# jweyn/DLWP-CS

Measured on AMD Instinct MI355X. Metric: cubed-sphere samples/sec (fwd+bwd), higher is better.
Workload: dtype bf16; 1 GPU; unet2 C48: x (32,6,48,48,14) per GPU, 14 out channels, base 32, MSE + Adam, fwd+bwd+update, bf16 activations + bf16 MFMA, fp32 master weights / gradients / Adam; global_batch=32, parallelism=dp1, hip_graphs=True

## Files before the change

dlwp-cs_amd/DLWP/_native.py:

```python
import ctypes
import os
import threading

import numpy as np
import torch

_HERE = os.path.dirname(os.path.abspath(__file__))
_TAG = os.environ.get('DLWPCS_LIB_TAG', '')
LIB_PATH = os.path.join(os.path.dirname(_HERE), 'lib', 'libdlwpcs%s.so' % ('_' + _TAG if _TAG else ''))

F32 = 0
BF16 = 1
I16 = 2
MAP_RENORMALIZE = 1
MSE_TARGET_F32 = 0x100
MSE_OVERWRITE = 0x200
ADAM_ZERO_GRAD = 1
HEAD_DEFER_STAGE2 = 2
LOSS_MSE, LOSS_MAE, LOSS_ACC = 0, 1, 2
REG_NONE, REG_MSE, REG_MAE, REG_GLOBAL = 0, 1, 2, 3
NORM_ALL, NORM_VALID = 0, 1
E_UNSUPPORTED = -2
ACT_NONE = 0
ACT_LEAKY_CLIP = 1
CONV_ACCUMULATE_WGRAD = 1
CONV_PREPACKED = 2
CONV_REUSE_DZ = 4
CONV_DEFER_REDUCE = 8
CONV_DEFER_RING0 = 16
CONV_OUT_PADDED = 32
CONV_DGRAD_GATHER = 64
CONSTRAINT_MAX_NORM, CONSTRAINT_NON_NEG, CONSTRAINT_UNIT_NORM, CONSTRAINT_MIN_MAX_NORM = 1, 2, 3, 4
PACK_FWD, PACK_BWD, PACK_BIAS = 0, 1, 2
WGRAD_BATCH_MAX = 24

c_void_p, c_int, c_float, c_size_t = ctypes.c_void_p, ctypes.c_int, ctypes.c_float, ctypes.c_size_t
c_i32p = ctypes.POINTER(ctypes.c_int32)


class ConvDesc(ctypes.Structure):
    _fields_ = [('B', ctypes.c_int32), ('N', ctypes.c_int32), ('C0', ctypes.c_int32), ('C1', ctypes.c_int32),
                ('Cout', ctypes.c_int32), ('ksize', ctypes.c_int32), ('halo', ctypes.c_int32),
                ('up0', ctypes.c_int32), ('flip_north_pole', ctypes.c_int32), ('act', ctypes.c_int32),
                ('alpha', ctypes.c_float), ('vmax', ctypes.c_float), ('dtype', ctypes.c_int32),
                ('flags', ctypes.c_int32), ('c0_valid', ctypes.c_int32)]


class PackItem(ctypes.Structure):
    _fields_ = [(n, ctypes.c_void_p) for n in ('w_eq', 'w_pol', 'w_np', 'b_eq', 'b_pol', 'b_np', 'wpk_fwd', 'wpk_bwd',
                                                'bias_pk')] + \
               [(n, ctypes.c_int32) for n in ('ksize', 'Cin', 'Cout', 'flip_north_pole', 'dtype', 'reserved')]


class ReduceItem(ctypes.Structure):
    _fields_ = [(n, ctypes.c_void_p) for n in ('partial', 'bpartial', 'dw_eq', 'dw_pol', 'dw_np', 'db_eq', 'db_pol',
                                                'db_np')] + \
               [(n, ctypes.c_int32) for n in ('ksize', 'Cin', 'Cout', 'CinP', 'CoutP', 'n_eq', 'n_4', 'n_5',
                                              'flip_north_pole', 'accumulate', 'vec', 'nblocks')] + \
               [('reserved', ctypes.c_int32 * 4)]


class WgradItem(ctypes.Structure):
    _fields_ = [('d', ConvDesc)] + [(n, ctypes.c_void_p) for n in ('src0', 'src1', 'dz', 'y', 'table_dev', 'dw_eq', 'dw_pol',
                                                                    'dw_np', 'db_eq', 'db_pol', 'db_np')]


class LossTail(ctypes.Structure):
    _fields_ = [('partial', ctypes.c_void_p), ('loss_out', ctypes.c_void_p), ('nblocks', ctypes.c_int32), ('inv_n', ctypes.c_float),
                ('weight', ctypes.c_float), ('overwrite', ctypes.c_int32)]


class LossDesc(ctypes.Structure):
    _fields_ = [('kind', ctypes.c_int32), ('loss_weight', ctypes.c_float), ('weight', ctypes.c_void_p),
                ('weight_div', ctypes.c_int32), ('weight_period', ctypes.c_int32), ('clim', ctypes.c_void_p),
                ('clim_div', ctypes.c_int32), ('clim_period', ctypes.c_int32), ('regularize', ctypes.c_int32),
                ('reverse', ctypes.c_int32), ('overwrite', ctypes.c_int32)]


class GConvDesc(ctypes.Structure):
    _fields_ = [(n, ctypes.c_int32) for n in
                ('B', 'H', 'W', 'Cin', 'Cout', 'kh', 'kw', 'sh', 'sw', 'dh', 'dw', 'pad_t', 'pad_l', 'Ho', 'Wo',
                 'flip_north_pole', 'dtype')]


SCORE_MSE, SCORE_RMSE, SCORE_MAE, SCORE_ACC, SCORE_COS, SCORE_MEAN = 0, 1, 2, 3, 4, 5
SCORE_MAX_DIMS = 8


class ScoreDesc(ctypes.Structure):
    _fields_ = [(n, ctypes.c_int32) for n in ('method', 'n_lead', 't_len', 't_cap', 't_slope', 'n_keep', 'n_red', 'kc')] + \
               [('keep_ext', ctypes.c_int64 * SCORE_MAX_DIMS), ('red_ext', ctypes.c_int64 * SCORE_MAX_DIMS),
                ('lead_stride', ctypes.c_int64 * 4), ('t_stride', ctypes.c_int64 * 4), ('kc_stride', ctypes.c_int64 * 4),
                ('keep_stride', (ctypes.c_int64 * SCORE_MAX_DIMS) * 4), ('red_stride', (ctypes.c_int64 * SCORE_MAX_DIMS) * 4)]


class OverlapDesc(ctypes.Structure):
    _fields_ = [('N', ctypes.c_int32), ('n_lat', ctypes.c_int32), ('n_lon', ctypes.c_int32), ('reserved', ctypes.c_int32),
                ('frames', ((ctypes.c_double * 3) * 3) * 6), ('dust', ctypes.c_double)]


class CubeBilinearDesc(ctypes.Structure):
    _fields_ = [('N', ctypes.c_int32), ('reserved', ctypes.c_int32), ('n_points', ctypes.c_int64),
                ('frames', ((ctypes.c_double * 3) * 3) * 6), ('edge', ((ctypes.c_int32 * 3) * 4) * 6)]


class SparseMapDesc(ctypes.Structure):
    _fields_ = [('n_a', ctypes.c_int64), ('n_b', ctypes.c_int64), ('nnz', ctypes.c_int64), ('x_dtype', ctypes.c_int32),
                ('n_outer', ctypes.c_int32), ('outer_ext', ctypes.c_int64 * 3), ('x_outer_stride', ctypes.c_int64 * 3),
                ('y_outer_stride', ctypes.c_int64 * 3), ('x_space_stride', ctypes.c_int64), ('y_space_stride', ctypes.c_int64),
                ('inner_ext', ctypes.c_int64), ('x_inner_stride', ctypes.c_int64), ('y_inner_stride', ctypes.c_int64)]


GROUP_SLAB_ROWS = 512


class RowsDesc(ctypes.Structure):
    _fields_ = [('n_inner', ctypes.c_int32), ('reserved', ctypes.c_int32), ('src_row_stride', ctypes.c_int64),
                ('out_row_stride', ctypes.c_int64), ('inner_ext', ctypes.c_int64 * SCORE_MAX_DIMS),
                ('src_stride', ctypes.c_int64 * SCORE_MAX_DIMS), ('out_stride', ctypes.c_int64 * SCORE_MAX_DIMS)]


class ZonalSpectrumDesc(ctypes.Structure):
    _fields_ = [(n, ctypes.c_int32) for n in ('L', 'n_wave', 'n_dims', 'remove_mean')] + \
               [('ext', ctypes.c_int64 * SCORE_MAX_DIMS), ('kept', ctypes.c_int32 * SCORE_MAX_DIMS),
                ('stride', (ctypes.c_int64 * SCORE_MAX_DIMS) * 3)]


ENSEMBLE_MAX_M = 128


class EnsembleDesc(ctypes.Structure):
    _fields_ = [(n, ctypes.c_int32) for n in ('M', 'n_dims', 'fair', 'ddof', 'variance', 'reserved')] + \
               [('member_stride', ctypes.c_int64), ('ext', ctypes.c_int64 * SCORE_MAX_DIMS),
                ('stride', (ctypes.c_int64 * SCORE_MAX_DIMS) * 2)]


AFFINE_MUL_ADD, AFFINE_SUB_DIV = 0, 1
AFFINE_MAX_CHANNELS = 1024


class ChanDesc(ctypes.Structure):
    _fields_ = [(n, ctypes.c_int64) for n in ('R', 'C', 'S', 'row_stride', 'chan_stride', 'inner_stride', 'dst_row_stride',
                                              'dst_chan_stride', 'dst_inner_stride')]


PROTOTYPES = {
    'dlwpcs_version': (c_int, []),
    'dlwpcs_last_error': (ctypes.c_char_p, []),
    'dlwpcs_halo_table': (c_int, [c_int, c_int, c_void_p]),
    'dlwpcs_halo_inverse_table': (c_int, [c_int, c_int, c_void_p]),
    'dlwpcs_dgrad_gather_plan_ints': (c_size_t, [c_int]),
    'dlwpcs_dgrad_gather_plan': (c_int, [c_int, c_void_p]),
    'dlwpcs_pad_fwd': (c_int, [c_void_p, c_void_p, c_int, c_int, c_int, c_int, c_int, c_void_p, c_void_p]),
    'dlwpcs_pad_bwd': (c_int, [c_void_p, c_void_p, c_int, c_int, c_int, c_int, c_int, c_void_p, c_void_p]),
    'dlwpcs_conv_workspace_bytes': (c_size_t, [ctypes.POINTER(ConvDesc)]),
    'dlwpcs_conv_packed_bytes': (c_size_t, [ctypes.POINTER(ConvDesc), c_int]),
    'dlwpcs_pack_batch': (c_int, [c_void_p, c_int, c_void_p]),
    'dlwpcs_conv_fwd': (c_int, [ctypes.POINTER(ConvDesc)] + [c_void_p] * 8 + [c_void_p, c_void_p, c_void_p, c_size_t,
                                                                                 c_void_p]),
    'dlwpcs_conv_fwd_pool': (c_int, [ctypes.POINTER(ConvDesc)] + [c_void_p] * 8 + [c_void_p, c_void_p, c_void_p, c_void_p, c_size_t,
                                                                                      c_void_p]),
    'dlwpcs_conv_fwd_head': (c_int, [ctypes.POINTER(ConvDesc)] + [c_void_p] * 4 + [ctypes.POINTER(ConvDesc)] + [c_void_p] * 6 +
                             [c_size_t, ctypes.POINTER(c_int), c_void_p]),
    'dlwpcs_conv_bwd_data': (c_int, [ctypes.POINTER(ConvDesc)] + [c_void_p] * 5 + [c_void_p, c_void_p, c_void_p,
                                                                                      c_void_p, c_size_t, c_void_p]),
    'dlwpcs_conv_bwd_data_masked': (c_int, [ctypes.POINTER(ConvDesc)] + [c_void_p] * 4 + [c_void_p] * 4 + [c_float, c_float] +
                                    [c_void_p, c_void_p, c_size_t, c_void_p]),
    'dlwpcs_conv_small_fwd': (c_int, [ctypes.POINTER(ConvDesc)] + [c_void_p] * 8 + [c_void_p, c_void_p, c_void_p, c_size_t,
                                                                                       c_void_p]),
    'dlwpcs_conv_small_bwd_data': (c_int, [ctypes.POINTER(ConvDesc)] + [c_void_p] * 4 + [c_void_p] * 4 + [c_float, c_float] +
                                   [c_void_p, c_void_p, c_size_t, c_void_p]),
    'dlwpcs_conv_bwd_weights': (c_int, [ctypes.POINTER(ConvDesc)] + [c_void_p] * 4 + [c_void_p] * 6 +
                                [c_void_p, c_void_p, c_size_t, c_void_p]),
    'dlwpcs_conv_wgrad_reduce_item': (c_int, [ctypes.POINTER(ConvDesc)] + [c_void_p] * 6 +
                                      [c_void_p, c_size_t, ctypes.POINTER(ReduceItem)]),
    'dlwpcs_wgrad_reduce_batch': (c_int, [c_void_p, c_void_p, c_int, c_void_p]),
    'dlwpcs_wgrad_batch_supported': (c_int, [ctypes.POINTER(ConvDesc)]),
    'dlwpcs_wgrad_batch_sizes': (c_int, [c_void_p, c_int, ctypes.POINTER(c_size_t), ctypes.POINTER(c_size_t)]),
    'dlwpcs_wgrad_batch_plan': (c_int, [c_void_p, c_int, c_void_p, c_size_t]),
    'dlwpcs_wgrad_batch': (c_int, [c_void_p, c_int, c_void_p, c_void_p, c_void_p, c_size_t, c_void_p]),
    'dlwpcs_wgrad_batch_adam': (c_int, [c_void_p, c_int, c_void_p, c_void_p, c_void_p, c_size_t, c_void_p, c_void_p, c_void_p,
                                        c_void_p, c_size_t, c_void_p, c_void_p, c_void_p]),
    'dlwpcs_wgrad_batch_adam_tail': (c_int, [c_void_p, c_int, c_void_p, c_void_p, c_void_p, c_size_t, c_void_p, c_void_p, c_void_p,
                                             c_void_p, c_size_t, c_void_p, c_void_p, c_void_p, c_void_p, c_void_p]),
    'dlwpcs_wgrad_batch_apply': (c_int, [c_void_p, c_int, c_void_p, c_void_p, c_void_p, c_void_p, c_void_p, c_void_p, c_size_t,
                                         c_void_p, c_void_p, c_void_p, c_void_p, c_void_p]),
    'dlwpcs_gconv_fwd': (c_int, [ctypes.POINTER(GConvDesc)] + [c_void_p] * 9),
    'dlwpcs_gconv_bwd_data': (c_int, [ctypes.POINTER(GConvDesc)] + [c_void_p] * 6),
    'dlwpcs_gconv_bwd_weights': (c_int, [ctypes.POINTER(GConvDesc)] + [c_void_p] * 9),
    'dlwpcs_act_fwd': (c_int, [c_void_p, c_void_p, c_size_t, c_int, c_float, c_float, c_int, c_void_p]),
    'dlwpcs_act_bwd': (c_int, [c_void_p, c_void_p, c_void_p, c_size_t, c_int, c_float, c_float, c_int, c_void_p]),
    'dlwpcs_avgpool2_fwd': (c_int, [c_void_p, c_void_p, c_int, c_int, c_int, c_int, c_void_p]),
    'dlwpcs_avgpool2_bwd': (c_int, [c_void_p, c_void_p, c_int, c_int, c_int, c_int, c_void_p]),
    'dlwpcs_avgpool2_bwd_add': (c_int, [c_void_p, c_void_p, c_void_p, c_int, c_int, c_int, c_int, c_void_p]),
    'dlwpcs_avgpool2_bwd_masked': (c_int, [c_void_p, c_void_p, c_void_p, c_void_p, c_int, c_int, c_int, c_float, c_float, c_int,
                                           c_void_p]),
    'dlwpcs_avgpool2_bwd_ring': (c_int, [c_void_p, c_void_p, c_void_p, c_void_p, c_int, c_int, c_int, c_float, c_float, c_int,
                                         c_void_p, c_void_p, c_int, c_int, c_void_p]),
    'dlwpcs_conv_ring_info': (c_int, [ctypes.POINTER(ConvDesc), ctypes.POINTER(c_size_t), ctypes.POINTER(c_int)]),
    'dlwpcs_upsample2_fwd': (c_int, [c_void_p, c_void_p, c_int, c_int, c_int, c_int, c_void_p]),
    'dlwpcs_upsample2_bwd': (c_int, [c_void_p, c_void_p, c_int, c_int, c_int, c_int, c_void_p]),
    'dlwpcs_concat2': (c_int, [c_void_p, c_void_p, c_void_p, c_size_t, c_int, c_int, c_int, c_void_p]),
    'dlwpcs_split2': (c_int, [c_void_p, c_void_p, c_void_p, c_size_t, c_int, c_int, c_int, c_void_p]),
    'dlwpcs_cf_to_cl': (c_int, [c_void_p, c_void_p, c_int, c_int, c_size_t, c_int, c_void_p]),
    'dlwpcs_cl_to_cf': (c_int, [c_void_p, c_void_p, c_int, c_int, c_size_t, c_int, c_void_p]),
    'dlwpcs_add': (c_int, [c_void_p, c_void_p, c_void_p, c_size_t, c_int, c_void_p]),
    'dlwpcs_l1l2_regularize': (c_int, [c_void_p, c_void_p, c_size_t, c_float, c_float, c_float, c_void_p, c_void_p]),
    'dlwpcs_weight_constraint': (c_int, [c_void_p, c_int, c_int, c_int, c_float, c_float, c_float, c_void_p]),
    'dlwpcs_mse_scratch_bytes': (c_size_t, []),
    'dlwpcs_mse_fwd_bwd': (c_int, [c_void_p, c_void_p, c_void_p, c_void_p, c_size_t, c_float, c_int, c_void_p,
                                   c_void_p]),
    'dlwpcs_loss_scratch_bytes': (c_size_t, []),
    'dlwpcs_loss_fwd_bwd': (c_int, [c_void_p, c_void_p, c_void_p, c_void_p, c_void_p, c_size_t, c_int, c_void_p, c_void_p]),
    'dlwpcs_loss_masked_fwd_bwd': (c_int, [c_void_p, c_void_p, c_void_p, c_int, c_void_p, c_void_p, c_void_p, c_size_t, c_int,
                                           c_void_p, c_void_p]),
    'dlwpcs_head_loss_step': (c_int, [c_void_p, c_void_p, c_void_p, c_void_p, c_void_p, c_void_p, c_void_p, c_void_p, c_void_p,
                                      c_void_p, c_void_p, c_int, c_float, c_float, c_void_p]),
    'dlwpcs_score_scratch_bytes': (c_size_t, [c_void_p]),
    'dlwpcs_score': (c_int, [c_void_p, c_void_p, c_void_p, c_void_p, c_void_p, c_void_p, c_int, c_void_p, c_size_t, c_void_p]),
    'dlwpcs_score_indexed': (c_int, [c_void_p, c_void_p, c_void_p, c_void_p, c_void_p, c_void_p, ctypes.c_int64, c_void_p, c_int,
                                     c_void_p, c_size_t, c_void_p]),
    'dlwpcs_score_plan_info': (c_int, [c_void_p, c_void_p, c_void_p, c_void_p, c_void_p, c_int, ctypes.c_int64, c_void_p]),
    'dlwpcs_group_mean_scratch_bytes': (c_size_t, [c_void_p, c_int, ctypes.c_int64, c_int]),
    'dlwpcs_group_mean': (c_int, [c_void_p, c_void_p, c_void_p, c_void_p, c_int, ctypes.c_int64, c_int, c_void_p, c_void_p,
                                  c_void_p, c_size_t, c_void_p]),
    'dlwpcs_rows_gather': (c_int, [c_void_p, c_void_p, c_void_p, ctypes.c_int64, c_void_p, c_void_p]),
    'dlwpcs_sparse_map_apply': (c_int, [c_void_p, c_void_p, c_void_p, c_void_p, c_void_p, c_void_p, c_void_p]),
    'dlwpcs_sparse_map_apply_masked': (c_int, [c_void_p, c_void_p, c_void_p, c_void_p, c_void_p, c_void_p, c_void_p, c_float, c_int,
                                               c_void_p]),
    'dlwpcs_missing_count': (c_int, [c_void_p, c_int, ctypes.c_int64, ctypes.c_int64, c_void_p, c_void_p]),
    'dlwpcs_fill_missing': (c_int, [c_void_p, c_int, c_size_t, c_void_p, c_int, c_int, c_void_p]),
    'dlwpcs_zonal_spectrum_scratch_bytes': (c_size_t, [c_void_p]),
    'dlwpcs_zonal_spectrum': (c_int, [c_void_p, c_void_p, c_void_p, c_void_p, c_void_p, c_void_p, c_void_p, c_void_p, c_void_p]),
    'dlwpcs_ensemble_stats': (c_int, [c_void_p, c_void_p, c_void_p, c_void_p, c_void_p, c_void_p, c_void_p, c_void_p]),
    'dlwpcs_ensemble_plan_info': (c_int, [c_void_p, c_void_p, c_void_p, c_void_p]),
    'dlwpcs_overlap_count': (c_int, [c_void_p, c_void_p, c_void_p, c_void_p, c_void_p]),
    'dlwpcs_overlap_fill': (c_int, [c_void_p, c_void_p, c_void_p, c_void_p, c_void_p, c_void_p, ctypes.c_int64, c_void_p]),
    'dlwpcs_cube_bilinear': (c_int, [c_void_p, c_void_p, c_void_p, c_void_p, c_void_p, c_void_p]),
    'dlwpcs_adam_step': (c_int, [c_void_p, c_void_p, c_void_p, c_void_p, c_size_t, c_void_p, c_float, c_float,
                                 c_float, c_float, c_float, c_void_p]),
    'dlwpcs_adam_step_fused': (c_int, [c_void_p, c_void_p, c_void_p, c_void_p, c_size_t, c_void_p, c_float, c_float,
                                       c_float, c_float, c_float, c_int, c_void_p]),
    'dlwpcs_pad_channels': (c_int, [c_void_p, c_void_p, c_size_t, c_int, c_int, c_int, c_void_p]),
    'dlwpcs_slice_channels': (c_int, [c_void_p, c_void_p, c_size_t, c_int, c_int, c_int, c_void_p]),
    'dlwpcs_state_repack': (c_int, [c_void_p, c_void_p, c_void_p, c_int, c_size_t, c_int, c_int, c_int, c_int, c_void_p]),
    'dlwpcs_head_mse_scratch_bytes': (c_size_t, []),
    'dlwpcs_head_mse_tail': (c_int, [c_void_p, c_float, c_int, c_void_p, c_void_p, c_void_p]),
    'dlwpcs_loss_tail_run': (c_int, [c_void_p, c_void_p]),
    'dlwpcs_head_mse_step': (c_int, [c_void_p, c_void_p, c_void_p, c_void_p, c_void_p, c_void_p, c_float, c_void_p, c_void_p,
                                     c_void_p, c_int, c_void_p, c_void_p]),
    'dlwpcs_head_mse_step_masked': (c_int, [c_void_p, c_void_p, c_void_p, c_void_p, c_void_p, c_void_p, c_float, c_void_p,
                                            c_void_p, c_void_p, c_int, c_void_p, c_float, c_float, c_void_p]),
    'dlwpcs_adam_step_dev': (c_int, [c_void_p, c_void_p, c_void_p, c_void_p, c_size_t, c_void_p, c_void_p, c_int,
                                     c_void_p]),
    'dlwpcs_batch_gather': (c_int, [c_void_p, ctypes.c_int64, c_int, ctypes.c_int64, c_void_p, c_int, c_void_p, c_int,
                                    c_int, c_int, c_int, c_void_p, c_int, c_int, c_int, c_int, c_int, c_void_p]),
    'dlwpcs_solar_fill': (c_int, [c_void_p, ctypes.c_int64, c_void_p, ctypes.c_int64, c_void_p, c_int, c_int, c_int, c_int,
                                  c_void_p, c_int, c_int, c_int, c_int, c_int, c_void_p]),
    'dlwpcs_channel_moments_scratch_bytes': (c_size_t, [c_void_p, ctypes.c_int64]),
    'dlwpcs_channel_moments': (c_int, [c_void_p, c_void_p, c_void_p, ctypes.c_int64, c_void_p, c_int, c_void_p, c_void_p, c_size_t,
                                       c_void_p]),
    'dlwpcs_channel_affine': (c_int, [c_void_p, c_void_p, c_void_p, c_void_p, c_int, c_void_p, c_void_p]),
    'dlwpcs_channel_range_scratch_bytes': (c_size_t, [ctypes.c_int64, ctypes.c_int64, ctypes.c_int64]),
    'dlwpcs_channel_range': (c_int, [c_void_p, ctypes.c_int64, ctypes.c_int64, ctypes.c_int64, c_void_p, c_void_p, c_void_p,
                                     c_size_t, c_void_p]),
    'dlwpcs_pack_i16': (c_int, [c_void_p, ctypes.c_int64, ctypes.c_int64, ctypes.c_int64, c_void_p, c_void_p, c_void_p, c_void_p]),
    'dlwpcs_unpack_i16': (c_int, [c_void_p, ctypes.c_int64, ctypes.c_int64, ctypes.c_int64, c_void_p, c_void_p, c_void_p,
                                  c_void_p]),
    'dlwpcs_batch_gather_i16': (c_int, [c_void_p, ctypes.c_int64, c_int, ctypes.c_int64, c_void_p, c_void_p, c_void_p, c_int,
                                        c_void_p, c_int, c_int, c_int, c_int, c_void_p, c_int, c_int, c_int, c_int, c_int,
                                        c_void_p]),
    'dlwpcs_comm_load': (c_int, [ctypes.c_char_p]),
    'dlwpcs_comm_unique_id': (c_int, [c_void_p]),
    'dlwpcs_comm_init': (c_int, [ctypes.POINTER(c_void_p), c_void_p, c_int, c_int]),
    'dlwpcs_comm_destroy': (c_int, [c_void_p]),
    'dlwpcs_allreduce_f32': (c_int, [c_void_p, c_void_p, c_size_t, c_void_p]),
    'dlwpcs_lds_oob_probe': (c_int, [c_void_p, c_void_p]),
    'dlwpcs_prof_enable': (c_int, [c_int]),
    'dlwpcs_prof_reset': (c_int, []),
    'dlwpcs_prof_count': (c_int, []),
    'dlwpcs_prof_get': (c_int, [c_int, ctypes.c_char_p, c_int, ctypes.POINTER(ctypes.c_double),
                                ctypes.POINTER(ctypes.c_double), ctypes.POINTER(ctypes.c_double)]),
    'dlwpcs_prof_known_tags': (c_int, []),
    'dlwpcs_prof_known_tag': (c_int, [c_int, ctypes.c_char_p, c_int]),
}

_lib = None
_lock = threading.Lock()


class NativeError(RuntimeError):
    pass


def lib():
    global _lib
    if _lib is None:
        with _lock:
            if _lib is None:
                if not os.path.exists(LIB_PATH):
                    raise NativeError(
                        'libdlwpcs.so not found at %s: build it with `python dlwp-cs_amd/build.py` '
                        '(or __graft_entry__.build()).  The DLWP-CS MI355X engine has no CPU fallback.' % LIB_PATH)
                handle = ctypes.CDLL(LIB_PATH)
                for name, (res, args) in PROTOTYPES.items():
                    fn = getattr(handle, name)
                    fn.restype = res
                    fn.argtypes = args
                _lib = handle
    return _lib


def check(rc, what):
    if rc != 0:
        msg = lib().dlwpcs_last_error()
        msg = msg.decode() if msg else ''
        if rc == -1:
            raise ValueError('%s: %s' % (what, msg))
        if rc == -2:
            raise NotImplementedError('%s: %s' % (what, msg))
        raise NativeError('%s failed (code %d): %s' % (what, rc, msg))


def require_device(t, what):
# ... 103 lines not shown
```

dlwp-cs_amd/DLWP/custom.py:

```python


import numpy as np

from . import ops
from ._native import ACT_LEAKY_CLIP, ACT_NONE
from .keras import constraints, engine, regularizers
from .keras.callbacks import Callback, EarlyStopping
from .keras.engine import Layer
from .keras.losses import LossSpec, mean_absolute_error, mean_squared_error, spec_of



def _normalize_tuple(value, n, name):
    if isinstance(value, int):
        return (value,) * n
    try:
        value_tuple = tuple(value)
    except TypeError:
        raise ValueError('The `' + name + '` argument must be a tuple of ' + str(n) + ' integers. Received: ' +
                         str(value))
    if len(value_tuple) != n:
        raise ValueError('The `' + name + '` argument must be a tuple of ' + str(n) + ' integers. Received: ' +
                         str(value))
    for single_value in value_tuple:
# ... 27 lines not shown


def _conv_output_length(input_length, filter_size, padding, stride, dilation=1):
    if input_length is None:
        return None
    dilated_filter_size = filter_size + (filter_size - 1) * (dilation - 1)
    if padding == 'same':
        output_length = input_length
    else:
        output_length = input_length - dilated_filter_size + 1
    return (output_length + stride - 1) // stride



class CubeSpherePadding2D(Layer):

    def __init__(self, padding=(1, 1), data_format='channels_first', **kwargs):
        data_format = _normalize_data_format(data_format)
        super(CubeSpherePadding2D, self).__init__(**kwargs)
        if isinstance(padding, int):
            padding = ((padding, padding), (padding, padding), (padding, padding))
        elif hasattr(padding, '__len__'):
            if len(padding) != 3:
                raise ValueError('`padding` should have 3 elements. Found: ' + str(padding))
            dim1_padding = _normalize_tuple(padding[0], 2, '1st entry of padding')
            dim2_padding = _normalize_tuple(padding[1], 2, '2nd entry of padding')
            dim3_padding = _normalize_tuple(padding[2], 2, '3rd entry of padding')
            padding = (dim1_padding, dim2_padding, dim3_padding)
        else:
            raise ValueError('`padding` should be either an int, a tuple of 3 ints (symmetric_dim1_pad, '
                             'symmetric_dim2_pad, symmetric_dim3_pad), or a tuple of 3 tuples of 2 ints ((left_dim1_pad, '
                             'right_dim1_pad), (left_dim2_pad, right_dim2_pad), (left_dim3_pad, right_dim2_pad)). '
                             'Found: ' + str(padding))
        self.data_format = data_format
        self.padding = ((0, 0),) + tuple(padding[1:])

    def compute_output_shape(self, input_shape):
        input_shape = tuple(input_shape)
        add = [q[0] + q[1] for q in self.padding]
        if self.data_format == 'channels_first':
            dims = [None if input_shape[2 + i] is None else input_shape[2 + i] + add[i] for i in range(3)]
            return (input_shape[0], input_shape[1]) + tuple(dims)
        dims = [None if input_shape[1 + i] is None else input_shape[1 + i] + add[i] for i in range(3)]
        return (input_shape[0],) + tuple(dims) + (input_shape[4],)

    def call(self, inputs):
        p = self.padding[1][0]
        if self.data_format == 'channels_first':
            x = ops.channels_first_to_last(inputs)
            return ops.channels_last_to_first(ops.cs_pad(x, p))
        return ops.cs_pad(inputs, p)

    def get_config(self):
        config = {'padding': self.padding, 'data_format': self.data_format}
        base_config = super(CubeSpherePadding2D, self).get_config()
        return dict(list(base_config.items()) + list(config.items()))


class CubeSphereConv2D(Layer):

    def __init__(self,
                 filters,
                 kernel_size,
                 strides=1,
                 padding='valid',
                 data_format='channels_first',
                 dilation_rate=1,
                 activation=None,
                 use_bias=True,
                 flip_north_pole=True,
                 independent_north_pole=False,
                 kernel_initializer='glorot_uniform',
                 bias_initializer='zeros',
                 kernel_regularizer=None,
                 bias_regularizer=None,
                 activity_regularizer=None,
                 kernel_constraint=None,
                 bias_constraint=None,
                 **kwargs):
        super(CubeSphereConv2D, self).__init__(**kwargs)
        self.filters = filters
        self.kernel_size = _normalize_tuple(kernel_size, 2, 'kernel_size')
        self.strides = _normalize_tuple(strides, 2, 'strides')
        self.padding = _normalize_padding(padding)
        self.data_format = _normalize_data_format(data_format)
        self.dilation_rate = _normalize_tuple(dilation_rate, 2, 'dilation_rate')
        self.activation = engine.get_activation(activation)
        self.use_bias = use_bias
        self.flip_north_pole = flip_north_pole
        self.independent_north_pole = independent_north_pole
        self.kernel_initializer = engine.get_initializer(kernel_initializer)
        self.bias_initializer = engine.get_initializer(bias_initializer)
        self.kernel_regularizer = regularizers.get(kernel_regularizer)
        self.bias_regularizer = regularizers.get(bias_regularizer)
        self.activity_regularizer = engine._passthrough_get(activity_regularizer)
        self.kernel_constraint = constraints.get(kernel_constraint)
        self.bias_constraint = constraints.get(bias_constraint)
        self.rank = 3

        self.equatorial_kernel = None
        self.equatorial_bias = None
        self.polar_kernel = None
        self.polar_bias = None
        self.north_pole_kernel = None
        self.north_pole_bias = None

    def _weight_attr_names(self):
        return ['equatorial_kernel', 'polar_kernel', 'north_pole_kernel', 'equatorial_bias', 'polar_bias',
                'north_pole_bias']

    def build(self, input_shape):
        if self.data_format == 'channels_first':
            channel_axis = 1
        else:
            channel_axis = -1
        if input_shape[channel_axis] is None:
            raise ValueError('The channel dimension of the inputs should be defined. Found `None`.')
        input_dim = int(input_shape[channel_axis])
        kernel_shape = self.kernel_size + (input_dim, self.filters)

        self.equatorial_kernel = self.add_weight(shape=kernel_shape, initializer=self.kernel_initializer,
                                                 name='equatorial_kernel', regularizer=self.kernel_regularizer,
                                                 constraint=self.kernel_constraint)
        self.polar_kernel = self.add_weight(shape=kernel_shape, initializer=self.kernel_initializer,
                                            name='polar_kernel', regularizer=self.kernel_regularizer,
                                            constraint=self.kernel_constraint)
        if self.independent_north_pole:
            self.north_pole_kernel = self.add_weight(shape=kernel_shape, initializer=self.kernel_initializer,
                                                     name='north_pole_kernel', regularizer=self.kernel_regularizer,
                                                     constraint=self.kernel_constraint)
        if self.use_bias:
            self.equatorial_bias = self.add_weight(shape=(self.filters,), initializer=self.bias_initializer,
                                                   name='equatorial_bias', regularizer=self.bias_regularizer,
                                                   constraint=self.bias_constraint)
            self.polar_bias = self.add_weight(shape=(self.filters,), initializer=self.bias_initializer,
                                              name='polar_bias', regularizer=self.bias_regularizer,
                                              constraint=self.bias_constraint)
            if self.independent_north_pole:
                self.north_pole_bias = self.add_weight(shape=(self.filters,), initializer=self.bias_initializer,
                                                       name='north_pole_bias', regularizer=self.bias_regularizer,
                                                       constraint=self.bias_constraint)
        self.input_dim = input_dim
        self.built = True

    def _is_mfma_config(self):
        k = self.kernel_size
        return (k[0] == k[1] and k[0] in (1, 3) and self.strides == (1, 1) and self.dilation_rate == (1, 1)
                and self.padding == 'valid')

    def can_fuse_halo(self, pad_width):
        return (self._is_mfma_config() and self.kernel_size[0] == 3 and pad_width == 1 and self.activation is None)

    def fused_call(self, src0, src1=None, up0=False, halo=True, act=ACT_NONE, alpha=0.0, vmax=0.0, premask0=None,
                   premask1=None, dy_premasked=False, defer_ring0=False, want_pool=False, out_padded=False, small=False):
        return ops.cs_conv(src0, self.equatorial_kernel, self.polar_kernel, self.north_pole_kernel,
                           self.equatorial_bias, self.polar_bias, self.north_pole_bias, src1=src1,
                           ksize=self.kernel_size[0], halo=halo, up0=up0, flip_north_pole=self.flip_north_pole,
                           act=act, alpha=alpha, vmax=vmax, premask0=premask0, premask1=premask1,
                           dy_premasked=dy_premasked, defer_ring0=defer_ring0, want_pool=want_pool, out_padded=out_padded,
                           small=small)

    def call(self, inputs, channels_last_io=False, **kwargs):
        channels_first = self.data_format == 'channels_first' and not channels_last_io
        x = ops.channels_first_to_last(inputs) if channels_first else inputs
        if self._is_mfma_config():
            outputs = ops.cs_conv(x, self.equatorial_kernel, self.polar_kernel, self.north_pole_kernel,
                                  self.equatorial_bias, self.polar_bias, self.north_pole_bias,
                                  ksize=self.kernel_size[0], halo=False, flip_north_pole=self.flip_north_pole)
        else:
            outputs = ops.cs_gconv(x, self.equatorial_kernel, self.polar_kernel, self.north_pole_kernel,
                                   self.equatorial_bias, self.polar_bias, self.north_pole_bias,
                                   strides=self.strides, padding=self.padding, dilation=self.dilation_rate,
                                   flip_north_pole=self.flip_north_pole)
        if channels_first:
            outputs = ops.channels_last_to_first(outputs)
        if self.activation is not None:
            return self.activation(outputs)
        return outputs

    def compute_output_shape(self, input_shape):
        if self.data_format == 'channels_last':
            space = input_shape[2:4]
        else:
            space = input_shape[-2:]
        new_space = []
        for i in range(len(space)):
            new_space.append(_conv_output_length(space[i], self.kernel_size[i], padding=self.padding,
                                                 stride=self.strides[i], dilation=self.dilation_rate[i]))
        if self.data_format == 'channels_last':
            return (input_shape[0], 6) + tuple(new_space) + (self.filters,)
        return (input_shape[0], self.filters, 6) + tuple(new_space)

    def get_config(self):
        config = {
            'filters': self.filters,
            'kernel_size': self.kernel_size,
            'strides': self.strides,
            'padding': self.padding,
            'data_format': self.data_format,
            'dilation_rate': self.dilation_rate,
            'activation': engine.serialize_activation(self.activation),
            'use_bias': self.use_bias,
            'flip_north_pole': self.flip_north_pole,
            'independent_north_pole': self.independent_north_pole,
            'kernel_initializer': engine.serialize_initializer(self.kernel_initializer),
            'bias_initializer': engine.serialize_initializer(self.bias_initializer),
            'kernel_regularizer': regularizers.serialize(self.kernel_regularizer),
            'bias_regularizer': regularizers.serialize(self.bias_regularizer),
            'activity_regularizer': self.activity_regularizer,
            'kernel_constraint': constraints.serialize(self.kernel_constraint),
            'bias_constraint': constraints.serialize(self.bias_constraint)
        }
        base_config = super(CubeSphereConv2D, self).get_config()
        return dict(list(base_config.items()) + list(config.items()))



def _adam_effective_lr(optimizer, beta_1, beta_2, with_bias_correction):
    it = float(optimizer.iterations)
    lr = float(optimizer.lr) / (1. + float(getattr(optimizer, 'decay', 0.)) * it)
    if with_bias_correction:
        t = it + 1.
        lr = lr * np.sqrt(1. - np.power(beta_2, t)) / (1. - np.power(beta_1, t))
    return lr


class AdamLearningRateTracker(Callback):

    def on_epoch_end(self, epoch, logs=None, beta_1=0.9, beta_2=0.999, ):
        print(' - LR: {:.6f}'.format(_adam_effective_lr(self.model.optimizer, beta_1, beta_2, True)))


class SGDLearningRateTracker(Callback):

    def on_epoch_end(self, epoch, logs=None):
        print(' - LR: {:.6f}'.format(_adam_effective_lr(self.model.optimizer, 0., 0., False)))


class BatchHistory(Callback):

    def on_train_begin(self, logs=None):
        self.history, self.epoch = [], 0

    def on_epoch_begin(self, epoch, logs=None):
        self.history.append(dict())

    def on_batch_end(self, batch, logs=None):
        for key, value in (logs or {}).items():
            self.history[self.epoch].setdefault(key, []).append(value)

    def on_epoch_end(self, epoch, logs=None):
        self.epoch += 1


class RunHistory(Callback):

    def __init__(self, run):
        super(RunHistory, self).__init__()
        self.run = run
        self.epoch, self.history = [], {}

    def on_train_begin(self, logs=None):
        self.epoch, self.history = [], {}

    def on_epoch_end(self, epoch, logs=None):
        self.epoch.append(epoch)
        for key, value in (logs or {}).items():
            self.history.setdefault(key, []).append(value)
            self.run.log(key, value)


class RNNResetStates(Callback):

    def on_epoch_begin(self, epoch, logs=None):
        self.model.reset_states()


class EarlyStoppingMin(EarlyStopping):

    def __init__(self, min_epochs=0, max_epochs=None, **kwargs):
        super(EarlyStoppingMin, self).__init__(**kwargs)
        if not isinstance(min_epochs, int) or min_epochs < 0:
            raise ValueError('min_epochs must be an integer >= 0')
        self.min_epochs = int(min_epochs)
        self.max_epochs = None if max_epochs is None else int(max_epochs)

    def _stop(self, epoch, message):
        self.stopped_epoch = epoch
        self.model.stop_training = True
        if self.restore_best_weights:
            if self.verbose > 0:
                print(message)
            self.model.set_weights(self.best_weights)

    def on_epoch_end(self, epoch, logs=None):
        if epoch < self.min_epochs:
            return
        current = self.get_monitor_value(logs)
        if current is None:
            return
        improved = self.monitor_op(current - self.min_delta, self.best)
        if improved:
            self.best, self.wait = current, 0
            if self.restore_best_weights:
                self.best_weights = self.model.get_weights()
        else:
            self.wait += 1
            if self.wait >= self.patience:
                self._stop(epoch, 'Restoring model weights from the end of the best epoch')
        if self.max_epochs is not None and epoch >= self.max_epochs:
            self._stop(epoch, 'Maximum epochs reached; restoring model weights from the end of the best epoch')
        if self.verbose > 1:
            print('EarlyStoppingMin: %d epochs since last minimum' % self.wait)
# ... 169 lines not shown
```

dlwp-cs_amd/DLWP/keras/models.py:

```python
import gc
import json
import os
import sys
import time

import numpy as np
import torch

from .. import ops, parallel
from ..options import option
from .. import _native as _nat
from .._native import ACT_LEAKY_CLIP, ACT_NONE
from . import backend, callbacks as cbks, losses as klosses, optimizers, staging
from .engine import KTensor, Layer
from .layers import AveragePooling3D, Concatenate, InputLayer, ReLU, UpSampling3D


def _new_graph():
    if os.environ.get('DLWPCS_KEEP_GRAPH', '0') == '1':
        return torch.cuda.CUDAGraph(keep_graph=True)
    return torch.cuda.CUDAGraph()


def _as_list(x):
    if isinstance(x, (list, tuple)):
        return list(x)
    return [x]


class Model(object):
    def __init__(self, inputs=None, outputs=None, name=None):
        if inputs is None or outputs is None:
            raise ValueError('Model needs `inputs` and `outputs`')
        self._single_input = not isinstance(inputs, (list, tuple))
        self.inputs = _as_list(inputs)
        self.outputs = _as_list(outputs)
        self._single_output = len(self.outputs) == 1
        for t in self.inputs + self.outputs:
            if not isinstance(t, KTensor):
                raise ValueError('Model inputs/outputs must be symbolic tensors created by Input() and layer calls')
        self.name = name or 'model'
        self.stop_training = False
        self.optimizer = None
        self.loss = None
        self._dev_losses = None
        self.loss_weights = None
        self.metrics = []
        self.history = None
        self.use_graphs = option('graphs')
        self.compute_dtype = backend.compute_dtype()
        self.prepack_weights = True
        self.wgrad_side_stream = False
        self.defer_wgrad_reduce = True
        self.batch_wgrad = option('wgrad_batch')
        self.check_finite = option('check_finite')
        self.fuse_adam = option('fuse_adam')
        self.fold_ring = option('fold_ring')
        self.fuse_pool = option('fuse_pool')
        self.fold_loss_tail = option('fold_loss_tail')
        self.fuse_pack = option('fuse_pack')
        self._packed_ok = False
        self.exchange_buckets = int(os.environ.get('DLWPCS_EXCHANGE_BUCKETS', '1'))
        self._stager = None
        self.fuse_head_loss = option('fuse_head')
        self.fold_head = option('fold_head')
        self.small_conv = option('small_conv')
        self.static_batch_buffers = False
        self._ones = {}
        self._compiled = False
        self._flat_params = self._flat_grads = None
        self._grads_clean = False
        self._graphs = {}
        self._infer_graphs = {}
        self._rollout_series = {}
        self.rollout_keep_bytes = 4 << 30
        self._seen_batch = {}
        self._toposort()
        self._build_plan()

    def _toposort(self):
        order, seen = [], set()

        def visit(t):
            if t.uid in seen:
                return
            seen.add(t.uid)
            for i in t.node_inputs:
                visit(i)
            order.append(t)
        for o in self.outputs:
            visit(o)
        input_uids = {t.uid for t in self.inputs}
        for t in order:
            if isinstance(t.layer, InputLayer) and t.uid not in input_uids:
                raise ValueError('Graph disconnected: cannot obtain value for tensor %r' % (t,))
        self._nodes = order
        layers, seen_l = [], set()
        for t in self.inputs + order:
            if t.layer is not None and id(t.layer) not in seen_l:
                seen_l.add(id(t.layer))
                layers.append(t.layer)
        self.layers = layers

    def _build_plan(self):
        consumers = {}
        for t in self._nodes:
            for i in t.node_inputs:
                consumers.setdefault(i.uid, []).append(t)
        out_uids = {o.uid for o in self.outputs}

        def sole_consumer(t):
            c = consumers.get(t.uid, [])
            return c[0] if (len(c) == 1 and t.uid not in out_uids) else None

        from ..custom import CubeSphereConv2D, CubeSpherePadding2D
        def cf_layer(t):
            lay = t.layer
            if isinstance(lay, InputLayer):
                return len(t.shape) == 5
            if isinstance(lay, CubeSphereConv2D) and lay.activation is not None \
                    and getattr(lay.activation, '_dlwp_name', None) != 'relu':
                return False
            if isinstance(lay, (CubeSpherePadding2D, CubeSphereConv2D, AveragePooling3D, UpSampling3D)):
                return lay.data_format == 'channels_first'
            if isinstance(lay, Concatenate):
                return lay._axis(len(t.shape)) == 1
            return isinstance(lay, ReLU)
        self._cf_model = (option('cf_model') and all(cf_layer(t) for t in self._nodes)
                          and any(isinstance(t.layer, (CubeSphereConv2D, CubeSpherePadding2D)) for t in self._nodes))
        fmt = 'channels_first' if self._cf_model else 'channels_last'
        virtual = set()
        fused = {}
        for t in self._nodes:
            lay = t.layer
            if not isinstance(lay, CubeSphereConv2D) or len(t.node_inputs) != 1:
                continue
            padt = t.node_inputs[0]
            if not isinstance(padt.layer, CubeSpherePadding2D) or sole_consumer(padt) is not t:
                continue
            if padt.layer.data_format != fmt or lay.data_format != fmt or not lay.can_fuse_halo(padt.layer.padding[1][0]):
                continue
            if padt.layer.padding[1] != padt.layer.padding[2] or padt.layer.padding[1][0] != padt.layer.padding[1][1]:
                continue
            x = padt.node_inputs[0]
            src0, src1, up0 = x, None, False
            chain = [padt]
            if isinstance(x.layer, Concatenate) and len(x.node_inputs) == 2 and sole_consumer(x) is padt \
                    and x.layer._axis(len(x.shape)) == (1 if self._cf_model else len(x.shape) - 1):
                src0, src1 = x.node_inputs
                chain.append(x)
            if isinstance(src0.layer, UpSampling3D) and sole_consumer(src0) is (chain[-1]) \
                    and src0.layer.size == (1, 2, 2):
                chain.append(src0)
                src0 = src0.node_inputs[0]
                up0 = True
            out_t, act, alpha, vmax = t, ACT_NONE, 0.0, 0.0
            nxt = sole_consumer(t)
            if nxt is not None and isinstance(nxt.layer, ReLU) and nxt.layer.threshold == 0.:
                out_t, act = nxt, ACT_LEAKY_CLIP
                alpha = nxt.layer.negative_slope
                vmax = float('inf') if nxt.layer.max_value is None else nxt.layer.max_value
                virtual.add(t.uid)
            for c in chain:
                virtual.add(c.uid)
            fused[out_t.uid] = ('fused_conv', out_t.uid, lay, src0.uid, None if src1 is None else src1.uid, up0, act,
                                alpha, vmax)
        steps = []
        for t in self._nodes:
            if isinstance(t.layer, InputLayer) or t.uid in virtual and t.uid not in fused:
                continue
            if t.uid in fused:
                steps.append(fused[t.uid])
            elif isinstance(t.layer, AveragePooling3D) and len(t.node_inputs) == 1 and self._runs_channels_last(t.layer) and (
                    len(consumers.get(t.node_inputs[0].uid, [])) > 1 or t.node_inputs[0].uid in out_uids):
                steps.append(('pool_skip', t.uid, t.layer, t.node_inputs[0].uid))
            else:
                steps.append(('layer', t.uid, t.layer, [i.uid for i in t.node_inputs],
                              isinstance(t.layer, Concatenate)))
        self._plan = steps
        self.n_fused = len(fused)
        self._padded_io_ok = False
        if len(self.inputs) == 1:
            u = self.inputs[0].uid
            rd = [st for st in steps
                  if (st[0] == 'fused_conv' and u in (st[3], st[4])) or (st[0] == 'pool_skip' and st[3] == u)
                  or (st[0] == 'layer' and u in st[3])]
            self._padded_io_ok = (len(rd) == 1 and rd[0][0] == 'fused_conv' and rd[0][3] == u and rd[0][4] is None
                                  and not rd[0][5] and u not in out_uids and not self._cf_model)
        self._plan_premask(steps, out_uids)
        self._head_fold = {}
        for i, st in enumerate(steps):
            if st[0] != 'fused_conv' or st[1] in out_uids:
                continue
            rd = [j for j, s2 in enumerate(steps)
                  if (s2[0] == 'fused_conv' and st[1] in (s2[3], s2[4])) or (s2[0] == 'pool_skip' and s2[3] == st[1])
                  or (s2[0] == 'layer' and st[1] in s2[3])]
            if len(rd) != 1 or steps[rd[0]][0] != 'layer':
                continue
            hl = steps[rd[0]][2]
            if (isinstance(hl, CubeSphereConv2D) and len(steps[rd[0]][3]) == 1 and tuple(hl.kernel_size) == (1, 1)
                    and hl.activation is None and not hl.independent_north_pole and not st[2].independent_north_pole
                    and st[2].filters == 32 and self._runs_channels_last(hl) and not self._cf_model):
                self._head_fold[i] = rd[0]
        uids = [o.uid for o in self.outputs]
        self._sole_outputs = {u for u in uids if not consumers.get(u) and uids.count(u) == 1}

    def _plan_premask(self, steps, out_uids):
        from ..custom import CubeSphereConv2D
        produced = {}
        for st in steps:
            if st[0] == 'fused_conv' and st[6] == ACT_LEAKY_CLIP:
                produced[st[1]] = (float(st[7]), float(st[8]))
        capable = {u: (u not in out_uids) for u in produced}
        in_uids_model = {t.uid for t in self.inputs}
        for st in steps:
            if st[0] == 'fused_conv' and st[1] in capable and st[3] in in_uids_model and (st[4] is None or st[4] in in_uids_model):
                capable[st[1]] = False
        aliased = set()
        src_mask = {}
# ... 19 lines not shown
        self._src_mask = src_mask
        readers = {}
        for i, st in enumerate(steps):
            ins = [st[3], st[4]] if st[0] == 'fused_conv' else ([st[3]] if st[0] == 'pool_skip' else list(st[3]))
            for u in ins:
                if u is not None:
                    readers.setdefault(u, []).append(i)
        self._pool_producers = set()
        for i, st in enumerate(steps):
            if st[0] == 'fused_conv':
                r = readers.get(st[1], [])
                if r and steps[r[0]][0] == 'pool_skip' and steps[r[0]][3] == st[1]:
                    self._pool_producers.add(i)
        self._defer_ring = set()
        for i, st in enumerate(steps):
            if st[0] != 'pool_skip' or not (src_mask.get(i) and st[3] in self._premask):
                continue
            r = readers.get(st[1], [])
            if len(r) == 1 and st[1] not in out_uids and steps[r[0]][0] == 'fused_conv' and steps[r[0]][3] == st[1] \
                    and steps[r[0]][4] != st[1] and not steps[r[0]][5]:
                self._defer_ring.add(r[0])

    def _runs_channels_last(self, lay):
        return lay.data_format == 'channels_last' or self._cf_model

    def _plan_exchange(self):
        if self._exchange_cut is not None:
            return self._exchange_cut or None
        self._exchange_cut = False
        if self._flat_grads is None:
            return None
        base = self._flat_grads.data_ptr()
        spans = []
        for st in self._plan:
            ws = [w for w in getattr(st[2], '_weights', []) if w.requires_grad and w.grad is not None]
            if ws:
                lo = min((w.grad.data_ptr() - base) // 4 for w in ws)
                hi = max((w.grad.data_ptr() - base) // 4 + w.numel() for w in ws)
                spans.append((lo, hi))
            else:
                spans.append(None)
        total = sum(hi - lo for sp in spans if sp for lo, hi in [sp])
        if total == 0:
            return None
        acc, cut = 0, None
        for i in range(len(spans) - 1, 0, -1):
            if spans[i]:
                acc += spans[i][1] - spans[i][0]
                if acc >= 0.4 * total:
                    cut = i
                    break
        if cut is None or not any(spans[:cut]):
            return None
        lo_a = min(sp[0] for sp in spans[cut:] if sp)
        if any(sp and sp[1] > lo_a for sp in spans[:cut]):
            return None
        self._exchange_cut = (cut, int(lo_a) // 64 * 64)
        return self._exchange_cut

    def _premask_on(self):
        return (self.compute_dtype == 'bfloat16' and torch.is_grad_enabled()
                and option('premask'))

    def _pack_state(self, device):
        from ..custom import CubeSphereConv2D
        from .. import _native as nat
        tag = nat.BF16 if self.compute_dtype == 'bfloat16' else nat.F32
        key = (str(device), tag, self._flat_params.data_ptr() if self._flat_params is not None else 0)
        st = getattr(self, '_pack_cache', None)
        if st is not None and st['key'] == key:
            return st
        entries, table, by_grad = [], {}, {}
        for lay in self.layers:
            if not isinstance(lay, CubeSphereConv2D) or not lay.built or not lay._is_mfma_config():
                continue
            we = lay.equatorial_kernel
            if we.device != device or id(we) in table:
                continue
            bufs = ops.conv_packed_buffers(lay.kernel_size[0], we.shape[2], we.shape[3], tag, device,
                                           bias=lay.equatorial_bias is not None)
            entries.append((we, lay.polar_kernel, lay.north_pole_kernel, lay.equatorial_bias, lay.polar_bias,
                            lay.north_pole_bias, bufs, lay.kernel_size[0], lay.flip_north_pole, tag))
            table[id(we)] = (tag, bufs[0], bufs[1], bufs[2])
            if we.grad is not None:
                by_grad[we.grad.data_ptr()] = entries[-1]
        st = {'key': key, 'items': ops.make_pack_items(entries, device) if entries else None, 'n': len(entries),
              'table': table, 'keep': entries, 'by_grad': by_grad}
        self._pack_cache = st
        return st

    def _forward(self, inputs, repack=True, fuse_targets=None):
        want = backend.torch_dtype(self.compute_dtype)
        inputs = [v if v.dtype == want else v.to(want) for v in inputs]
        if inputs and inputs[0].is_cuda and self.prepack_weights:
            st = self._pack_state(inputs[0].device)
            if st['n'] and (repack or not st.get('packed')):
                ops.pack_batch(st['items'], st['n'])
                st['packed'] = True
                st['packed_version'] = self._flat_params._version if self._flat_params is not None else None
                self._packed_ok = True
            ops.PREPACKED = st['table']
            try:
                return self._run_plan(inputs, fuse_targets)
            finally:
                ops.PREPACKED = {}
        return self._run_plan(inputs, fuse_targets)

    def _run_plan(self, inputs, fuse_targets=None):
        from ..custom import CubeSphereConv2D, CubeSpherePadding2D
        cf = self._cf_model
        if cf:
            inputs = [ops.channels_first_to_last(v) for v in inputs]
        values = {t.uid: v for t, v in zip(self.inputs, inputs)}
        self._fused_outputs = set()
        pm = self._premask if self._premask_on() else {}
        cut = getattr(self, '_record_cut', None)
        self._cut_tensors = []
        ops._POOLED.clear()
        folded = set()
        for i, st in enumerate(self._plan):
            if i in folded:
                continue
            if cut is not None and i == cut:
                need, seen = set(), set()
                for s2 in self._plan[cut:]:
                    ins = [s2[3], s2[4]] if s2[0] == 'fused_conv' else ([s2[3]] if s2[0] == 'pool_skip' else list(s2[3]))
                    need.update(u for u in ins if u is not None)
                for u, v in values.items():
                    if u in need and isinstance(v, torch.Tensor) and v.requires_grad and id(v) not in seen:
                        seen.add(id(v))
                        self._cut_tensors.append(v)
            if st[0] == 'fused_conv':
                _, out_uid, lay, s0, s1, up0, act, alpha, vmax = st
                j = self._head_fold.get(i) if self.fold_head else None
                if j is not None and fuse_targets is None and not torch.is_grad_enabled():
                    hl, h_uid = self._plan[j][2], self._plan[j][1]
                    padded = bool(getattr(self, '_padded_io', False) and h_uid in self._sole_outputs and hl.filters % 8 != 0)
                    if (lay._is_mfma_config() and hl._is_mfma_config() and hl.built and lay.built and ops.cs_conv_head_applicable(
                            values[s0], None if s1 is None else values[s1], lay.equatorial_kernel, hl.equatorial_kernel, padded)):
                        values[h_uid] = ops.cs_conv_head(values[s0], lay.equatorial_kernel, lay.equatorial_bias,
                                                         hl.equatorial_kernel, hl.equatorial_bias,
                                                         src1=None if s1 is None else values[s1], up0=up0,
                                                         flip_north_pole=lay.flip_north_pole, act=act, alpha=alpha, vmax=vmax,
                                                         out_padded=padded)
                        folded.add(j)
                        continue
                m0, m1 = self._src_mask[i]
                values[out_uid] = lay.fused_call(values[s0], None if s1 is None else values[s1], up0=up0, halo=True,
                                                 act=act, alpha=alpha, vmax=vmax,
                                                 premask0=pm.get(s0) if m0 else None, premask1=pm.get(s1) if m1 else None,
                                                 dy_premasked=out_uid in pm,
                                                 defer_ring0=bool(pm) and self.fold_ring and i in self._defer_ring,
                                                 want_pool=self.fuse_pool and i in self._pool_producers,
                                                 small=self.small_conv)
            elif st[0] == 'pool_skip':
                _, out_uid, lay, in_uid = st
                values[out_uid], values[in_uid] = ops.avgpool2_skip(values[in_uid],
                                                                     pm.get(in_uid) if self._src_mask[i] else None)
                if cut is not None and i < cut:
                    values[in_uid] = ops.detour(values[in_uid])
            else:
                _, out_uid, lay, in_uids, takes_list = st
                args = [values[u] for u in in_uids]
                head_pm = pm.get(in_uids[0]) if (self._src_mask[i] and in_uids) else None
                if (fuse_targets is not None and out_uid in fuse_targets and out_uid in self._sole_outputs
                        and isinstance(lay, CubeSphereConv2D) and len(args) == 1 and lay._is_mfma_config()
                        and self._runs_channels_last(lay) and lay.activation is None and lay.north_pole_kernel is None
                        and ops.head_mse_applicable(args[0], lay.equatorial_kernel, lay.kernel_size[0], ACT_NONE,
                                                    fuse_targets[out_uid][0], fuse_targets[out_uid][2])):
                    tgt, wgt, dl = fuse_targets[out_uid]
                    values[out_uid] = ops.head_mse(args[0], tgt, lay.equatorial_kernel, lay.polar_kernel, lay.equatorial_bias,
                                                   lay.polar_bias, wgt, lay.flip_north_pole, premask=head_pm, loss=dl)
                    self._fused_outputs.add(out_uid)
                    continue
                if head_pm is not None:
                    values[out_uid] = lay.fused_call(args[0], halo=False, premask0=head_pm)
                    continue
                if (getattr(self, '_padded_io', False) and out_uid in self._sole_outputs and isinstance(lay, CubeSphereConv2D)
                        and len(args) == 1 and lay._is_mfma_config() and self._runs_channels_last(lay)
                        and lay.activation is None and lay.kernel_size[0] == 1 and args[0].dtype == torch.bfloat16
                        and args[0].shape[-1] == 32 and 8 <= lay.filters <= 32 and lay.filters % 2 == 0
                        and (args[0].shape[2] * args[0].shape[3]) % 16 == 0):
                    values[out_uid] = lay.fused_call(args[0], halo=False, out_padded=True)
                    continue
                if cf:
                    if isinstance(lay, CubeSphereConv2D):
                        values[out_uid] = lay.call(args[0], channels_last_io=True)
                    elif isinstance(lay, CubeSpherePadding2D):
                        values[out_uid] = ops.cs_pad(args[0], lay.padding[1][0])
                    elif isinstance(lay, AveragePooling3D):
                        values[out_uid] = ops.avgpool2(args[0])
                    elif isinstance(lay, UpSampling3D):
                        values[out_uid] = ops.upsample2(args[0])
                    elif isinstance(lay, Concatenate):
                        values[out_uid] = ops.concat_channels(list(args))
                    else:
                        values[out_uid] = lay.call(args[0])
                    continue
                values[out_uid] = lay.call(args if (takes_list or len(args) > 1) else args[0])
        if cf and not getattr(self, '_loss_in_cl', False):
            return [values[o.uid] if o.uid in self._fused_outputs else ops.channels_last_to_first(values[o.uid])
                    for o in self.outputs]
        return [values[o.uid] for o in self.outputs]

    def __call__(self, inputs):
        self._grads_clean = False
        outs = self._forward(_as_list(inputs))
        return outs[0] if self._single_output else outs

    def _weight_layers(self):
        return [l for l in self.layers if l._weights]

    @property
    def weights(self):
        return [w for l in self._weight_layers() for w in l._weights]

    @property
    def trainable_weights(self):
        return [w for w in self.weights if w.requires_grad]

    def count_params(self):
        return int(sum(w.numel() for w in self.weights))

    def get_weights(self):
        return [a for l in self._weight_layers() for a in l.get_weights()]

    def set_weights(self, weights):
        weights = list(weights)
        n = sum(len(l._weights) for l in self._weight_layers())
        if len(weights) != n:
            raise ValueError('You called `set_weights(weights)` on model "%s" with a weight list of length %d, but the '
                             'model was expecting %d weights.' % (self.name, len(weights), n))
        k = 0
        for l in self._weight_layers():
            l.set_weights(weights[k:k + len(l._weights)])
            k += len(l._weights)

    def _flatten_parameters(self):
        ws = self.weights
        dev = backend.device()
        total = sum(w.numel() for w in ws)
        offsets, off = [], 0
        for w in ws:
            offsets.append(off)
            off += (w.numel() + 63) // 64 * 64
        flat = torch.zeros(off, dtype=torch.float32, device=dev)
        grads = torch.zeros(off, dtype=torch.float32, device=dev)
        k = 0
        for l in self._weight_layers():
            new = []
            for w in l._weights:
                o = offsets[k]
                view = flat[o:o + w.numel()].view(w.shape)
                with torch.no_grad():
                    view.copy_(w.detach().to(dev))
                view.requires_grad_(w.requires_grad)
                if w.requires_grad:
                    view.grad = grads[o:o + w.numel()].view(w.shape)
                new.append(view)
                k += 1
            l._rebind(new)
        self._flat_params, self._flat_grads = flat, grads
        self._wrules = None
        self._flat_len = off
        self._n_params = total
        self._exchange_cut = None

    def compile(self, optimizer='adam', loss=None, metrics=None, loss_weights=None, **kwargs):
        self.optimizer = optimizers.get(optimizer)
        mp_dtype = getattr(self.optimizer, '_mixed_precision', None)
        if mp_dtype is not None and mp_dtype != backend.compute_dtype() and mp_dtype != self.compute_dtype:
            import warnings
            warnings.warn('compile(): the optimizer was returned by enable_mixed_precision_graph_rewrite(); the model is put '
                          'into the %s mode although the global policy is %s now (pass a fresh optimizer to avoid this)'
                          % (mp_dtype, backend.compute_dtype()))
        if mp_dtype is not None and mp_dtype != self.compute_dtype:
            self.compute_dtype = mp_dtype
            self._pack_cache = None
        n_out = len(self.outputs)
        losses = _as_list(loss) if isinstance(loss, (list, tuple)) else [loss] * n_out
        if len(losses) != n_out:
            raise ValueError('When passing a list as loss, it should have one entry per model output. The model has %d '
                             'outputs, but you passed loss=%s' % (n_out, loss))
        specs = []
        for l in losses:
            sp = klosses.spec_of(l) if not isinstance(l, str) or l in ('mse', 'mean_squared_error', 'MSE') else None
            if sp is None and isinstance(l, str):
                raise NotImplementedError("loss %r: of the loss names the DLWP-CS engine takes 'mse' (reference "
                                          "Azure/train_cs.py:424); pass the function for the others, e.g. "
                                          "DLWP.keras.losses.mean_absolute_error" % (l,))
            if sp is None:
                raise NotImplementedError("loss %r: the DLWP-CS engine provides 'mse', 'mae' (DLWP.keras.losses) and the "
                                          "losses of DLWP.custom: latitude_weighted_loss, anomaly_correlation(_loss), masked_loss" % (l,))
            if sp.regularize == 'spatial':
                raise NotImplementedError("anomaly-correlation regularize_mean='spatial': a per-sample reduction over the layout's "
                                          "last two axes (reference DLWP/custom.py:1604-1606,1657-1659) the DLWP-CS engine does "
                                          "not build")
            if sp.kind == 'acc' and parallel.world()[1] > 1:
                raise NotImplementedError('the anomaly-correlation loss is a ratio of sums over the WHOLE batch: per-rank values '
                                          'averaged across %d data-parallel ranks are a different loss (train it on one rank)'
                                          % parallel.world()[1])
            if sp.masked == 'valid' and parallel.world()[1] > 1:
                raise NotImplementedError("masked_loss(normalize='valid') divides by the number of valid elements of the WHOLE "
                                          "batch: per-rank nan-means averaged across %d data-parallel ranks are a different loss "
                                          "(train it on one rank, or use normalize='all', which is exact under averaging)"
                                          % parallel.world()[1])
            specs.append(sp)
# ... 1307 lines not shown
```

dlwp-cs_amd/DLWP/ops.py:

```python
import ctypes
import os

import numpy as np
import torch

from . import _native as nat
from .options import option
from ._native import ConvDesc, GConvDesc, check, lib, ptr, require_device, stream_ptr

DIRECT_PARAM_GRADS = False

PREPACKED = {}

WGRAD_SIDE_STREAM = False
_side_streams = {}


def side_stream(device):
    key = str(device)
    st = _side_streams.get(key)
    if st is None:
        st = torch.cuda.Stream(device=device)
        _side_streams[key] = st
    return st
# ... 257 lines not shown
def _c(t):
    return t if t.is_contiguous() else t.contiguous()



class _CSPad(torch.autograd.Function):
    @staticmethod
    def forward(ctx, x, p):
        require_device(x, 'cs_pad')
        x = _c(x)
        B, F6, N, N2, C = x.shape
        if F6 != 6 or N != N2:
            raise ValueError('cs_pad: expected (B, 6, N, N, C), got %s' % (tuple(x.shape),))
        table, inv = nat.halo_tables(N, p, x.device)
        y = torch.empty((B, 6, N + 2 * p, N + 2 * p, C), dtype=x.dtype, device=x.device)
        check(lib().dlwpcs_pad_fwd(ptr(x), ptr(y), B, N, C, p, nat.dtype_tag(x), ptr(table), stream_ptr()),
              'dlwpcs_pad_fwd')
        ctx.p, ctx.shape = p, (B, N, C)
        ctx.inv = inv
        return y

    @staticmethod
    def backward(ctx, dy):
        B, N, C = ctx.shape
        dy = _c(dy)
        dx = torch.empty((B, 6, N, N, C), dtype=dy.dtype, device=dy.device)
        check(lib().dlwpcs_pad_bwd(ptr(dy), ptr(dx), B, N, C, ctx.p, nat.dtype_tag(dy), ptr(ctx.inv), stream_ptr()),
              'dlwpcs_pad_bwd')
        return dx, None


def cs_pad(x, p):
    return _CSPad.apply(x, int(p))



def _make_desc(B, N, C0, C1, Cout, ksize, halo, up0, flip, act, alpha, vmax, dtype=nat.F32, c0_valid=0):
    return ConvDesc(B=B, N=N, C0=C0, C1=C1, Cout=Cout, ksize=ksize, halo=int(halo), up0=int(up0),
                    flip_north_pole=int(flip), act=int(act), alpha=float(alpha), vmax=float(vmax), dtype=int(dtype),
                    flags=0, c0_valid=int(c0_valid))


class _PadChannels(torch.autograd.Function):

    @staticmethod
    def forward(ctx, x, cp):
        require_device(x, 'pad_channels')
        x = _c(x)
        C = x.shape[-1]
        rows = x.numel() // C if C else 0
        y = torch.empty(tuple(x.shape[:-1]) + (cp,), dtype=x.dtype, device=x.device)
        check(lib().dlwpcs_pad_channels(ptr(x), ptr(y), rows, C, cp, nat.dtype_tag(x), stream_ptr()), 'dlwpcs_pad_channels')
        ctx.c = C
        return y

    @staticmethod
    def backward(ctx, dy):
        dy = _c(dy)
        cp = dy.shape[-1]
        rows = dy.numel() // cp
        dx = torch.empty(tuple(dy.shape[:-1]) + (ctx.c,), dtype=dy.dtype, device=dy.device)
        check(lib().dlwpcs_slice_channels(ptr(dy), ptr(dx), rows, cp, ctx.c, nat.dtype_tag(dy), stream_ptr()),
              'dlwpcs_slice_channels')
        return dx, None


def pad_channels(x, cp):
    if x.shape[-1] == cp:
        return x
    if x.shape[-1] > cp:
        raise ValueError('pad_channels: tensor has %d channels, asked for %d' % (x.shape[-1], cp))
    return _PadChannels.apply(x, int(cp))


def channel_vector(dtype):
    return 8 if dtype == torch.bfloat16 else 4


def padded_channels(c, dtype, even_too=None):
    v = channel_vector(dtype)
    if c % v == 0:
        return c
    if c % 2 == 1 or even_too:
        return (c + v - 1) // v * v
    return c


def _f32_param(t, what):
    if t is not None and t.dtype != torch.float32:
        raise TypeError('%s: parameters must be float32 master copies, got %s' % (what, t.dtype))


def _weight_gradients(d, src0, src1, dy, y, params, table, ws, nbytes, direct, defer, need, has_np, has_bias, has_bnp,
                      batch_mask_ok=False):
    dev = dy.device
    w_eq, w_pol, w_np = params[0], params[1], params[2]
    dw_eq = dw_pol = dw_np = db_eq = db_pol = db_np = None
    if (direct and WGRAD_BATCH and d.B > 0 and not WGRAD_SIDE_STREAM and wgrad_batch_supported(d)
            and (d.act == nat.ACT_NONE or (batch_mask_ok and d.ksize == 3 and y is not None))):
        pe, pp, pn, be, bp, bn = params
        d2 = ConvDesc.from_buffer_copy(d)
        _wb_pending.append((d2, src0, src1, dy, table,
                            (pe.grad, pp.grad, None if pn is None else pn.grad, None if be is None else be.grad,
                             None if bp is None else bp.grad, None if bn is None else bn.grad),
                            None if d.act == nat.ACT_NONE else y))
        return dw_eq, dw_pol, dw_np, db_eq, db_pol, db_np
    if direct:
        pe, pp, pn, be, bp, bn = params
        d2 = ConvDesc.from_buffer_copy(d)
        d2.flags = d.flags | nat.CONV_ACCUMULATE_WGRAD | (nat.CONV_DEFER_REDUCE if defer else 0)
        grads = (ptr(pe.grad), ptr(pp.grad), ptr(None if pn is None else pn.grad),
                 ptr(None if be is None else be.grad), ptr(None if bp is None else bp.grad),
                 ptr(None if bn is None else bn.grad))

        def launch(wsx):
            check(lib().dlwpcs_conv_bwd_weights(ctypes.byref(d2), ptr(src0), ptr(src1), ptr(dy), ptr(y), *grads,
                                                ptr(table), ptr(wsx), wsx.numel(), stream_ptr()),
                  'dlwpcs_conv_bwd_weights')
            if defer:
                item = nat.ReduceItem()
                check(lib().dlwpcs_conv_wgrad_reduce_item(ctypes.byref(d2), *grads, ptr(wsx), wsx.numel(),
                                                          ctypes.byref(item)), 'dlwpcs_conv_wgrad_reduce_item')
                _deferred.append((item, wsx))
        if WGRAD_SIDE_STREAM:
            side = side_stream(dev)
            side.wait_stream(torch.cuda.current_stream(dev))
            ws2 = _workspace(nbytes, dev, 'side')
            with torch.cuda.stream(side):
                launch(ws2)
            for t in (src0, src1, dy, y):
                if t is not None:
                    t.record_stream(side)
        else:
            launch(ws)
    elif any(need):
        dw_eq, dw_pol = torch.empty_like(w_eq), torch.empty_like(w_pol)
        dw_np = torch.empty_like(w_np) if has_np else None
        if has_bias:
            db_eq = torch.empty(d.Cout, dtype=torch.float32, device=dev)
            db_pol = torch.empty(d.Cout, dtype=torch.float32, device=dev)
            db_np = torch.empty(d.Cout, dtype=torch.float32, device=dev) if has_bnp else None
        check(lib().dlwpcs_conv_bwd_weights(ctypes.byref(d), ptr(src0), ptr(src1), ptr(dy), ptr(y), ptr(dw_eq),
                                            ptr(dw_pol), ptr(dw_np), ptr(db_eq), ptr(db_pol), ptr(db_np),
                                            ptr(table), ptr(ws), ws.numel(), stream_ptr()),
              'dlwpcs_conv_bwd_weights')
    return dw_eq, dw_pol, dw_np, db_eq, db_pol, db_np


class _CSConv(torch.autograd.Function):

    @staticmethod
    def forward(ctx, src0, src1, w_eq, w_pol, w_np, b_eq, b_pol, b_np, ksize, halo, up0, flip, act, alpha, vmax,
                c0_valid=0, premask0=None, premask1=None, dy_premasked=False, defer_ring0=False, want_pool=False,
                out_padded=False, small=False):
        require_device(src0, 'cs_conv')
        src0 = _c(src0)
        B = src0.shape[0]
        if src0.dim() != 5 or src0.shape[1] != 6 or src0.shape[2] != src0.shape[3]:
            raise ValueError('cs_conv: expected (B, 6, N, N, C), got %s' % (tuple(src0.shape),))
        N = src0.shape[2] * (2 if up0 else 1)
        C0 = src0.shape[4]
        C1 = 0
        if src1 is not None:
            require_device(src1, 'cs_conv')
            src1 = _c(src1)
            if tuple(src1.shape[:4]) != (B, 6, N, N):
                raise ValueError('cs_conv: src1 shape %s does not match (B,6,%d,%d,*)' % (tuple(src1.shape), N, N))
            C1 = src1.shape[4]
            if src1.dtype != src0.dtype:
                raise TypeError('cs_conv: src0 is %s but src1 is %s' % (src0.dtype, src1.dtype))
        for prm in (w_eq, w_pol, w_np, b_eq, b_pol, b_np):
            _f32_param(prm, 'cs_conv')
        kh, kw, cin, Cout = w_eq.shape
        if kh != ksize or kw != ksize or cin != (c0_valid or C0) + C1:
            raise ValueError('cs_conv: kernel shape %s does not match ksize=%d, C_in=%d' % (tuple(w_eq.shape), ksize,
                                                                                          (c0_valid or C0) + C1))
        w_eq, w_pol = _c(w_eq), _c(w_pol)
        w_np = _c(w_np) if w_np is not None else None
        d = _make_desc(B, N, C0, C1, Cout, ksize, halo, up0, flip, act, alpha, vmax, nat.dtype_tag(src0), c0_valid)
        No = N if halo else N - ksize + 1
        if out_padded:
            if torch.is_grad_enabled() and any(t is not None and t.requires_grad for t in (src0, src1, w_eq)):
                raise RuntimeError('cs_conv: out_padded is an inference-only layout')
            d.flags |= nat.CONV_OUT_PADDED
        y = torch.empty((B, 6, No, No, (Cout + 7) // 8 * 8 if out_padded else Cout), dtype=src0.dtype, device=src0.device)
        table = inv = None
        if halo:
            table, inv = nat.halo_tables(N, (ksize - 1) // 2, src0.device)
        nbytes = lib().dlwpcs_conv_workspace_bytes(ctypes.byref(d))
        ws = _workspace(nbytes, src0.device)
        packed = PREPACKED.get(id(w_eq))
        if packed is not None and packed[0] != d.dtype:
            packed = None
        yp = None
        if want_pool and halo and No % 2 == 0:
            yp = torch.empty((B, 6, No // 2, No // 2, Cout), dtype=src0.dtype, device=src0.device)
        wargs = ((ptr(packed[1]), 0, 0, ptr(packed[2]) if b_eq is not None else 0, 0, 0) if packed is not None else
                 (ptr(w_eq), ptr(w_pol), ptr(w_np), ptr(b_eq), ptr(b_pol), ptr(b_np)))
        if packed is not None:
            d.flags |= nat.CONV_PREPACKED
        small = bool(small) and _small_conv_ok(d)
        if yp is not None:
            check(lib().dlwpcs_conv_fwd_pool(ctypes.byref(d), ptr(src0), ptr(src1), *wargs, ptr(y), ptr(yp), ptr(table), ptr(ws),
                                             ws.numel(), stream_ptr()), 'dlwpcs_conv_fwd_pool')
            _POOLED[y.data_ptr()] = yp
        else:
            rc = nat.E_UNSUPPORTED
            if small:
                rc = lib().dlwpcs_conv_small_fwd(ctypes.byref(d), ptr(src0), ptr(src1), *wargs, ptr(y), ptr(table), ptr(ws),
                                                 ws.numel(), stream_ptr())
            if rc == nat.E_UNSUPPORTED:
                rc = lib().dlwpcs_conv_fwd(ctypes.byref(d), ptr(src0), ptr(src1), *wargs, ptr(y), ptr(table), ptr(ws),
                                           ws.numel(), stream_ptr())
            check(rc, 'dlwpcs_conv_fwd')
        ctx.small = small
        if premask0 is not None and premask1 is not None and tuple(premask0) != tuple(premask1):
            raise ValueError('cs_conv: both sources must share the activation parameters of their masks')
        ctx.premask = (premask0, premask1)
        ctx.dy_premasked = bool(dy_premasked) and act != nat.ACT_NONE
        ctx.defer_ring0 = bool(defer_ring0)
        ctx.packed = packed
        ctx.desc = d
        ctx.tables = (table, inv)
        ctx.has = (src1 is not None, w_np is not None, b_eq is not None, b_np is not None)
        ctx.params = (w_eq, w_pol, w_np, b_eq, b_pol, b_np)
        ctx.save_for_backward(src0, src1, w_eq, w_pol, w_np, y if act != nat.ACT_NONE else None)
        return y

    @staticmethod
    def backward(ctx, dy):
        src0, src1, w_eq, w_pol, w_np, y = ctx.saved_tensors
        d = ctx.desc
        table, inv = ctx.tables
        has_src1, has_np, has_bias, has_bnp = ctx.has
        dy = _c(dy)
        dev = dy.device
        nbytes = lib().dlwpcs_conv_workspace_bytes(ctypes.byref(d))
        need = ctx.needs_input_grad
        dsrc0 = torch.empty_like(src0) if need[0] else None
        dsrc1 = torch.empty_like(src1) if (has_src1 and need[1]) else None
        want_w = any(need[2:8])
        direct = DIRECT_PARAM_GRADS and (need[2] or need[3]) and all(
            p is None or (p.is_leaf and p.grad is not None and p.grad.is_contiguous()) for p in ctx.params)
        pm0, pm1 = ctx.premask
        if dsrc0 is None:
            pm0 = None
        if dsrc1 is None:
            pm1 = None
        masked_io = ctx.dy_premasked or pm0 is not None or pm1 is not None
        if masked_io:
            if ctx.dy_premasked or d.act == nat.ACT_NONE:
                dz = dy
            else:
                dz = torch.empty_like(dy)
                check(lib().dlwpcs_act_bwd(ptr(dy), ptr(y), ptr(dz), dy.numel(), nat.ACT_LEAKY_CLIP, d.alpha, d.vmax,
                                           nat.dtype_tag(dy), stream_ptr()), 'dlwpcs_act_bwd')
            dn = ConvDesc.from_buffer_copy(d)
            dn.act = nat.ACT_NONE
            dn.flags = (d.flags & nat.CONV_PREPACKED) | _gather_flag(d, dev)
            batching = (direct and WGRAD_BATCH and d.B > 0 and not WGRAD_SIDE_STREAM and wgrad_batch_supported(dn))
            defer = direct and DEFER_WGRAD_REDUCE and not WGRAD_SIDE_STREAM and d.B > 0 and not batching
            ws = _workspace(nbytes, dev, 'defer%d' % len(_deferred)) if defer else _workspace(nbytes, dev)
            ring = None
            if ctx.defer_ring0 and dsrc0 is not None and pm0 is None and halo_ring_info(dn) is not None:
                ring = halo_ring_info(dn)
                dn.flags |= nat.CONV_DEFER_RING0
                if not defer:
                    ws = _workspace(nbytes, dev, 'ring%d' % len(_pending_ring))
            if dsrc0 is not None or dsrc1 is not None:
                wq = ctx.packed[3] if ctx.packed is not None else w_eq
                pm = pm0 if pm0 is not None else pm1
                ma, mv = (float(pm[0]), float(pm[1])) if pm is not None else (0.0, 0.0)
                bargs = (ctypes.byref(dn), ptr(dz), ptr(wq), ptr(w_pol), ptr(w_np), ptr(dsrc0), ptr(dsrc1),
                         ptr(src0 if pm0 is not None else None), ptr(src1 if pm1 is not None else None), ma, mv, ptr(inv), ptr(ws),
                         ws.numel(), stream_ptr())
                rc = nat.E_UNSUPPORTED
                if ctx.small and dsrc0 is not None and dsrc1 is None:
                    rc = lib().dlwpcs_conv_small_bwd_data(*bargs)
                if rc == nat.E_UNSUPPORTED:
                    rc = lib().dlwpcs_conv_bwd_data_masked(*bargs)
                check(rc, 'dlwpcs_conv_bwd_data_masked')
                if ring is not None:
                    _pending_ring[dsrc0.data_ptr()] = (ws, ring[0], ring[1], nat.halo_tables(d.N, 1, dev)[1])
                    dn.flags &= ~nat.CONV_DEFER_RING0
            dw_eq, dw_pol, dw_np, db_eq, db_pol, db_np = _weight_gradients(
                dn, src0, src1, dz, None, ctx.params, table, ws, nbytes, direct, defer, need[2:8], has_np, has_bias, has_bnp)
            return (dsrc0, dsrc1, dw_eq, dw_pol, dw_np, db_eq, db_pol, db_np) + (None,) * 15
        no_dgrad = dsrc0 is None and dsrc1 is None
        mask_on_load = d.ksize == 3 and (no_dgrad or d.dtype == nat.F32)
        batching = (direct and WGRAD_BATCH and d.B > 0 and not WGRAD_SIDE_STREAM and wgrad_batch_supported(d)
                    and (d.act == nat.ACT_NONE or mask_on_load))
        defer = direct and DEFER_WGRAD_REDUCE and not WGRAD_SIDE_STREAM and d.B > 0 and not batching
        ws = _workspace(nbytes, dev, 'defer%d' % len(_deferred)) if defer else _workspace(nbytes, dev)
        reuse_dz = ((dsrc0 is not None or dsrc1 is not None) and want_w and d.act != nat.ACT_NONE
                    and not WGRAD_SIDE_STREAM and not batching)
        if reuse_dz:
            d.flags |= nat.CONV_REUSE_DZ

        def run_bwd_data():
            if dsrc0 is not None or dsrc1 is not None:
                wq = ctx.packed[3] if ctx.packed is not None else w_eq
                d.flags |= _gather_flag(d, dev)
                check(lib().dlwpcs_conv_bwd_data(ctypes.byref(d), ptr(dy), ptr(y), ptr(wq), ptr(w_pol), ptr(w_np),
                                                 ptr(dsrc0), ptr(dsrc1), ptr(inv), ptr(ws), ws.numel(), stream_ptr()),
                      'dlwpcs_conv_bwd_data')
                d.flags &= ~nat.CONV_DGRAD_GATHER
        if not reuse_dz:
            run_bwd_data()
        dw_eq, dw_pol, dw_np, db_eq, db_pol, db_np = _weight_gradients(
            d, src0, src1, dy, y, ctx.params, table, ws, nbytes, direct, defer, need[2:8], has_np, has_bias, has_bnp,
            batch_mask_ok=mask_on_load)
        if reuse_dz:
            run_bwd_data()
        return (dsrc0, dsrc1, dw_eq, dw_pol, dw_np, db_eq, db_pol, db_np) + (None,) * 15


def _small_conv_ok(d):
    return (d.dtype == nat.BF16 and d.ksize == 3 and d.halo and d.C1 == 0 and not d.up0 and d.c0_valid == 0
            and d.N * d.N <= 320 and d.C0 % 32 == 0 and d.Cout % 32 == 0 and d.B > 0)


_ring_info_cache = {}



def _gather_flag(d, dev):
    if option('dgrad_gather') and d.halo and d.ksize == 3 and d.dtype == nat.BF16 and nat.dgrad_gather_ready(d.N, 1, dev):
        return nat.CONV_DGRAD_GATHER
    return 0


def halo_ring_info(d):
    key = (d.B, d.N, d.C0, d.C1, d.Cout, d.ksize, d.halo, d.up0, d.dtype, d.c0_valid, d.flags & nat.CONV_DGRAD_GATHER)
    if key not in _ring_info_cache:
        off, ch = ctypes.c_size_t(), ctypes.c_int()
        ok = lib().dlwpcs_conv_ring_info(ctypes.byref(d), ctypes.byref(off), ctypes.byref(ch))
        _ring_info_cache[key] = (off.value, ch.value) if ok else None
    return _ring_info_cache[key]


def conv_packed_buffers(ksize, cin, cout, dtype_tag, device, bias=True):
    d = _make_desc(1, max(ksize, 2), cin, 0, cout, ksize, False, False, True, nat.ACT_NONE, 0.0, 0.0, dtype_tag)
    out = []
    for which in (nat.PACK_FWD, nat.PACK_BIAS, nat.PACK_BWD):
        n = lib().dlwpcs_conv_packed_bytes(ctypes.byref(d), which)
        if n == 0:
            check(-1, 'dlwpcs_conv_packed_bytes')
        out.append(torch.empty(n, dtype=torch.uint8, device=device))
    if not bias:
        out[1] = None
    return tuple(out)


def make_pack_items(entries, device):
    arr = (nat.PackItem * len(entries))()
    for it, (we, wp, wn, be, bp, bn, bufs, ksize, flip, tag) in zip(arr, entries):
        it.w_eq, it.w_pol, it.w_np = ptr(we), ptr(wp), ptr(wn)
        it.b_eq, it.b_pol, it.b_np = ptr(be), ptr(bp), ptr(bn)
        it.wpk_fwd, it.bias_pk, it.wpk_bwd = ptr(bufs[0]), ptr(bufs[1]), ptr(bufs[2])
        it.ksize, it.Cin, it.Cout = int(ksize), int(we.shape[2]), int(we.shape[3])
        it.flip_north_pole, it.dtype, it.reserved = int(flip), int(tag), 0
    raw = bytes(arr)
    host = torch.frombuffer(bytearray(raw), dtype=torch.uint8) if raw else torch.empty(0, dtype=torch.uint8)
    return host.to(device)


def pack_batch(items_dev, n_items):
    check(lib().dlwpcs_pack_batch(ptr(items_dev), int(n_items), stream_ptr()), 'dlwpcs_pack_batch')


def cs_conv(src0, w_eq, w_pol, w_np=None, b_eq=None, b_pol=None, b_np=None, src1=None, ksize=3, halo=True, up0=False,
            flip_north_pole=True, act=nat.ACT_NONE, alpha=0.0, vmax=0.0, premask0=None, premask1=None, dy_premasked=False,
            defer_ring0=False, want_pool=False, out_padded=False, small=False):
    if (w_np is None) != (b_np is None) and b_eq is not None:
        raise ValueError('cs_conv: north-pole kernel and bias must be given together')
    c0_valid = 0
    cin_w = w_eq.shape[2]
    if src1 is None and not up0:
        c_phys = src0.shape[-1]
        if c_phys == cin_w:
            cp = padded_channels(c_phys, src0.dtype)
            if cp != c_phys:
                src0 = pad_channels(src0, cp)
                c0_valid = cin_w
        elif cin_w < c_phys <= (cin_w + channel_vector(src0.dtype) - 1) // channel_vector(src0.dtype) * channel_vector(src0.dtype):
            c0_valid = cin_w
    return _CSConv.apply(src0, src1, w_eq, w_pol, w_np, b_eq, b_pol, b_np, int(ksize), bool(halo), bool(up0),
                         bool(flip_north_pole), int(act), float(alpha), float(vmax), int(c0_valid), premask0, premask1,
                         bool(dy_premasked), bool(defer_ring0), bool(want_pool), bool(out_padded), bool(small))


def cs_conv_head_applicable(src0, src1, w_eq, head_w_eq, out_padded):
    if torch.is_grad_enabled() or not src0.is_cuda or src0.dtype != torch.bfloat16:
        return False
    pk, hk = PREPACKED.get(id(w_eq)), PREPACKED.get(id(head_w_eq))
    if pk is None or hk is None or pk[0] != nat.BF16 or hk[0] != nat.BF16:
        return False
    cout2 = head_w_eq.shape[3]
    rows = (cout2 + 7) // 8 * 8 if out_padded else cout2
    c0, c1 = src0.shape[-1], (src1.shape[-1] if src1 is not None else 0)
    if c0 % 8 or c1 % 8 or c0 + c1 != w_eq.shape[2]:
        return False
    return (tuple(w_eq.shape[:2]) == (3, 3) and w_eq.shape[3] == 32 and tuple(head_w_eq.shape[:3]) == (1, 1, 32) and rows == 32
            and cout2 % 2 == 0 and cout2 >= 8)


def cs_conv_head(src0, w_eq, b_eq, head_w_eq, head_b_eq, src1=None, up0=False, flip_north_pole=True, act=nat.ACT_NONE,
                 alpha=0.0, vmax=0.0, out_padded=False):
    require_device(src0, 'cs_conv_head')
    src0 = _c(src0)
    B = src0.shape[0]
    N = src0.shape[2] * (2 if up0 else 1)
    C0, C1 = src0.shape[4], 0
    if src1 is not None:
        src1 = _c(src1)
        C1 = src1.shape[4]
    Cout, cout2 = w_eq.shape[3], head_w_eq.shape[3]
    pk, hk = PREPACKED[id(w_eq)], PREPACKED[id(head_w_eq)]
    d = _make_desc(B, N, C0, C1, Cout, 3, True, up0, flip_north_pole, act, alpha, vmax, nat.BF16, 0)
    d.flags |= nat.CONV_PREPACKED
    dh = _make_desc(B, N, Cout, 0, cout2, 1, False, False, flip_north_pole, nat.ACT_NONE, 0.0, 0.0, nat.BF16, 0)
    dh.flags |= nat.CONV_PREPACKED | (nat.CONV_OUT_PADDED if out_padded else 0)
    rows = (cout2 + 7) // 8 * 8 if out_padded else cout2
    y = torch.empty((B, 6, N, N, Cout), dtype=src0.dtype, device=src0.device)
    yh = torch.empty((B, 6, N, N, rows), dtype=src0.dtype, device=src0.device)
    table = nat.halo_tables(N, 1, src0.device)[0]
    nbytes = max(lib().dlwpcs_conv_workspace_bytes(ctypes.byref(d)), lib().dlwpcs_conv_workspace_bytes(ctypes.byref(dh)))
    ws = _workspace(nbytes, src0.device)
    fused = ctypes.c_int(0)
    check(lib().dlwpcs_conv_fwd_head(ctypes.byref(d), ptr(src0), ptr(src1), ptr(pk[1]), ptr(pk[2]) if b_eq is not None else 0,
                                     ctypes.byref(dh), ptr(hk[1]), ptr(hk[2]) if head_b_eq is not None else 0, ptr(y), ptr(yh),
                                     ptr(table), ptr(ws), ws.numel(), ctypes.byref(fused), stream_ptr()), 'dlwpcs_conv_fwd_head')
    global HEAD_FOLDED
    HEAD_FOLDED = bool(fused.value)
    return yh


HEAD_FOLDED = False



def _same_pads(n, k, s, dil):
    out = -(-n // s)
    total = max((out - 1) * s + (k - 1) * dil + 1 - n, 0)
    return total // 2, out


def _valid_len(n, k, s, dil):
    return (n - (k - 1) * dil - 1) // s + 1


class _GConv(torch.autograd.Function):
    @staticmethod
    def forward(ctx, x, w_eq, w_pol, w_np, b_eq, b_pol, b_np, strides, padding, dilation, flip):
        require_device(x, 'cs_gconv')
        for prm in (w_eq, w_pol, w_np, b_eq, b_pol, b_np):
            _f32_param(prm, 'cs_gconv')
        x, w_eq, w_pol = _c(x), _c(w_eq), _c(w_pol)
        w_np = _c(w_np) if w_np is not None else None
        B, F6, H, W, Cin = x.shape
        kh, kw, cin, Cout = w_eq.shape
        if F6 != 6 or cin != Cin:
            raise ValueError('cs_gconv: bad shapes x=%s kernel=%s' % (tuple(x.shape), tuple(w_eq.shape)))
        sh, sw = strides
        dh, dw = dilation
        if padding == 'same':
            pad_t, Ho = _same_pads(H, kh, sh, dh)
            pad_l, Wo = _same_pads(W, kw, sw, dw)
        elif padding == 'valid':
            pad_t = pad_l = 0
            Ho = _valid_len(H, kh, sh, dh)
            Wo = _valid_len(W, kw, sw, dw)
        else:
            raise ValueError('padding must be "valid" or "same"')
        if Ho < 1 or Wo < 1:
            raise ValueError('cs_gconv: empty output')
        d = GConvDesc(B=B, H=H, W=W, Cin=Cin, Cout=Cout, kh=kh, kw=kw, sh=sh, sw=sw, dh=dh, dw=dw, pad_t=pad_t,
                      pad_l=pad_l, Ho=Ho, Wo=Wo, flip_north_pole=int(flip), dtype=nat.dtype_tag(x))
        y = torch.empty((B, 6, Ho, Wo, Cout), dtype=x.dtype, device=x.device)
        check(lib().dlwpcs_gconv_fwd(ctypes.byref(d), ptr(x), ptr(w_eq), ptr(w_pol), ptr(w_np), ptr(b_eq), ptr(b_pol),
                                     ptr(b_np), ptr(y), stream_ptr()), 'dlwpcs_gconv_fwd')
        ctx.desc = d
        ctx.has = (w_np is not None, b_eq is not None, b_np is not None)
        ctx.save_for_backward(x, w_eq, w_pol, w_np)
        return y

    @staticmethod
    def backward(ctx, dy):
        x, w_eq, w_pol, w_np = ctx.saved_tensors
        d = ctx.desc
        has_np, has_bias, has_bnp = ctx.has
        dy = _c(dy)
        dx = None
        if ctx.needs_input_grad[0]:
            dx = torch.empty_like(x)
            check(lib().dlwpcs_gconv_bwd_data(ctypes.byref(d), ptr(dy), ptr(w_eq), ptr(w_pol), ptr(w_np), ptr(dx),
                                              stream_ptr()), 'dlwpcs_gconv_bwd_data')
        dw_eq, dw_pol = torch.empty_like(w_eq), torch.empty_like(w_pol)
        dw_np = torch.empty_like(w_np) if has_np else None
        db_eq = db_pol = db_np = None
        if has_bias:
            db_eq = torch.empty(d.Cout, dtype=torch.float32, device=dy.device)
            db_pol = torch.empty_like(db_eq)
            db_np = torch.empty_like(db_eq) if has_bnp else None
        check(lib().dlwpcs_gconv_bwd_weights(ctypes.byref(d), ptr(x), ptr(dy), ptr(dw_eq), ptr(dw_pol), ptr(dw_np),
                                             ptr(db_eq), ptr(db_pol), ptr(db_np), stream_ptr()),
              'dlwpcs_gconv_bwd_weights')
        return dx, dw_eq, dw_pol, dw_np, db_eq, db_pol, db_np, None, None, None, None


def cs_gconv(x, w_eq, w_pol, w_np=None, b_eq=None, b_pol=None, b_np=None, strides=(1, 1), padding='valid',
             dilation=(1, 1), flip_north_pole=True):
    return _GConv.apply(x, w_eq, w_pol, w_np, b_eq, b_pol, b_np, tuple(strides), padding, tuple(dilation),
                        bool(flip_north_pole))



class _Act(torch.autograd.Function):
    @staticmethod
    def forward(ctx, x, alpha, vmax):
        require_device(x, 'leaky_clip_relu')
        x = _c(x)
        y = torch.empty_like(x)
        check(lib().dlwpcs_act_fwd(ptr(x), ptr(y), x.numel(), nat.ACT_LEAKY_CLIP, alpha, vmax, nat.dtype_tag(x),
                                   stream_ptr()),
              'dlwpcs_act_fwd')
        ctx.alpha, ctx.vmax = alpha, vmax
        ctx.save_for_backward(y)
        return y

    @staticmethod
    def backward(ctx, dy):
        (y,) = ctx.saved_tensors
        dy = _c(dy)
        dx = torch.empty_like(dy)
        check(lib().dlwpcs_act_bwd(ptr(dy), ptr(y), ptr(dx), dy.numel(), nat.ACT_LEAKY_CLIP, ctx.alpha, ctx.vmax,
                                   nat.dtype_tag(dy), stream_ptr()), 'dlwpcs_act_bwd')
        return dx, None, None


def leaky_clip_relu(x, negative_slope=0.0, max_value=None):
    vmax = float('inf') if max_value is None else float(max_value)
# ... 1383 lines not shown
```

dlwp-cs_amd/DLWP/options.py:

```python
import os

DEFAULTS = {
    'graphs': True, 'premask': True, 'wgrad_batch': True, 'fuse_adam': True, 'fuse_pack': True, 'fuse_head': True,
    'fold_loss_tail': True, 'fuse_pool': True, 'fold_ring': True, 'cf_model': True, 'padded_io': True, 'host_staging': True, 'resident_data': True,
    'dgrad_gather': True, 'fold_head': True, 'small_conv': True, 'check_finite': False,
}


_parsed = {}


def _parse(env):
    hit = _parsed.get(env)
    if hit is None:
        hit = {}
        for item in env.split(','):
            item = item.strip()
            if not item:
                continue
            k, _, v = item.partition('=')
            k = k.strip()
            if k not in DEFAULTS:
                raise KeyError('DLWPCS_OPTIONS: unknown engine option %r (known: %s)' % (k, ', '.join(sorted(DEFAULTS))))
            hit[k] = v.strip() not in ('0', 'false', 'False', 'off', '')
        if len(_parsed) > 64:
            _parsed.clear()
        _parsed[env] = hit
    return hit


def option(name):
    if name not in DEFAULTS:
        raise KeyError('unknown engine option %r (known: %s)' % (name, ', '.join(sorted(DEFAULTS))))
    return _parse(os.environ.get('DLWPCS_OPTIONS', '')).get(name, DEFAULTS[name])


def snapshot():
    over = _parse(os.environ.get('DLWPCS_OPTIONS', ''))
    return {k: over.get(k, v) for k, v in DEFAULTS.items()}
```

dlwp-cs_amd/build.py:

```python
#!/usr/bin/env python3
import os
import subprocess
import sys
from concurrent.futures import ThreadPoolExecutor

HERE = os.path.dirname(os.path.abspath(__file__))
CSRC = os.path.join(HERE, 'csrc')
TAG = os.environ.get('DLWPCS_LIB_TAG', '')
OBJ = os.path.join(HERE, 'build' + ('_' + TAG if TAG else ''))
LIBDIR = os.path.join(HERE, 'lib')
LIB = os.path.join(LIBDIR, 'libdlwpcs%s.so' % ('_' + TAG if TAG else ''))
SOURCES = ['halo_table.cpp', 'prof.cpp', 'comm.cpp', 'elementwise.hip', 'conv_mfma.hip', 'conv_inst_f32.hip', 'conv_inst_bf16.hip', 'conv_inst_edge.hip', 'conv_small.hip',
           'conv_generic.hip', 'wgrad_batch.hip', 'verify.hip', 'remap.hip', 'climatology.hip', 'solar.hip', 'scaling.hip', 'overlap.hip', 'packed.hip',
           'bilinear.hip', 'missing.hip', 'spectrum.hip', 'masked_loss.hip', 'ensemble.hip']
HIPCC = os.environ.get('HIPCC', '/opt/rocm/bin/hipcc')
ARCH = 'gfx950'
CFLAGS = ['-O3', '-std=c++17', '-fPIC', '--offload-arch=' + ARCH, '-x', 'hip', '-Wall', '-Wno-unused-function'] + \
    os.environ.get('DLWPCS_EXTRA_CFLAGS', '').split()


def _torch_lib_dir():
    try:
        import torch
        d = os.path.join(os.path.dirname(torch.__file__), 'lib')
        if os.path.exists(os.path.join(d, 'libamdhip64.so')):
            return d
    except Exception:
        pass
    return None


def _newer(src, dst, extra=()):
    if not os.path.exists(dst):
        return True
    t = os.path.getmtime(dst)
    return any((not os.path.exists(s)) or os.path.getmtime(s) > t for s in (src,) + tuple(extra))


def _deps(obj, fallback):
    d = os.path.splitext(obj)[0] + '.d'
    if not os.path.exists(d):
        return fallback
    try:
        words = open(d).read().replace('\\\n', ' ').split()
    except OSError:
        return fallback
    own = os.path.dirname(HERE)
    return tuple(w for w in words[1:] if w.endswith('.h') and os.path.abspath(w).startswith(own))


def build(force=False, verbose=True):
    os.makedirs(OBJ, exist_ok=True)
    os.makedirs(LIBDIR, exist_ok=True)
    headers = tuple(os.path.join(CSRC, h) for h in os.listdir(CSRC) if h.endswith('.h')) + \
        (os.path.join(HERE, '..', 'include', 'dlwpcs.h'),)
    jobs = []
    objs = []
    for src in SOURCES:
        s = os.path.join(CSRC, src)
        o = os.path.join(OBJ, os.path.splitext(src)[0] + '.o')
        objs.append(o)
        if force or _newer(s, o, _deps(o, headers)):
            jobs.append([HIPCC] + CFLAGS + ['-MD', '-MF', os.path.splitext(o)[0] + '.d', '-c', s, '-o', o])

    def run(cmd):
        if verbose:
            print(' '.join(cmd), flush=True)
        r = subprocess.run(cmd, capture_output=True, text=True)
        if r.returncode != 0:
            raise RuntimeError('hipcc failed:\n%s\n%s' % (' '.join(cmd), r.stderr[-8000:]))
        if verbose and r.stderr.strip():
            print(r.stderr[-4000:])

    with ThreadPoolExecutor(max_workers=8) as ex:
        list(ex.map(run, jobs))
    if jobs or force or not os.path.exists(LIB):
        link = ['g++', '-shared', '-fPIC', '-o', LIB] + objs
        tl = _torch_lib_dir()
        if tl:
            link += ['-L' + tl]
        link += ['-L/opt/rocm/lib', '-lamdhip64', '-ldl', '-Wl,-rpath,/opt/rocm/lib', '-Wl,--no-undefined']
        run(link)
    return LIB


if __name__ == '__main__':
    print(build(force='--force' in sys.argv))
```

dlwp-cs_amd/csrc/conv_mfma.hip:

```cpp
#include <stdlib.h>
#include <type_traits>
#include "common.h"
#include "mfma_common.h"
#include "conv_ws.h"
#include "conv_launch.h"

namespace dlwpcs {

template <typename T>
__device__ __forceinline__ void pack_weights_range(const float *__restrict__ w_eq, const float *__restrict__ w_pol,
                                                   const float *__restrict__ w_np, T *__restrict__ out,
                                                   int KS, int Cin, int Cout, int K, int Ncol, int CG, int NTtot,
                                                   int flip, int transposed, size_t total, size_t first, size_t stride) {
    constexpr int J = 16 / (int)sizeof(T);
    const int TAPS = KS * KS;
    const size_t entries = total / J;
    for (size_t e = first; e < entries; e += stride) {
        unsigned r = (unsigned)e;
        const int n = r % 32; r /= 32;
        const int hf = r % 2; r /= 2;
        const int tap = r % TAPS; r /= TAPS;
        const int cg = r % CG; r /= CG;
        const int nt = r % NTtot; r /= NTtot;
        const int v = (int)r;
// ... 1039 lines not shown
                    }
                    if (kvalid) {
                        a0 = *reinterpret_cast<const uint4 *>(wblane + v * kgroups * 256);
                        a1 = *reinterpret_cast<const uint4 *>(wblane + v * kgroups * 256 + 128);
                    }
                }
#pragma unroll
                for (int t = 0; t < MT; ++t) {
                    const f32x4 d = __builtin_amdgcn_mfma_f32_16x16x32_bf16(__builtin_bit_cast(bf16x8, a[t]), __builtin_bit_cast(bf16x8, xv[u]),
                                                                            b[t], 0, 0, 0);
                    const int co0 = t * 16 + q * 4, sidx = (n * Cout + co0) >> 1;
                    const uint32_t y01 = f2bf2(d[0], d[1]), y23 = f2bf2(d[2], d[3]);
                    const float e0 = bf_lo(y01) - tv[u][t][0].x, e1 = bf_hi(y01) - tv[u][t][0].y;
                    const float e2 = bf_lo(y23) - tv[u][t][1].x, e3 = bf_hi(y23) - tv[u][t][1].y;
                    if (co0 + 2 <= Cout) {
                        const float g0 = loss_elem<LK, W>(e0, tw[u], H.gscale, sq, ab);
                        const float g1 = loss_elem<LK, W>(e1, tw[u], H.gscale, sq, ab);
                        stage[sidx] = f2bf2(g0, g1);
                    }
                    if (co0 + 4 <= Cout) {
                        const float g2 = loss_elem<LK, W>(e2, tw[u], H.gscale, sq, ab);
                        const float g3 = loss_elem<LK, W>(e3, tw[u], H.gscale, sq, ab);
                        stage[sidx + 1] = f2bf2(g2, g3);
                    }
                }
                __builtin_amdgcn_wave_barrier();
                if (wr16) *reinterpret_cast<uint4 *>(dst + (unsigned)r.g * (unsigned)(16 * Cout)) = reinterpret_cast<const uint4 *>(stage)[lane];
                uint4 bv = make_uint4(0, 0, 0, 0);
                if (k1) bv.x = frag[0];
                if (k2) bv.y = frag[1];
                if (k3) bv.z = frag[2];
                if (k4) bv.w = frag[3];
                __builtin_amdgcn_wave_barrier();
                const f32x4 d0 = __builtin_amdgcn_mfma_f32_16x16x32_bf16(__builtin_bit_cast(bf16x8, a0), __builtin_bit_cast(bf16x8, bv),
                                                                         (f32x4)0.f, 0, 0, 0);
                const f32x4 d1 = __builtin_amdgcn_mfma_f32_16x16x32_bf16(__builtin_bit_cast(bf16x8, a1), __builtin_bit_cast(bf16x8, bv),
                                                                         (f32x4)0.f, 0, 0, 0);
                bf16_t *o_ptr = dxl + (unsigned)r.g * 512u;
                uint2 o;
                o.x = f2bf2(d0[0], d0[1]); o.y = f2bf2(d0[2], d0[3]);
                if (H.mask_dx) { o.x = bmask2(o.x, xm[u][0].x, H.m_alpha, H.m_vmax); o.y = bmask2(o.y, xm[u][0].y, H.m_alpha, H.m_vmax); }
                *reinterpret_cast<uint2 *>(o_ptr) = o;
                o.x = f2bf2(d1[0], d1[1]); o.y = f2bf2(d1[2], d1[3]);
                if (H.mask_dx) { o.x = bmask2(o.x, xm[u][1].x, H.m_alpha, H.m_vmax); o.y = bmask2(o.y, xm[u][1].y, H.m_alpha, H.m_vmax); }
                *reinterpret_cast<uint2 *>(o_ptr + 16) = o;
                pw_next(r, gpf);
            }
        }
    }
    __shared__ float s_sq[256], s_ab[256];
    s_sq[threadIdx.x] = sq; s_ab[threadIdx.x] = ab;
    __syncthreads();
    for (int st = 128; st > 0; st >>= 1) {
        if ((int)threadIdx.x < st) { s_sq[threadIdx.x] += s_sq[threadIdx.x + st]; s_ab[threadIdx.x] += s_ab[threadIdx.x + st]; }
        __syncthreads();
    }
    if (threadIdx.x == 0) { H.partial[2 * blockIdx.x] = s_sq[0]; H.partial[2 * blockIdx.x + 1] = s_ab[0]; }
}

template <int MT>
__global__ void __launch_bounds__(256) pw_head_train_kernel(HeadParams H) { pw_head_train_body<MT, DLWPCS_LOSS_MSE, false>(H, nullptr, 0u); }
template <int MT, int LK, bool W>
__global__ void __launch_bounds__(256) pw_head_loss_kernel(HeadParams H, const float *wfield, uint32_t wper) {
    pw_head_train_body<MT, LK, W>(H, wfield, wper);
}

__global__ void __launch_bounds__(256) head_stage2_kernel(const float *__restrict__ partial, float *__restrict__ loss_out,
                                                          int nblocks, float inv_n, float weight, int overwrite) {
    loss_stage2_body(partial, loss_out, nblocks, inv_n, weight, overwrite);
}

static bool pw_applies(const dlwpcs_conv_desc *d) {
    return d->dtype == DLWPCS_BF16 && d->ksize == 1 && !d->halo && !d->up0 && d->C1 == 0 && d->C0 == 32 && d->Cout % 2 == 0 &&
           d->Cout >= 8 && d->Cout <= 32 && ((long)d->N * d->N) % 16 == 0 && d->B > 0 &&
           (long)d->B * 6 * d->N * d->N * 32 < (1l << 31);
}
static unsigned pw_grid(long ngroups) {
    long blocks = (ngroups + 4 * PW_U - 1) / (4 * PW_U);
    return (unsigned)(blocks > 2048 ? 2048 : blocks);
}

static inline int cin_logical(const dlwpcs_conv_desc *d);

thread_local ConvEdgeArgs g_edge_args{};

struct WgradBf16Name { static const char *str() { return "wgrad_bf16_kernel"; } };
struct WgradMfmaName { static const char *str() { return "wgrad_mfma_kernel"; } };
struct PwHeadName { static const char *str() { return "pw_head_train_kernel"; } };
struct PwFwdName { static const char *str() { return "pw_fwd_kernel"; } };
static const int g_plain_tags[] = {prof_register_tag("pw_dgrad_kernel<false>"), prof_register_tag("pw_dgrad_kernel<true>"),
                                   prof_register_tag("wgrad_reduce_batch_kernel")};

static int dispatch_conv(int dtype, int KS, int vw, const ConvKParams &P, const Work &W, hipStream_t s) {
    if (KS == 3 && P.mode == MODE_HALO && P.edge) {
        if (dtype == DLWPCS_BF16 && vw == 8) return dispatch_conv_edge(P, W, s);
        return fail(DLWPCS_E_UNSUPPORTED, "conv: gather-form data gradient serves bf16 with 16-B channel vectors");
    }
    return dtype == DLWPCS_BF16 ? dispatch_conv_bf16(KS, vw, P, W, s) : dispatch_conv_f32(KS, vw, P, W, s);
}

static inline int vec_width(int c0, int c1, int dtype) {
    if (dtype == DLWPCS_BF16 && c0 % 8 == 0 && c1 % 8 == 0) return 8;
    if (c0 % 4 == 0 && c1 % 4 == 0) return 4;
    if (c0 % 2 == 0 && c1 % 2 == 0) return 2;
    return 1;
}
static inline int cgw_of(int dtype) { return dtype == DLWPCS_BF16 ? 16 : 8; }

static Work conv_work(const dlwpcs_conv_desc *d) {
    const double No = d->halo ? d->N : d->N - d->ksize + 1;
    const double Cin = cin_logical(d), taps = (double)d->ksize * d->ksize;
    const double n0 = d->up0 ? d->N / 2 : d->N;
    Work w;
    w.flops = 2.0 * d->B * 6 * No * No * taps * Cin * d->Cout;
    w.bytes = (double)dtype_size(d->dtype) * d->B * 6.0 * (n0 * n0 * d->C0 + (double)d->N * d->N * d->C1 + No * No * d->Cout) +
              4.0 * 2.0 * taps * Cin * d->Cout;
    return w;
}

struct Geometry {
    int Cin, CinP8, CG, NT_f, CoutP, NT_b, CGb, No, TAPS;
};

static int validate(const dlwpcs_conv_desc *d, const char *who) {
    if (!d) return fail(DLWPCS_E_INVALID, "%s: null descriptor", who);
    if (!dtype_ok(d->dtype)) return fail(DLWPCS_E_UNSUPPORTED, "%s: dtype %d not built", who, d->dtype);
    if (d->ksize != 1 && d->ksize != 3) return fail(DLWPCS_E_UNSUPPORTED, "%s: kernel size %d (MFMA path serves 1 and 3)", who, d->ksize);
    if (d->B < 0 || d->N < 1 || d->C0 < 1 || d->C1 < 0 || d->Cout < 1) return fail(DLWPCS_E_INVALID, "%s: bad shape B=%d N=%d C0=%d C1=%d Cout=%d", who, d->B, d->N, d->C0, d->C1, d->Cout);
    if (d->up0 && (d->N % 2)) return fail(DLWPCS_E_INVALID, "%s: up0 needs even N", who);
    if (d->halo && d->ksize == 1) return fail(DLWPCS_E_INVALID, "%s: halo with a 1x1 kernel", who);
    if (!d->halo && d->N < d->ksize) return fail(DLWPCS_E_INVALID, "%s: N < kernel size", who);
    if (d->act != DLWPCS_ACT_NONE && d->act != DLWPCS_ACT_LEAKY_CLIP) return fail(DLWPCS_E_INVALID, "%s: unknown activation %d", who, d->act);
    if (d->act == DLWPCS_ACT_LEAKY_CLIP && (!(d->alpha >= 0.f) || !(d->vmax >= 0.f)))
        return fail(DLWPCS_E_INVALID, "%s: activation needs negative_slope >= 0 and max_value >= 0, got %g / %g", who, d->alpha, d->vmax);
    if (d->N > 1024) return fail(DLWPCS_E_UNSUPPORTED, "%s: N > 1024", who);
    if (d->c0_valid != 0) {
        if (d->c0_valid < 1 || d->c0_valid > d->C0) return fail(DLWPCS_E_INVALID, "%s: c0_valid %d outside [1, C0 = %d]", who, d->c0_valid, d->C0);
        if (d->C1 != 0) return fail(DLWPCS_E_INVALID, "%s: c0_valid needs a single source (C1 = 0)", who);
        if (ceil_div(d->c0_valid, 32) != ceil_div(d->C0, 32))
            return fail(DLWPCS_E_INVALID, "%s: c0_valid %d and C0 %d must share their last 32-channel tile", who, d->c0_valid, d->C0);
    }
    return DLWPCS_OK;
}

static inline int out_size(const dlwpcs_conv_desc *d) { return d->halo ? d->N : d->N - d->ksize + 1; }
static inline int cin_logical(const dlwpcs_conv_desc *d) { return (d->c0_valid > 0 ? d->c0_valid : d->C0) + d->C1; }

bool conv_small_serves(int B, int N, int Cin, int Cout);
int launch_conv_small(const ConvKParams &K, hipStream_t s);
static bool conv_small_layer_ok(const dlwpcs_conv_desc *d) {
    return d->dtype == DLWPCS_BF16 && d->ksize == 3 && d->halo && d->C1 == 0 && !d->up0 && d->c0_valid == 0 &&
           !(d->flags & DLWPCS_CONV_OUT_PADDED) && conv_small_serves(d->B, d->N, d->C0, d->Cout);
}

struct WsLayout {
    size_t wpk_f, bias, wpk_b, dxv, dz, partial, bpartial, total;
    int n_eq, n_4, n_5, wg_pix, wg_nblk;
};

static bool wgrad_bf16_eligible(const dlwpcs_conv_desc *d) {
    const bool dz_ok = d->Cout % 8 == 0 || (d->ksize == 1 && d->Cout % 2 == 0 && d->Cout <= 16);
    if (d->Cout % 8 != 0 && (d->C0 % 8 != 0 || d->C1 % 8 != 0)) return false;
    return d->dtype == DLWPCS_BF16 && d->C0 % 2 == 0 && d->C1 % 2 == 0 && dz_ok;
}
static void wgrad_bf16_xcfg(const dlwpcs_conv_desc *d, int &xv, int &qx, int &cap_px, int &ct) {
    ct = 1;
    if (d->C0 % 8 == 0 && d->C1 % 8 == 0) {
        xv = 8; qx = 4; cap_px = 512;
        if ((d->C0 + d->C1) % 64 == 0 && d->Cout % 8 == 0) { ct = 2; cap_px = 320; }
    }
    else if (d->C0 + d->C1 <= 16) { xv = 2; qx = 8; cap_px = 512; }
    else { xv = 2; qx = 16; cap_px = 256; }
}

static bool dz_handover(const dlwpcs_conv_desc *d);

static void wgrad_tiling(const dlwpcs_conv_desc *d, int &pix, int &nblk, int &n_eq, int &n_4, int &n_5) {
    const int No = out_size(d);
    const int face_pix = No * No;
    int CAP = 192;
    int ci_tile = 32;
    if (wgrad_bf16_eligible(d)) {
        int xv, qx, cap_px, ct;
        wgrad_bf16_xcfg(d, xv, qx, cap_px, ct);
        CAP = ct == 2 ? 192 : 384;
        ci_tile = 32 * ct;
        while (CAP > 96 && (long)(tile_rows_for(No <= CAP ? (CAP / No) * No : CAP, No) + d->ksize - 1) * (No + d->ksize - 1) > cap_px)
            CAP -= 96;
    }
    pix = CAP;
    if (No <= CAP) pix = (CAP / No) * No;
    if (pix > face_pix) pix = face_pix;
    nblk = ceil_div(face_pix, pix);
    const int CinP = ceil_div(d->C0 + d->C1, 32) * 32, CoutP = ceil_div(d->Cout, 32) * 32;
    const int pairs = ceil_div(CinP, ci_tile) * (CoutP / 32);
    int wpp = 256 / pairs;
    if (wpp < 3) wpp = 3;
    const long items_per_face = (long)(d->B > 0 ? d->B : 1) * nblk;
    if (wpp > 6 * items_per_face) wpp = (int)(6 * items_per_face);
    if (wpp < 3) wpp = 3;
    n_4 = (wpp + 3) / 6; if (n_4 < 1) n_4 = 1;
    n_5 = n_4;
    n_eq = wpp - n_4 - n_5; if (n_eq < 1) n_eq = 1;
}

static WsLayout ws_layout(const dlwpcs_conv_desc *d);
static bool wgrad_bf16_fits(const dlwpcs_conv_desc *d, const struct WsLayout &L);

static WsLayout ws_layout(const dlwpcs_conv_desc *d) {
    WsLayout L{};
    const int Cin = d->C0 + d->C1, TAPS = d->ksize * d->ksize;
    const int cgw = cgw_of(d->dtype);
    const int CGf = ceil_div(Cin, cgw), NTf = ceil_div(d->Cout, 32);
    const int CGb = ceil_div(d->Cout, cgw), NTb = ceil_div(Cin, 32);
    const int No = out_size(d);
    size_t off = 0;
    L.wpk_f = off; off += align_up((size_t)3 * NTf * CGf * TAPS * 256 * 4, 256);
    L.bias = off;  off += align_up((size_t)3 * NTf * 32 * 4, 256);
    L.wpk_b = off; off += align_up((size_t)3 * NTb * CGb * TAPS * 256 * 4, 256);
    const int Nv = d->halo ? d->N + d->ksize - 1 : d->N;
    L.dxv = off;   off += align_up((size_t)d->B * 6 * Nv * Nv * Cin * dtype_size(d->dtype), 256);
    L.dz = off;    off += align_up((size_t)d->B * 6 * No * No * d->Cout * dtype_size(d->dtype), 256);
    int pix, nblk;
    wgrad_tiling(d, pix, nblk, L.n_eq, L.n_4, L.n_5);
    L.wg_pix = pix; L.wg_nblk = nblk;
    const int nworkers = L.n_eq + L.n_4 + L.n_5;
    const int CinP = ceil_div(Cin, 32) * 32, CoutP = ceil_div(d->Cout, 32) * 32;
    L.partial = off;  off += align_up((size_t)nworkers * TAPS * CinP * CoutP * 4, 256);
    L.bpartial = off; off += align_up((size_t)nworkers * CoutP * 4, 256);
    (void)No;
    L.total = off;
    return L;
}

static bool wgrad_bf16_fits(const dlwpcs_conv_desc *d, const WsLayout &L) {
    if (!wgrad_bf16_eligible(d)) return false;
    int xv, qx, cap_px, ct;
    wgrad_bf16_xcfg(d, xv, qx, cap_px, ct);
    const int No = out_size(d), KS = d->ksize;
    const long tile_px = (long)(tile_rows_for(L.wg_pix, No) + KS - 1) * (No + KS - 1);
    return tile_px <= cap_px && L.wg_pix <= 384;
}
static bool dz_handover(const dlwpcs_conv_desc *d) {
    if (!(d->flags & DLWPCS_CONV_REUSE_DZ) || d->act == DLWPCS_ACT_NONE || d->B == 0) return false;
    if (d->dtype == DLWPCS_F32) return d->Cout % 4 == 0;
    return wgrad_bf16_fits(d, ws_layout(d));
}

static void launch_pack(const void *w_eq, const void *w_pol, const void *w_np, void *out, int KS, int Cin, int Cout,
                        int transposed, int flip, int dtype, hipStream_t s) {
    const int K = transposed ? Cout : Cin, Ncol = transposed ? Cin : Cout;
    const int CG = ceil_div(K, cgw_of(dtype)), NTtot = ceil_div(Ncol, 32);
    const size_t total = (size_t)3 * NTtot * CG * KS * KS * 64 * (16 / dtype_size(dtype));
    size_t g = (total + 255) / 256;
    if (g > 1024) g = 1024;
    if (dtype == DLWPCS_BF16)
        hipLaunchKernelGGL(pack_weights_kernel<bf16_t>, dim3((unsigned)g), dim3(256), 0, s, (const float *)w_eq,
                           (const float *)w_pol, (const float *)w_np, (bf16_t *)out, KS, Cin, Cout, K, Ncol, CG, NTtot, flip,
                           transposed, total);
    else
        hipLaunchKernelGGL(pack_weights_kernel<float>, dim3((unsigned)g), dim3(256), 0, s, (const float *)w_eq,
                           (const float *)w_pol, (const float *)w_np, (float *)out, KS, Cin, Cout, K, Ncol, CG, NTtot, flip,
                           transposed, total);
}

}

using namespace dlwpcs;

extern "C" size_t dlwpcs_conv_workspace_bytes(const dlwpcs_conv_desc *d) {
    if (validate(d, "conv_workspace_bytes") != DLWPCS_OK) return 0;
    return ws_layout(d).total;
}

extern "C" size_t dlwpcs_conv_packed_bytes(const dlwpcs_conv_desc *d, int which) {
    if (validate(d, "conv_packed_bytes") != DLWPCS_OK) return 0;
    const WsLayout L = ws_layout(d);
    if (which == DLWPCS_PACK_FWD) return L.bias - L.wpk_f;
    if (which == DLWPCS_PACK_BIAS) return L.wpk_b - L.bias;
    if (which == DLWPCS_PACK_BWD) return L.dxv - L.wpk_b;
    fail(DLWPCS_E_INVALID, "conv_packed_bytes: which = %d", which);
    return 0;
}

extern "C" int dlwpcs_pack_batch(const dlwpcs_pack_item *items_dev, int n_items, dlwpcs_stream_t stream) {
    if (n_items < 0 || (n_items > 0 && !items_dev)) return fail(DLWPCS_E_INVALID, "pack_batch: bad arguments");
    if (n_items == 0) return DLWPCS_OK;
    if (n_items > 65535) return fail(DLWPCS_E_UNSUPPORTED, "pack_batch: more than 65535 items");
    const int gx = 96;
    hipLaunchKernelGGL(pack_batch_kernel, dim3((unsigned)gx, (unsigned)n_items), dim3(256), 0, (hipStream_t)stream, items_dev);
    return check_launch("pack_batch");
}

extern "C" int dlwpcs_head_mse_tail(const dlwpcs_conv_desc *d, float weight, int overwrite, void *scratch, float *loss_out,
                                    dlwpcs_loss_tail *tail) {
    if (!d || !scratch || !loss_out || !tail) return fail(DLWPCS_E_INVALID, "head_mse_tail: null pointer");
    if (!pw_applies(d)) return fail(DLWPCS_E_UNSUPPORTED, "head_mse_tail: not a layer dlwpcs_head_mse_step serves");
    const double n = (double)d->B * 6 * d->N * d->N * d->Cout;
    tail->partial = (const float *)scratch; tail->loss_out = loss_out;
    tail->nblocks = (int)pw_grid((long)d->B * 6 * d->N * d->N / 16);
    tail->inv_n = (float)(1.0 / n); tail->weight = weight; tail->overwrite = overwrite & 1;
    return DLWPCS_OK;
}
extern "C" int dlwpcs_loss_tail_run(const dlwpcs_loss_tail *tail, dlwpcs_stream_t stream) {
    if (!tail || !tail->partial || !tail->loss_out || tail->nblocks < 1) return fail(DLWPCS_E_INVALID, "loss_tail_run: bad tail");
    hipLaunchKernelGGL(head_stage2_kernel, dim3(1), dim3(256), 0, (hipStream_t)stream, tail->partial, tail->loss_out, tail->nblocks,
                       tail->inv_n, tail->weight, tail->overwrite);
    return check_launch("loss_tail_run");
}

extern "C" size_t dlwpcs_head_mse_scratch_bytes(void) { return (size_t)2048 * 2 * sizeof(float); }

static int head_loss_impl(const dlwpcs_conv_desc *d, const dlwpcs_loss_desc *L, const void *x, const void *wpk_fwd,
                          const void *bias_pk, const void *wpk_bwd, const float *target, void *dy, void *dx, float *loss_out,
                          void *scratch, int mask_dx, float m_alpha, float m_vmax, dlwpcs_stream_t stream);

static int head_mse_impl(const dlwpcs_conv_desc *d, const void *x, const void *wpk_fwd, const void *bias_pk,
                         const void *wpk_bwd, const float *target, float weight, void *dy, void *dx,
                         float *loss_out, int overwrite, void *scratch, int mask_dx, float m_alpha, float m_vmax,
                         dlwpcs_stream_t stream) {
    dlwpcs_loss_desc L{};
    L.kind = DLWPCS_LOSS_MSE;
    L.loss_weight = weight;
    L.overwrite = overwrite;
    return head_loss_impl(d, &L, x, wpk_fwd, bias_pk, wpk_bwd, target, dy, dx, loss_out, scratch, mask_dx, m_alpha, m_vmax, stream);
}

extern "C" int dlwpcs_head_mse_step(const dlwpcs_conv_desc *d, const void *x, const void *wpk_fwd, const void *bias_pk,
                                    const void *wpk_bwd, const float *target, float weight, void *dy, void *dx,
                                    float *loss_out, int overwrite, void *scratch, dlwpcs_stream_t stream) {
    return head_mse_impl(d, x, wpk_fwd, bias_pk, wpk_bwd, target, weight, dy, dx, loss_out, overwrite, scratch, 0, 0.f, 0.f, stream);
}

extern "C" int dlwpcs_head_mse_step_masked(const dlwpcs_conv_desc *d, const void *x, const void *wpk_fwd, const void *bias_pk,
                                           const void *wpk_bwd, const float *target, float weight, void *dy, void *dx,
                                           float *loss_out, int overwrite, void *scratch, float m_alpha, float m_vmax,
                                           dlwpcs_stream_t stream) {
    if (!(m_alpha >= 0.f) || !(m_vmax >= 0.f))
        return fail(DLWPCS_E_INVALID, "head_mse_step_masked: activation needs negative_slope >= 0 and max_value >= 0");
    return head_mse_impl(d, x, wpk_fwd, bias_pk, wpk_bwd, target, weight, dy, dx, loss_out, overwrite, scratch, 1, m_alpha, m_vmax, stream);
}

extern "C" int dlwpcs_head_loss_step(const dlwpcs_conv_desc *d, const dlwpcs_loss_desc *L, const void *x, const void *wpk_fwd,
                                     const void *bias_pk, const void *wpk_bwd, const float *target, void *dy, void *dx,
                                     float *loss_out, void *scratch, int mask_dx, float m_alpha, float m_vmax,
                                     dlwpcs_stream_t stream) {
    if (!L) return fail(DLWPCS_E_INVALID, "head_loss_step: null loss descriptor");
    if (mask_dx && (!(m_alpha >= 0.f) || !(m_vmax >= 0.f)))
        return fail(DLWPCS_E_INVALID, "head_loss_step: activation needs negative_slope >= 0 and max_value >= 0");
    return head_loss_impl(d, L, x, wpk_fwd, bias_pk, wpk_bwd, target, dy, dx, loss_out, scratch, mask_dx ? 1 : 0, m_alpha, m_vmax,
                          stream);
}

template <int LK, bool W>
static void head_launch(int Cout, unsigned grid, hipStream_t s, const HeadParams &H, const float *wfield, uint32_t wper) {
    if constexpr (LK == DLWPCS_LOSS_MSE && !W) {
        if (Cout <= 16) hipLaunchKernelGGL((pw_head_train_kernel<1>), dim3(grid), dim3(256), 0, s, H);
        else hipLaunchKernelGGL((pw_head_train_kernel<2>), dim3(grid), dim3(256), 0, s, H);
    } else {
        if (Cout <= 16) hipLaunchKernelGGL((pw_head_loss_kernel<1, LK, W>), dim3(grid), dim3(256), 0, s, H, wfield, wper);
        else hipLaunchKernelGGL((pw_head_loss_kernel<2, LK, W>), dim3(grid), dim3(256), 0, s, H, wfield, wper);
    }
}
static int head_loss_impl(const dlwpcs_conv_desc *d, const dlwpcs_loss_desc *L, const void *x, const void *wpk_fwd,
                          const void *bias_pk, const void *wpk_bwd, const float *target, void *dy, void *dx, float *loss_out,
                          void *scratch, int mask_dx, float m_alpha, float m_vmax, dlwpcs_stream_t stream) {
    int rc = validate(d, "head_mse_step");
    if (rc) return rc;
    if (!x || !wpk_fwd || !wpk_bwd || !target || !dy || !dx || !loss_out || !scratch)
        return fail(DLWPCS_E_INVALID, "head_mse_step: null pointer");
    if (!pw_applies(d) || d->act != DLWPCS_ACT_NONE || d->c0_valid != 0)
        return fail(DLWPCS_E_UNSUPPORTED, "head_mse_step: serves the bf16 pointwise head (k = 1, 32 input channels, even C_out in "
                                         "8..32, no activation)");
    if (L->kind != DLWPCS_LOSS_MSE && L->kind != DLWPCS_LOSS_MAE)
        return fail(DLWPCS_E_UNSUPPORTED, "head_loss_step: serves 'mse' and 'mae' (kind %d)", L->kind);
    const long cells = 6L * d->N * d->N;
    if (L->clim || (L->weight && (L->weight_div != d->Cout || L->weight_period != cells)))
        return fail(DLWPCS_E_UNSUPPORTED, "head_loss_step: takes a per-cell weight field only (div = C_out, period = 6*N*N)");
    const int overwrite = L->overwrite;
    const float weight = L->loss_weight;
    hipStream_t s = (hipStream_t)stream;
    HeadParams H{};
    H.f.in = (const bf16_t *)x; H.f.wpk = (const bf16_t *)wpk_fwd; H.f.bias = (const float *)bias_pk; H.f.out = (bf16_t *)dy;
    H.f.ngroups = (long)d->B * 6 * d->N * d->N / 16; H.f.groups_per_face = d->N * d->N / 16; H.f.Cout = d->Cout;
    H.wpk_bwd = (const bf16_t *)wpk_bwd; H.target = target; H.dx = (bf16_t *)dx; H.partial = (float *)scratch;
    const double n = (double)d->B * 6 * d->N * d->N * d->Cout;
    H.gscale = (float)(weight * (L->kind == DLWPCS_LOSS_MSE ? 2.0 : 1.0) / n);
    H.mask_dx = mask_dx; H.m_alpha = m_alpha; H.m_vmax = mask_vmax_for(d->dtype, m_vmax);
    const unsigned grid = pw_grid(H.f.ngroups);
    const bool W = L->weight != nullptr, mae = L->kind == DLWPCS_LOSS_MAE;
    int pidx = -1;
    if (prof_enabled() && !mae && !W) {
        Work wk = conv_work(d);
        wk.flops *= 2.0;
        wk.bytes = (double)d->B * 6 * d->N * d->N * (2.0 * 32 * 2 + d->Cout * (4.0 + 2.0));
        pidx = prof_begin(d->Cout <= 16 ? KTag<PwHeadName, void, 1>::tag() : KTag<PwHeadName, void, 2>::tag(), wk.flops, wk.bytes, s);
    }
    const uint32_t wper = (uint32_t)cells;
    if (!mae && !W) head_launch<DLWPCS_LOSS_MSE, false>(d->Cout, grid, s, H, L->weight, wper);
    else if (!mae) head_launch<DLWPCS_LOSS_MSE, true>(d->Cout, grid, s, H, L->weight, wper);
    else if (!W) head_launch<DLWPCS_LOSS_MAE, false>(d->Cout, grid, s, H, L->weight, wper);
    else head_launch<DLWPCS_LOSS_MAE, true>(d->Cout, grid, s, H, L->weight, wper);
    if (pidx >= 0) prof_end(pidx, s);
    if (!(overwrite & DLWPCS_HEAD_DEFER_STAGE2))
        hipLaunchKernelGGL(head_stage2_kernel, dim3(1), dim3(256), 0, s, (const float *)scratch, loss_out, (int)grid,
                           (float)(1.0 / n), weight, overwrite & 1);
    return check_launch("head_mse_step");
}

struct ConvHeadArgs { const void *wpk; const float *bias; void *out; int *done; };
static int conv_fwd_impl(const dlwpcs_conv_desc *d, const void *src0, const void *src1,
                         const void *w_eq, const void *w_pol, const void *w_np,
                         const void *b_eq, const void *b_pol, const void *b_np,
                         void *y, const int32_t *table_dev,
                         void *workspace, size_t workspace_bytes, dlwpcs_stream_t stream, void *y_pooled, int *pool_done,
                         const ConvHeadArgs *head = nullptr, bool small = false);

extern "C" int dlwpcs_conv_fwd(const dlwpcs_conv_desc *d, const void *src0, const void *src1,
                               const void *w_eq, const void *w_pol, const void *w_np,
                               const void *b_eq, const void *b_pol, const void *b_np,
                               void *y, const int32_t *table_dev,
                               void *workspace, size_t workspace_bytes, dlwpcs_stream_t stream) {
    return conv_fwd_impl(d, src0, src1, w_eq, w_pol, w_np, b_eq, b_pol, b_np, y, table_dev, workspace, workspace_bytes, stream,
                         nullptr, nullptr);
}

extern "C" int dlwpcs_avgpool2_fwd(const void *x, void *y, int B, int N, int C, int dtype, dlwpcs_stream_t stream);

extern "C" int dlwpcs_conv_fwd_pool(const dlwpcs_conv_desc *d, const void *src0, const void *src1,
                                    const void *w_eq, const void *w_pol, const void *w_np,
                                    const void *b_eq, const void *b_pol, const void *b_np,
                                    void *y, void *y_pooled, const int32_t *table_dev,
                                    void *workspace, size_t workspace_bytes, dlwpcs_stream_t stream) {
    if (!y_pooled) return fail(DLWPCS_E_INVALID, "conv_fwd_pool: null pointer");
    if (!d || !d->halo || d->N % 2) return fail(DLWPCS_E_INVALID, "conv_fwd_pool: needs a halo convolution on an even face size");
    int done = 0;
    int rc = conv_fwd_impl(d, src0, src1, w_eq, w_pol, w_np, b_eq, b_pol, b_np, y, table_dev, workspace, workspace_bytes, stream,
                           y_pooled, &done);
    if (rc || done || d->B == 0) return rc;
    return dlwpcs_avgpool2_fwd(y, y_pooled, d->B, d->N, d->Cout, d->dtype, stream);
}

extern "C" int dlwpcs_conv_fwd_head(const dlwpcs_conv_desc *d, const void *src0, const void *src1, const void *wpk_fwd,
                                    const void *bias_pk, const dlwpcs_conv_desc *dh, const void *head_wpk_fwd,
                                    const void *head_bias_pk, void *y, void *y_head, const int32_t *table_dev,
                                    void *workspace, size_t workspace_bytes, int *fused, dlwpcs_stream_t stream) {
    if (fused) *fused = 0;
    int rc = validate(d, "conv_fwd_head");
    if (rc) return rc;
    rc = validate(dh, "conv_fwd_head (head)");
    if (rc) return rc;
    if (!wpk_fwd || !head_wpk_fwd || !y || !y_head) return fail(DLWPCS_E_INVALID, "conv_fwd_head: null pointer");
    if (!(d->flags & DLWPCS_CONV_PREPACKED) || !(dh->flags & DLWPCS_CONV_PREPACKED))
        return fail(DLWPCS_E_INVALID, "conv_fwd_head: both layers take dlwpcs_pack_batch operands (DLWPCS_CONV_PREPACKED)");
    const int No = out_size(d);
    if (dh->B != d->B || dh->N != No || dh->C0 != d->Cout || dh->dtype != d->dtype)
        return fail(DLWPCS_E_INVALID, "conv_fwd_head: the head (B=%d N=%d C_in=%d) does not consume the layer's output (B=%d N=%d C=%d)",
                    dh->B, dh->N, dh->C0, d->B, No, d->Cout);
    if (d->flags & DLWPCS_CONV_OUT_PADDED) return fail(DLWPCS_E_INVALID, "conv_fwd_head: DLWPCS_CONV_OUT_PADDED belongs to the head's descriptor");
    if (d->B == 0) return DLWPCS_OK;
    const int head_rows = (dh->flags & DLWPCS_CONV_OUT_PADDED) ? (dh->Cout + 7) / 8 * 8 : dh->Cout;
    const bool can = pw_applies(dh) && dh->act == DLWPCS_ACT_NONE && dh->c0_valid == 0 && head_rows == 32 && d->Cout == 32 &&
                     d->dtype == DLWPCS_BF16 && d->ksize == 3;
    int done = 0;
    ConvHeadArgs H{head_wpk_fwd, (const float *)head_bias_pk, y_head, &done};
    rc = conv_fwd_impl(d, src0, src1, wpk_fwd, nullptr, nullptr, bias_pk, nullptr, nullptr, y, table_dev, workspace, workspace_bytes,
                       stream, nullptr, nullptr, can ? &H : nullptr);
    if (rc) return rc;
    if (done) { if (fused) *fused = 1; return DLWPCS_OK; }
    return conv_fwd_impl(dh, y, nullptr, head_wpk_fwd, nullptr, nullptr, head_bias_pk, nullptr, nullptr, y_head, nullptr, workspace,
                         workspace_bytes, stream, nullptr, nullptr);
}

static int conv_fwd_impl(const dlwpcs_conv_desc *d, const void *src0, const void *src1,
                         const void *w_eq, const void *w_pol, const void *w_np,
                         const void *b_eq, const void *b_pol, const void *b_np,
                         void *y, const int32_t *table_dev,
                         void *workspace, size_t workspace_bytes, dlwpcs_stream_t stream, void *y_pooled, int *pool_done,
                         const ConvHeadArgs *head, bool small) {
    int rc = validate(d, "conv_fwd");
    if (rc) return rc;
    if (small && !conv_small_layer_ok(d))
        return fail(DLWPCS_E_UNSUPPORTED, "conv_small_fwd: serves bf16 3x3 halo layers with one source on faces of <= 320 cells, channel counts multiples of 32");
    if (!src0 || !w_eq || (!w_pol && !(d->flags & DLWPCS_CONV_PREPACKED)) || !y || !workspace)
        return fail(DLWPCS_E_INVALID, "conv_fwd: null pointer");
    if (d->C1 > 0 && !src1) return fail(DLWPCS_E_INVALID, "conv_fwd: C1 > 0 but src1 is null");
    if (d->halo && !table_dev) return fail(DLWPCS_E_INVALID, "conv_fwd: halo requested without table");
    const bool prepacked = (d->flags & DLWPCS_CONV_PREPACKED) != 0;
    if (!prepacked && (b_eq == nullptr) != (b_pol == nullptr)) return fail(DLWPCS_E_INVALID, "conv_fwd: b_eq and b_pol must both be given or both be null");
    const WsLayout L = ws_layout(d);
    if (workspace_bytes < L.total) return fail(DLWPCS_E_WORKSPACE, "conv_fwd: workspace %zu < %zu bytes", workspace_bytes, L.total);
    if (d->B == 0) return DLWPCS_OK;
    hipStream_t s = (hipStream_t)stream;
    char *ws = (char *)workspace;
    const int Cin = d->C0 + d->C1;
    const void *wpk = prepacked ? w_eq : ws + L.wpk_f;
    const float *bpk = prepacked ? (const float *)b_eq : (const float *)(ws + L.bias);
    if (!prepacked) launch_pack(w_eq, w_pol, w_np, ws + L.wpk_f, d->ksize, cin_logical(d), d->Cout, 0, d->flip_north_pole, d->dtype, s);
    const int NTtot = ceil_div(d->Cout, 32);
    if (b_eq && !prepacked) {
        const int n = 3 * NTtot * 32;
        hipLaunchKernelGGL(pack_bias_kernel, dim3(ceil_div(n, 256)), dim3(256), 0, s, (const float *)b_eq,
                           (const float *)b_pol, (const float *)b_np, (float *)(ws + L.bias), d->Cout, NTtot * 32);
    }
    ConvKParams P{};
    P.src0 = src0; P.src1 = src1; P.ymask = nullptr;
    P.wpk = wpk; P.bias = b_eq ? bpk : nullptr; P.out = y; P.table = table_dev;
    P.B = d->B; P.Nin = d->N; P.No = out_size(d);
    P.C0 = d->C0; P.C1 = d->C1; P.Cin = Cin; P.Cout = d->Cout;
    P.CG = ceil_div(Cin, cgw_of(d->dtype)); P.NTtot = NTtot; P.up0 = d->up0;
    P.mode = d->halo ? MODE_HALO : MODE_DIRECT;
    P.act = d->act; P.alpha = d->alpha; P.vmax = d->vmax;
    P.pool_out = y_pooled; P.pool_done = pool_done;
    if (head) { P.head_w = head->wpk; P.head_b = head->bias; P.head_out = head->out; P.head_done = head->done; }
    if ((d->flags & DLWPCS_CONV_OUT_PADDED) && !pw_applies(d))
        return fail(DLWPCS_E_UNSUPPORTED, "conv_fwd: DLWPCS_CONV_OUT_PADDED serves the bf16 pointwise output layer only");
    if (small) return launch_conv_small(P, s);
    if (pw_applies(d)) {
        PwParams Q{};
        Q.in = (const bf16_t *)src0; Q.wpk = (const bf16_t *)wpk; Q.bias = b_eq ? bpk : nullptr; Q.out = (bf16_t *)y;
        Q.ngroups = (long)d->B * 6 * d->N * d->N / 16; Q.groups_per_face = d->N * d->N / 16; Q.Cout = d->Cout;
        if (d->flags & DLWPCS_CONV_OUT_PADDED) Q.Cout = (d->Cout + 7) / 8 * 8;
        Q.alpha = d->alpha; Q.vmax = d->vmax;
        int pidx = -1;
        const bool actv = d->act != DLWPCS_ACT_NONE;
        if (prof_enabled()) {
            const Work wk = conv_work(d);
            const char *tag = Q.Cout <= 16 ? (actv ? KTag<PwFwdName, void, true, 1>::tag() : KTag<PwFwdName, void, false, 1>::tag())
                                           : (actv ? KTag<PwFwdName, void, true, 2>::tag() : KTag<PwFwdName, void, false, 2>::tag());
            pidx = prof_begin(tag, wk.flops, wk.bytes, s);
        }
        const dim3 pgrid(pw_grid(Q.ngroups));
        if (Q.Cout <= 16) {
            if (actv) hipLaunchKernelGGL((pw_fwd_kernel<true, 1>), pgrid, dim3(256), 0, s, Q);
            else hipLaunchKernelGGL((pw_fwd_kernel<false, 1>), pgrid, dim3(256), 0, s, Q);
        } else {
            if (actv) hipLaunchKernelGGL((pw_fwd_kernel<true, 2>), pgrid, dim3(256), 0, s, Q);
            else hipLaunchKernelGGL((pw_fwd_kernel<false, 2>), pgrid, dim3(256), 0, s, Q);
        }
        if (pidx >= 0) prof_end(pidx, s);
        return check_launch("pw_fwd");
    }
    if (d->dtype == DLWPCS_BF16 && d->ksize == 3 && d->halo && d->C1 == 0 && d->C0 >= 8 && d->C0 % 2 == 0 && d->C0 % 8 != 0 &&
        NTtot <= 2) {
        return dispatch_conv_tail8(d->C0 <= 16 ? 16 : 32, NTtot, P, conv_work(d), s);
    }
    return dispatch_conv(d->dtype, d->ksize, vec_width(d->C0, d->C1, d->dtype), P, conv_work(d), s);
}

static int conv_bwd_data_impl(const dlwpcs_conv_desc *d, const void *dy, const void *y, bool dz_given,
                              const void *w_eq, const void *w_pol, const void *w_np,
                              void *dsrc0, void *dsrc1, const void *m0, const void *m1, float m_alpha, float m_vmax,
                              const int32_t *inv_table_dev, void *workspace, size_t workspace_bytes, dlwpcs_stream_t stream,
                              const char *who, int *ring_query = nullptr, bool small = false) {
    int rc = validate(d, who);
    if (rc) return rc;
    if (small && (!conv_small_layer_ok(d) || (d->act != DLWPCS_ACT_NONE && !dz_given) || dsrc1 || !dsrc0))
        return fail(DLWPCS_E_UNSUPPORTED, "%s: serves bf16 3x3 halo layers with one source on faces of <= 320 cells, channel counts multiples of 32, gradient given as dz", who);
    const bool prepacked = (d->flags & DLWPCS_CONV_PREPACKED) != 0;
    if (!dy || !w_eq || (!w_pol && !prepacked) || !workspace) return fail(DLWPCS_E_INVALID, "%s: null pointer", who);
    const bool has_act = d->act != DLWPCS_ACT_NONE && !dz_given;
    if (has_act && !y) return fail(DLWPCS_E_INVALID, "%s: activation needs the saved output y", who);
    if (d->halo && !inv_table_dev) return fail(DLWPCS_E_INVALID, "%s: halo requested without inverse table", who);
    if ((m0 || m1) && (!(m_alpha >= 0.f) || !(m_vmax >= 0.f)))
        return fail(DLWPCS_E_INVALID, "%s: mask activation needs negative_slope >= 0 and max_value >= 0, got %g / %g", who, m_alpha, m_vmax);
    if (!dsrc0 && !dsrc1) return DLWPCS_OK;
    if (!dsrc0) m0 = nullptr;
    if (!dsrc1 || d->C1 == 0) m1 = nullptr;
    const WsLayout L = ws_layout(d);
    if (workspace_bytes < L.total) return fail(DLWPCS_E_WORKSPACE, "%s: workspace %zu < %zu bytes", who, workspace_bytes, L.total);
    if (d->B == 0) return DLWPCS_OK;
    hipStream_t s = (hipStream_t)stream;
    char *ws = (char *)workspace;
    const int Cin = d->C0 + d->C1;
    const void *wpk = prepacked ? w_eq : ws + L.wpk_b;
    void *dxv = ws + L.dxv;
    if (!prepacked) launch_pack(w_eq, w_pol, w_np, ws + L.wpk_b, d->ksize, cin_logical(d), d->Cout, 1, d->flip_north_pole, d->dtype, s);
    const int No = out_size(d);
    const int n0 = d->up0 ? d->N / 2 : d->N;
    const size_t n_src0 = (size_t)d->B * 6 * n0 * n0 * d->C0, n_src1 = (size_t)d->B * 6 * d->N * d->N * d->C1;
    auto finish_masks = [&](bool todo0, bool todo1) -> int {
        int r = DLWPCS_OK;
        if (todo0 && m0) r = launch_mask_inplace(dsrc0, m0, n_src0, m_alpha, m_vmax, d->dtype, s);
        if (!r && todo1 && m1) r = launch_mask_inplace(dsrc1, m1, n_src1, m_alpha, m_vmax, d->dtype, s);
        return r;
    };
    if (pw_applies(d) && !has_act && dsrc0) {
        PwParams Q{};
        Q.in = (const bf16_t *)dy; Q.wpk = (const bf16_t *)wpk; Q.bias = nullptr; Q.out = (bf16_t *)dsrc0;
        Q.ngroups = (long)d->B * 6 * d->N * d->N / 16; Q.groups_per_face = d->N * d->N / 16; Q.Cout = d->Cout;
        int pidx = -1;
        const bool in_kernel_mask = m0 != nullptr;
        if (prof_enabled()) {
            const Work wk = conv_work(d);
            pidx = prof_begin(in_kernel_mask ? "pw_dgrad_kernel<true>" : "pw_dgrad_kernel<false>", wk.flops, wk.bytes, s);
        }
        Q.mask = (const bf16_t *)m0; Q.m_alpha = m_alpha; Q.m_vmax = mask_vmax_for(d->dtype, m_vmax);
        if (in_kernel_mask) hipLaunchKernelGGL(pw_dgrad_kernel<true>, dim3(pw_grid(Q.ngroups)), dim3(256), 0, s, Q);
        else hipLaunchKernelGGL(pw_dgrad_kernel<false>, dim3(pw_grid(Q.ngroups)), dim3(256), 0, s, Q);
        if (pidx >= 0) prof_end(pidx, s);
        rc = check_launch("pw_dgrad");
        return rc ? rc : finish_masks(!in_kernel_mask, false);
    }
    ConvKParams P{};
    const bool dz_ready = !dz_given && dz_handover(d);
    P.src0 = dz_ready ? (const void *)(ws + L.dz) : dy; P.src1 = nullptr;
    P.ymask = (has_act && !dz_ready) ? y : nullptr;
    P.wpk = wpk; P.bias = nullptr; P.out = dxv; P.table = nullptr;
    P.B = d->B; P.Nin = No; P.No = No + d->ksize - 1;
    P.C0 = d->Cout; P.C1 = 0; P.Cin = d->Cout; P.Cout = Cin;
    P.CG = ceil_div(d->Cout, cgw_of(d->dtype)); P.NTtot = ceil_div(Cin, 32); P.up0 = 0;
    P.mode = MODE_ZERO;
    P.act = DLWPCS_ACT_NONE; P.alpha = d->alpha; P.vmax = mask_vmax_for(d->dtype, d->vmax);
    int direct_done = 0, mask_done = 0;
    const bool can_direct = d->halo && d->ksize == 3;
    P.d0 = (can_direct && dsrc0 && !d->up0) ? dsrc0 : nullptr;
    P.d1 = (can_direct && dsrc1 && d->C1 > 0) ? dsrc1 : nullptr;
    P.dsplit = d->C0;
    P.direct_done = &direct_done;
    P.m0 = P.d0 ? m0 : nullptr; P.m1 = P.d1 ? m1 : nullptr;
    P.m_alpha = m_alpha; P.m_vmax = mask_vmax_for(d->dtype, m_vmax); P.m_thr1 = bf16_mask_threshold(m_vmax);
    P.mask_done = &mask_done;
    if ((d->flags & DLWPCS_CONV_DGRAD_GATHER) && d->halo && d->ksize == 3 && d->dtype == DLWPCS_BF16 && !P.ymask && d->N >= 8 &&
        vec_width(d->Cout, 0, d->dtype) == 8 && d->C0 % 8 == 0 && d->C1 % 8 == 0) {
        ConvKParams G = P;
        const int M = d->N + 2;
        const int32_t *plan = inv_table_dev + (size_t)6 * d->N * d->N * 4 + DGG_HEADER;
        G.table = plan; G.edge = 1;
        G.mode = MODE_HALO; G.Nin = d->N; G.No = d->N;
        ConvEdgeArgs EA{};
        EA.src = plan + (size_t)6 * M * M;
        int32_t wids[36];
        int grc = dgrad_gather_wids(d->N, wids);
        for (int k = 0; k < 36; ++k) EA.wids[k] = (int8_t)wids[k];
        g_edge_args = EA;
        G.d0 = (dsrc0 && !d->up0) ? dsrc0 : nullptr;
        G.d1 = (dsrc1 && d->C1 > 0) ? dsrc1 : nullptr;
        G.m0 = G.d0 ? m0 : nullptr; G.m1 = G.d1 ? m1 : nullptr;
        int g_usum = 0;
        G.pool_out = (dsrc0 && d->up0) ? dsrc0 : nullptr; G.pool_mask = G.pool_out ? m0 : nullptr; G.pool_done = &g_usum;
        int g_direct = 0, g_mask = 0;
        G.direct_done = &g_direct; G.mask_done = &g_mask;
        G.dry_run = 1;
        const bool need_direct = G.d0 || G.d1;
        if (!grc) grc = dispatch_conv(d->dtype, d->ksize, 8, G, conv_work(d), s);
        if (!grc && (g_direct || !need_direct)) {
            if (small) return fail(DLWPCS_E_UNSUPPORTED, "%s: this shape is served in gather form", who);
            if (ring_query) { *ring_query = 0; return DLWPCS_OK; }
            G.dry_run = 0;
            grc = dispatch_conv(d->dtype, d->ksize, 8, G, conv_work(d), s);
            if (grc) return grc;
            bool todo0 = m0 != nullptr && !(G.d0 && (g_mask & 1)) && !g_usum, todo1 = m1 != nullptr && !(G.d1 && (g_mask & 2));
            if (dsrc0 && !G.d0 && !g_usum) {
                int masked = 0;
                grc = launch_src_grad(dxv, dsrc0, nullptr, d->B, d->N, Cin, 0, d->C0, d->up0, 0, d->dtype, s, m0, m_alpha, m_vmax, &masked);
                if (grc) return grc;
                if (masked) todo0 = false;
            }
            if (dsrc1 && d->C1 > 0 && !G.d1) {
                int masked = 0;
                grc = launch_src_grad(dxv, dsrc1, nullptr, d->B, d->N, Cin, d->C0, d->C1, 0, 0, d->dtype, s, m1, m_alpha, m_vmax, &masked);
                if (grc) return grc;
                if (masked) todo1 = false;
            }
            return finish_masks(todo0, todo1);
        }
    }
    const bool whole = !d->halo && !d->up0 && d->C1 == 0 && dsrc0;
    if (whole) P.out = dsrc0;
    P.dry_run = ring_query ? 1 : 0;
    rc = small ? launch_conv_small(P, s) : dispatch_conv(d->dtype, d->ksize, vec_width(d->Cout, 0, d->dtype), P, conv_work(d), s);
    if (ring_query) { *ring_query = (!rc && direct_done && P.d0 && !m0) ? 1 : 0; return rc; }
    if (rc) return rc;
    if (whole) return finish_masks(true, false);
    bool todo0 = m0 != nullptr, todo1 = m1 != nullptr;
    const bool direct0 = direct_done && P.d0, direct1 = direct_done && P.d1;
    const void *rm0 = (direct0 && !(mask_done & 1)) ? nullptr : m0;
    const void *rm1 = (direct1 && !(mask_done & 2)) ? nullptr : m1;
    if (dsrc0 && dsrc1 && d->C1 > 0 && d->halo && direct_done && !P.d0 && P.d1) {
        rc = launch_src_pair(dxv, dsrc0, dsrc1, inv_table_dev, d->B, d->N, d->C0, d->C1, d->up0, d->dtype, s, m0, rm1, m_alpha, m_vmax);
        if (rc) return rc;
        return finish_masks(false, todo1 && !rm1);
    }
    if (dsrc0) {
        if (direct0 && !m0 && (d->flags & DLWPCS_CONV_DEFER_RING0)) {
        } else if (direct0) {
            rc = launch_ring_fix(dxv, dsrc0, inv_table_dev, d->B, d->N, Cin, 0, d->C0, d->dtype, s, rm0, m_alpha, m_vmax);
            if (rm0) todo0 = false;
        } else {
            int masked = 0;
            rc = launch_src_grad(dxv, dsrc0, inv_table_dev, d->B, d->N, Cin, 0, d->C0, d->up0, d->halo, d->dtype, s, m0, m_alpha, m_vmax, &masked);
            if (masked) todo0 = false;
        }
        if (rc) return rc;
    }
    if (dsrc1 && d->C1 > 0) {
        if (direct1) {
            rc = launch_ring_fix(dxv, dsrc1, inv_table_dev, d->B, d->N, Cin, d->C0, d->C1, d->dtype, s, rm1, m_alpha, m_vmax);
            if (rm1) todo1 = false;
        } else {
            int masked = 0;
            rc = launch_src_grad(dxv, dsrc1, inv_table_dev, d->B, d->N, Cin, d->C0, d->C1, 0, d->halo, d->dtype, s, m1, m_alpha, m_vmax, &masked);
            if (masked) todo1 = false;
        }
        if (rc) return rc;
    }
    return finish_masks(todo0, todo1);
}

extern "C" int dlwpcs_conv_bwd_data(const dlwpcs_conv_desc *d, const void *dy, const void *y,
                                    const void *w_eq, const void *w_pol, const void *w_np,
                                    void *dsrc0, void *dsrc1, const int32_t *inv_table_dev,
                                    void *workspace, size_t workspace_bytes, dlwpcs_stream_t stream) {
    return conv_bwd_data_impl(d, dy, y, false, w_eq, w_pol, w_np, dsrc0, dsrc1, nullptr, nullptr, 0.f, 0.f, inv_table_dev, workspace,
                              workspace_bytes, stream, "conv_bwd_data");
}

extern "C" int dlwpcs_conv_bwd_data_masked(const dlwpcs_conv_desc *d, const void *dz,
                                           const void *w_eq, const void *w_pol, const void *w_np,
                                           void *dsrc0, void *dsrc1, const void *m0, const void *m1, float m_alpha, float m_vmax,
                                           const int32_t *inv_table_dev,
                                           void *workspace, size_t workspace_bytes, dlwpcs_stream_t stream) {
    return conv_bwd_data_impl(d, dz, nullptr, true, w_eq, w_pol, w_np, dsrc0, dsrc1, m0, m1, m_alpha, m_vmax, inv_table_dev, workspace,
                              workspace_bytes, stream, "conv_bwd_data_masked");
}

extern "C" int dlwpcs_conv_small_fwd(const dlwpcs_conv_desc *d, const void *src0, const void *src1,
                                     const void *w_eq, const void *w_pol, const void *w_np,
                                     const void *b_eq, const void *b_pol, const void *b_np,
                                     void *y, const int32_t *table_dev,
                                     void *workspace, size_t workspace_bytes, dlwpcs_stream_t stream) {
    return conv_fwd_impl(d, src0, src1, w_eq, w_pol, w_np, b_eq, b_pol, b_np, y, table_dev, workspace, workspace_bytes, stream,
                         nullptr, nullptr, nullptr, true);
}

extern "C" int dlwpcs_conv_small_bwd_data(const dlwpcs_conv_desc *d, const void *dz,
                                          const void *w_eq, const void *w_pol, const void *w_np,
                                          void *dsrc0, void *dsrc1, const void *m0, const void *m1, float m_alpha, float m_vmax,
                                          const int32_t *inv_table_dev,
                                          void *workspace, size_t workspace_bytes, dlwpcs_stream_t stream) {
    return conv_bwd_data_impl(d, dz, nullptr, true, w_eq, w_pol, w_np, dsrc0, dsrc1, m0, m1, m_alpha, m_vmax, inv_table_dev, workspace,
                              workspace_bytes, stream, "conv_small_bwd_data", nullptr, true);
}

extern "C" int dlwpcs_conv_ring_info(const dlwpcs_conv_desc *d, size_t *dxv_offset, int *channels) {
    if (validate(d, "conv_ring_info") != DLWPCS_OK || !dxv_offset || !channels) return 0;
    if (!d->halo || d->ksize != 3 || d->up0 || d->B < 1) return 0;
    const WsLayout L = ws_layout(d);
    int q = 0;
    char dummy = 0;
    dlwpcs_conv_desc dd = *d;
    dd.act = DLWPCS_ACT_NONE;
    dd.flags |= DLWPCS_CONV_PREPACKED;
    const int rc = conv_bwd_data_impl(&dd, &dummy, nullptr, true, &dummy, nullptr, nullptr, &dummy, d->C1 > 0 ? &dummy : nullptr, nullptr,
                                      nullptr, 0.f, 0.f, (const int32_t *)&dummy, &dummy, L.total, nullptr, "conv_ring_info", &q);
    if (rc || !q) return 0;
    *dxv_offset = L.dxv;
    *channels = d->C0 + d->C1;
    return 1;
}

extern "C" int dlwpcs_conv_bwd_weights(const dlwpcs_conv_desc *d, const void *src0, const void *src1, const void *dy,
                                       const void *y, void *dw_eq, void *dw_pol, void *dw_np,
                                       void *db_eq, void *db_pol, void *db_np, const int32_t *table_dev,
                                       void *workspace, size_t workspace_bytes, dlwpcs_stream_t stream) {
    int rc = validate(d, "conv_bwd_weights");
    if (rc) return rc;
    if (!src0 || !dy || !dw_eq || !dw_pol || !workspace) return fail(DLWPCS_E_INVALID, "conv_bwd_weights: null pointer");
    if (d->C1 > 0 && !src1) return fail(DLWPCS_E_INVALID, "conv_bwd_weights: C1 > 0 but src1 is null");
    if (d->act != DLWPCS_ACT_NONE && !y) return fail(DLWPCS_E_INVALID, "conv_bwd_weights: activation needs the saved output y");
    if (d->halo && !table_dev) return fail(DLWPCS_E_INVALID, "conv_bwd_weights: halo requested without table");
    if ((db_np != nullptr) != (dw_np != nullptr) && db_eq) return fail(DLWPCS_E_INVALID, "conv_bwd_weights: dw_np/db_np must match");
    const WsLayout L = ws_layout(d);
    if (workspace_bytes < L.total) return fail(DLWPCS_E_WORKSPACE, "conv_bwd_weights: workspace %zu < %zu bytes", workspace_bytes, L.total);
    hipStream_t s = (hipStream_t)stream;
    char *ws = (char *)workspace;
    const int Cin = d->C0 + d->C1, KS = d->ksize, TAPS = KS * KS;
    const int CinP = ceil_div(Cin, 32) * 32, CoutP = ceil_div(d->Cout, 32) * 32;
    if (d->B == 0 && (d->flags & DLWPCS_CONV_ACCUMULATE_WGRAD)) return DLWPCS_OK;
    if (d->B == 0) {
        const size_t wbytes = (size_t)TAPS * cin_logical(d) * d->Cout * 4;
        (void)hipMemsetAsync(dw_eq, 0, wbytes, s);
        (void)hipMemsetAsync(dw_pol, 0, wbytes, s);
        if (dw_np) (void)hipMemsetAsync(dw_np, 0, wbytes, s);
        if (db_eq) (void)hipMemsetAsync(db_eq, 0, (size_t)d->Cout * 4, s);
        if (db_pol) (void)hipMemsetAsync(db_pol, 0, (size_t)d->Cout * 4, s);
        if (db_np) (void)hipMemsetAsync(db_np, 0, (size_t)d->Cout * 4, s);
        return DLWPCS_OK;
    }
    WgradKParams W{};
    ConvKParams &P = W.c;
    P.src0 = src0; P.src1 = src1; P.ymask = nullptr; P.table = table_dev;
    P.B = d->B; P.Nin = d->N; P.No = out_size(d);
    P.C0 = d->C0; P.C1 = d->C1; P.Cin = Cin; P.Cout = d->Cout; P.up0 = d->up0;
    P.mode = d->halo ? MODE_HALO : MODE_DIRECT;
    P.alpha = d->alpha; P.vmax = mask_vmax_for(d->dtype, d->vmax);
    P.pix_per_block = L.wg_pix; P.nblk_face = L.wg_nblk;
    P.W2 = P.No + KS - 1; P.magicW2 = div_magic(P.W2); P.magicNo = div_magic(P.No);
    P.tile_rows_max = tile_rows_for(L.wg_pix, P.No) + (KS - 1);
    W.dy = dy; W.y = y;
    W.dz_out = dz_handover(d) ? ws + L.dz : nullptr;
    W.partial = (float *)(ws + L.partial);
    const bool want_bias = db_eq || db_pol || db_np;
    W.bpartial = want_bias ? (float *)(ws + L.bpartial) : nullptr;
    W.CinP = CinP; W.CoutP = CoutP;
    W.n_eq = L.n_eq; W.n_4 = L.n_4; W.n_5 = L.n_5;
    P.magicN = div_magic(P.Nin);
    P.tune = tune_bits();
    W.magicB = P.B > 1 ? div_magic(P.B) : 0; W.magicNb = P.nblk_face > 1 ? div_magic(P.nblk_face) : 0;
    if (P.C1 == 0) P.src1 = P.src0;
    const bool mask = d->act != DLWPCS_ACT_NONE;
    dim3 grid((unsigned)(L.n_eq + L.n_4 + L.n_5), (unsigned)(CinP / 32), (unsigned)(CoutP / 32));
    int xv = 0, qx = 0, cap_px = 0, ct = 1;
    if (wgrad_bf16_eligible(d)) wgrad_bf16_xcfg(d, xv, qx, cap_px, ct);
    if (wgrad_bf16_fits(d, L)) {
        const int pcap = (L.wg_pix + 15) & ~15;
        size_t lds = 2 * ((size_t)ct * P.tile_rows_max * P.W2 * 64 + (size_t)pcap * 64);
        grid.y = (unsigned)(CinP / (32 * ct));
        {
            const int nph = 4 / ct, rslots = TAPS - TAPS / nph;
            const size_t need = ((size_t)4 * rslots * 1024 + 2048) * 4;
            if (lds < need) lds = need;
        }
        if (lds > 160 * 1024) return fail(DLWPCS_E_UNSUPPORTED, "conv_bwd_weights: LDS tile of %zu bytes exceeds 160 KiB", lds);
        if ((long)P.Nin * P.Nin >= (1l << 16))
            return fail(DLWPCS_E_UNSUPPORTED, "conv_bwd_weights: face size %d too large for the 16-bit index arithmetic", P.Nin);
#define WGB_LAUNCH(KSV, MASKV, XVV, QXV, CTV, DVV)                                                                        \
    do {                                                                                                                  \
        auto kern = wgrad_bf16_kernel<KSV, MASKV, XVV, QXV, CTV, DVV>;                                                    \
        if (lds > 64 * 1024) {                                                                                            \
            hipError_t e = hipFuncSetAttribute((const void *)kern, hipFuncAttributeMaxDynamicSharedMemorySize, (int)lds); \
            if (e != hipSuccess) return fail(DLWPCS_E_LAUNCH, "wgrad: hipFuncSetAttribute: %s", hipGetErrorString(e));    \
        }                                                                                                                 \
        int pidx = -1;                                                                                                    \
        if (prof_enabled()) {                                                                                             \
            const Work wk = conv_work(d);                                                                                 \
            pidx = prof_begin(KTag<WgradBf16Name, void, KSV, MASKV, XVV, QXV, CTV, DVV>::tag(), wk.flops, wk.bytes, s);   \
        }                                                                                                                 \
        hipLaunchKernelGGL(kern, grid, dim3(512), lds, s, W);                                                             \
        if (pidx >= 0) prof_end(pidx, s);                                                                                 \
    } while (0)
#define WGB_X(KSV, MASKV)                                                                                                 \
    do {                                                                                                                  \
        if (xv == 8 && ct == 2) WGB_LAUNCH(KSV, MASKV, 8, 4, 2, 8);                                                       \
        else if (xv == 8) WGB_LAUNCH(KSV, MASKV, 8, 4, 1, 8);                                                             \
        else if (qx == 8) WGB_LAUNCH(KSV, MASKV, 2, 8, 1, 8);                                                             \
        else WGB_LAUNCH(KSV, MASKV, 2, 16, 1, 8);                                                                         \
    } while (0)
        if (d->Cout % 8 != 0) {
            if (xv != 8) return fail(DLWPCS_E_UNSUPPORTED, "conv_bwd_weights: even-only C_in and C_out together");
            if (mask) WGB_LAUNCH(1, true, 8, 4, 1, 2); else WGB_LAUNCH(1, false, 8, 4, 1, 2);
        }
        else if (KS == 3) { if (mask) WGB_X(3, true); else WGB_X(3, false); }
        else { if (mask) WGB_X(1, true); else WGB_X(1, false); }
#undef WGB_X
#undef WGB_LAUNCH
        rc = check_launch("wgrad_bf16");
        if (rc || (d->flags & DLWPCS_CONV_DEFER_REDUCE)) return rc;
        launch_wgrad_reduce(s, W.partial, W.bpartial, dw_eq, dw_pol, dw_np, db_eq, db_pol, db_np, KS, cin_logical(d), d->Cout, CinP, CoutP,
                            L.n_eq, L.n_4, L.n_5, d->flip_north_pole, (d->flags & DLWPCS_CONV_ACCUMULATE_WGRAD) ? 1 : 0, want_bias);
        return check_launch("wgrad_reduce");
    }
    const int pix_cap = (L.wg_pix + 1) & ~1;
    const int vw = vec_width(d->C0, d->C1, d->dtype);
    const bool bf = d->dtype == DLWPCS_BF16;
    const size_t bufb = ((size_t)P.tile_rows_max * P.W2 * 32 + (size_t)pix_cap * 32) * 4;
    if ((size_t)P.tile_rows_max * P.W2 > 448 || pix_cap > 192)
        return fail(DLWPCS_E_UNSUPPORTED, "conv_bwd_weights: tile of %d x %d pixels exceeds the producers' register capacity", P.tile_rows_max, P.W2);
    if ((long)P.Nin * P.Nin >= (1l << 16))
        return fail(DLWPCS_E_UNSUPPORTED, "conv_bwd_weights: face size %d too large for the 16-bit index arithmetic", P.Nin);
    size_t lds = 2 * bufb;
    if (lds < (WG_SCRATCH_FLOATS + 1024) * 4) lds = (WG_SCRATCH_FLOATS + 1024) * 4;
    if (lds > 160 * 1024) return fail(DLWPCS_E_UNSUPPORTED, "conv_bwd_weights: LDS tile of %zu bytes exceeds 160 KiB", lds);
#define WG_LAUNCH(TV, TS, KSV, VWV, MASKV)                                                                                \
    do {                                                                                                                  \
        auto kern = wgrad_mfma_kernel<TV, KSV, VWV, MASKV>;                                                               \
        if (lds > 64 * 1024) {                                                                                            \
            hipError_t e = hipFuncSetAttribute((const void *)kern, hipFuncAttributeMaxDynamicSharedMemorySize, (int)lds); \
            if (e != hipSuccess) return fail(DLWPCS_E_LAUNCH, "wgrad: hipFuncSetAttribute: %s", hipGetErrorString(e));    \
        }                                                                                                                 \
        int pidx = -1;                                                                                                    \
        if (prof_enabled()) {                                                                                             \
            const Work wk = conv_work(d);                                                                                 \
            pidx = prof_begin(KTag<WgradMfmaName, TV, KSV, VWV, MASKV>::tag(), wk.flops, wk.bytes, s);                    \
        }                                                                                                                 \
        hipLaunchKernelGGL(kern, grid, dim3(512), lds, s, W);                                                             \
// ... 85 lines not shown
```

include/dlwpcs.h:

```cpp
#ifndef DLWPCS_H
#define DLWPCS_H

#include <stddef.h>
#include <stdint.h>

#ifdef __cplusplus
extern "C" {
#endif

#define DLWPCS_VERSION 105

#define DLWPCS_OK             0
#define DLWPCS_E_INVALID     -1
#define DLWPCS_E_UNSUPPORTED -2
#define DLWPCS_E_WORKSPACE   -3
#define DLWPCS_E_LAUNCH      -4

#define DLWPCS_F32  0
#define DLWPCS_BF16 1

#define DLWPCS_ACT_NONE        0
#define DLWPCS_ACT_LEAKY_CLIP  1

typedef void *dlwpcs_stream_t;

int dlwpcs_version(void);
const char *dlwpcs_last_error(void);


int dlwpcs_halo_table(int N, int p, int32_t *out);

int dlwpcs_halo_inverse_table(int N, int p, int32_t *inv);

size_t dlwpcs_dgrad_gather_plan_ints(int N);
int dlwpcs_dgrad_gather_plan(int N, int32_t *out);

int dlwpcs_pad_fwd(const void *x, void *y, int B, int N, int C, int p, int dtype,
                   const int32_t *table_dev, dlwpcs_stream_t stream);
int dlwpcs_pad_bwd(const void *dy, void *dx, int B, int N, int C, int p, int dtype,
                   const int32_t *inv_table_dev, dlwpcs_stream_t stream);

#define DLWPCS_CONV_ACCUMULATE_WGRAD 1
#define DLWPCS_CONV_PREPACKED        2
#define DLWPCS_CONV_REUSE_DZ         4
#define DLWPCS_CONV_DEFER_RING0     16
#define DLWPCS_CONV_DGRAD_GATHER    64
#define DLWPCS_CONV_OUT_PADDED      32
#define DLWPCS_CONV_DEFER_REDUCE     8

typedef struct dlwpcs_conv_desc {
    int32_t B;
    int32_t N;
    int32_t C0, C1;
    int32_t Cout;
    int32_t ksize;
    int32_t halo;
    int32_t up0;
    int32_t flip_north_pole;
    int32_t act;
    float   alpha, vmax;
    int32_t dtype;
    int32_t flags;
    int32_t c0_valid;
} dlwpcs_conv_desc;

size_t dlwpcs_conv_workspace_bytes(const dlwpcs_conv_desc *d);

#define DLWPCS_PACK_FWD  0
#define DLWPCS_PACK_BWD  1
#define DLWPCS_PACK_BIAS 2
typedef struct dlwpcs_pack_item {
    const void *w_eq, *w_pol, *w_np;
    const void *b_eq, *b_pol, *b_np;
    void *wpk_fwd, *wpk_bwd, *bias_pk;
    int32_t ksize, Cin, Cout, flip_north_pole, dtype, reserved;
} dlwpcs_pack_item;
size_t dlwpcs_conv_packed_bytes(const dlwpcs_conv_desc *d, int which);
int dlwpcs_pack_batch(const dlwpcs_pack_item *items_dev, int n_items, dlwpcs_stream_t stream);

int dlwpcs_conv_fwd(const dlwpcs_conv_desc *d,
                    const void *src0, const void *src1,
                    const void *w_eq, const void *w_pol, const void *w_np,
                    const void *b_eq, const void *b_pol, const void *b_np,
                    void *y, const int32_t *table_dev,
                    void *workspace, size_t workspace_bytes, dlwpcs_stream_t stream);
int dlwpcs_conv_fwd_pool(const dlwpcs_conv_desc *d, const void *src0, const void *src1,
                         const void *w_eq, const void *w_pol, const void *w_np,
                         const void *b_eq, const void *b_pol, const void *b_np,
                         void *y, void *y_pooled, const int32_t *table_dev,
                         void *workspace, size_t workspace_bytes, dlwpcs_stream_t stream);
int dlwpcs_conv_fwd_head(const dlwpcs_conv_desc *d, const void *src0, const void *src1, const void *wpk_fwd,
                         const void *bias_pk, const dlwpcs_conv_desc *dh, const void *head_wpk_fwd,
                         const void *head_bias_pk, void *y, void *y_head, const int32_t *table_dev,
                         void *workspace, size_t workspace_bytes, int *fused, dlwpcs_stream_t stream);

int dlwpcs_conv_bwd_data(const dlwpcs_conv_desc *d,
                         const void *dy, const void *y,
                         const void *w_eq, const void *w_pol, const void *w_np,
                         void *dsrc0, void *dsrc1, const int32_t *inv_table_dev,
                         void *workspace, size_t workspace_bytes, dlwpcs_stream_t stream);

int dlwpcs_conv_bwd_data_masked(const dlwpcs_conv_desc *d, const void *dz,
                                const void *w_eq, const void *w_pol, const void *w_np,
                                void *dsrc0, void *dsrc1, const void *m0, const void *m1, float m_alpha, float m_vmax,
                                const int32_t *inv_table_dev,
                                void *workspace, size_t workspace_bytes, dlwpcs_stream_t stream);

int dlwpcs_conv_small_fwd(const dlwpcs_conv_desc *d,
                          const void *src0, const void *src1,
                          const void *w_eq, const void *w_pol, const void *w_np,
                          const void *b_eq, const void *b_pol, const void *b_np,
                          void *y, const int32_t *table_dev,
                          void *workspace, size_t workspace_bytes, dlwpcs_stream_t stream);
int dlwpcs_conv_small_bwd_data(const dlwpcs_conv_desc *d, const void *dz,
                               const void *w_eq, const void *w_pol, const void *w_np,
                               void *dsrc0, void *dsrc1, const void *m0, const void *m1, float m_alpha, float m_vmax,
                               const int32_t *inv_table_dev,
                               void *workspace, size_t workspace_bytes, dlwpcs_stream_t stream);

int dlwpcs_conv_ring_info(const dlwpcs_conv_desc *d, size_t *dxv_offset, int *channels);

int dlwpcs_conv_bwd_weights(const dlwpcs_conv_desc *d,
                            const void *src0, const void *src1, const void *dy, const void *y,
                            void *dw_eq, void *dw_pol, void *dw_np,
                            void *db_eq, void *db_pol, void *db_np,
                            const int32_t *table_dev,
                            void *workspace, size_t workspace_bytes, dlwpcs_stream_t stream);

typedef struct dlwpcs_reduce_item {
    const float *partial, *bpartial;
    float *dw_eq, *dw_pol, *dw_np, *db_eq, *db_pol, *db_np;
    int32_t ksize, Cin, Cout, CinP, CoutP, n_eq, n_4, n_5, flip_north_pole, accumulate, vec, nblocks;
    int32_t reserved[4];
} dlwpcs_reduce_item;
int dlwpcs_conv_wgrad_reduce_item(const dlwpcs_conv_desc *d,
                                  void *dw_eq, void *dw_pol, void *dw_np,
                                  void *db_eq, void *db_pol, void *db_np,
                                  void *workspace, size_t workspace_bytes, dlwpcs_reduce_item *item);
int dlwpcs_wgrad_reduce_batch(const dlwpcs_reduce_item *items_dev, const dlwpcs_reduce_item *items_host, int n_items,
                              dlwpcs_stream_t stream);

#define DLWPCS_WGRAD_BATCH_MAX 24
typedef struct dlwpcs_wgrad_item {
    dlwpcs_conv_desc d;
    const void *src0, *src1;
    const void *dz;
    const void *y;
    const int32_t *table_dev;
    void *dw_eq, *dw_pol, *dw_np;
    void *db_eq, *db_pol, *db_np;
} dlwpcs_wgrad_item;
int dlwpcs_wgrad_batch_supported(const dlwpcs_conv_desc *d);
int dlwpcs_wgrad_batch_sizes(const dlwpcs_wgrad_item *items, int n_items, size_t *plan_bytes, size_t *workspace_bytes);
int dlwpcs_wgrad_batch_plan(const dlwpcs_wgrad_item *items, int n_items, void *plan_host, size_t plan_bytes);
int dlwpcs_wgrad_batch(const dlwpcs_wgrad_item *items, int n_items, const void *plan_host, const void *plan_dev,
                       void *workspace, size_t workspace_bytes, dlwpcs_stream_t stream);
int dlwpcs_wgrad_batch_adam(const dlwpcs_wgrad_item *items, int n_items, const void *plan_host, const void *plan_dev,
                            void *workspace, size_t workspace_bytes, float *p, float *g, float *m, float *v, size_t n,
                            int32_t *state_dev, const float *hyper_dev, dlwpcs_stream_t stream);
struct dlwpcs_loss_tail;
int dlwpcs_wgrad_batch_adam_tail(const dlwpcs_wgrad_item *items, int n_items, const void *plan_host, const void *plan_dev,
                                 void *workspace, size_t workspace_bytes, float *p, float *g, float *m, float *v, size_t n,
                                 int32_t *state_dev, const float *hyper_dev, const struct dlwpcs_loss_tail *tail,
                                 const dlwpcs_pack_item *pack_items_host, dlwpcs_stream_t stream);

int dlwpcs_wgrad_batch_apply(const dlwpcs_wgrad_item *items, int n_items, const void *plan_host, const void *plan_dev,
                             float *p, float *g, float *m, float *v, size_t n, int32_t *state_dev, const float *hyper_dev,
                             const struct dlwpcs_loss_tail *tail, const dlwpcs_pack_item *pack_items_host, dlwpcs_stream_t stream);

typedef struct dlwpcs_gconv_desc {
    int32_t B, H, W, Cin, Cout;
    int32_t kh, kw, sh, sw, dh, dw;
    int32_t pad_t, pad_l;
    int32_t Ho, Wo;
    int32_t flip_north_pole;
    int32_t dtype;
} dlwpcs_gconv_desc;

int dlwpcs_gconv_fwd(const dlwpcs_gconv_desc *d, const void *x,
                     const void *w_eq, const void *w_pol, const void *w_np,
                     const void *b_eq, const void *b_pol, const void *b_np, void *y, dlwpcs_stream_t stream);
int dlwpcs_gconv_bwd_data(const dlwpcs_gconv_desc *d, const void *dy,
                          const void *w_eq, const void *w_pol, const void *w_np, void *dx, dlwpcs_stream_t stream);
int dlwpcs_gconv_bwd_weights(const dlwpcs_gconv_desc *d, const void *x, const void *dy,
                             void *dw_eq, void *dw_pol, void *dw_np, void *db_eq, void *db_pol, void *db_np,
                             dlwpcs_stream_t stream);

int dlwpcs_act_fwd(const void *x, void *y, size_t n, int act, float alpha, float vmax, int dtype,
                   dlwpcs_stream_t stream);
int dlwpcs_act_bwd(const void *dy, const void *y, void *dx, size_t n, int act, float alpha, float vmax, int dtype,
                   dlwpcs_stream_t stream);
int dlwpcs_avgpool2_fwd(const void *x, void *y, int B, int N, int C, int dtype, dlwpcs_stream_t stream);
int dlwpcs_avgpool2_bwd(const void *dy, void *dx, int B, int N, int C, int dtype, dlwpcs_stream_t stream);
int dlwpcs_avgpool2_bwd_add(const void *dy, const void *dskip, void *dx, int B, int N, int C, int dtype,
                            dlwpcs_stream_t stream);
int dlwpcs_avgpool2_bwd_masked(const void *dy, const void *dskip, const void *m, void *dx, int B, int N, int C,
                               float m_alpha, float m_vmax, int dtype, dlwpcs_stream_t stream);
int dlwpcs_avgpool2_bwd_ring(const void *dy, const void *dskip, const void *m, void *dx, int B, int N, int C,
                             float m_alpha, float m_vmax, int dtype, const void *ring, const int32_t *inv_half_dev,
                             int ring_channels, int ring_choff, dlwpcs_stream_t stream);
int dlwpcs_upsample2_fwd(const void *x, void *y, int B, int N, int C, int dtype, dlwpcs_stream_t stream);
int dlwpcs_upsample2_bwd(const void *dy, void *dx, int B, int N, int C, int dtype, dlwpcs_stream_t stream);
int dlwpcs_concat2(const void *a, const void *b, void *y, size_t rows, int Ca, int Cb, int dtype,
                   dlwpcs_stream_t stream);
int dlwpcs_split2(const void *y, void *a, void *b, size_t rows, int Ca, int Cb, int dtype, dlwpcs_stream_t stream);
int dlwpcs_pad_channels(const void *x, void *y, size_t rows, int C, int Cp, int dtype, dlwpcs_stream_t stream);
int dlwpcs_slice_channels(const void *y, void *x, size_t rows, int Cp, int C, int dtype, dlwpcs_stream_t stream);
int dlwpcs_state_repack(const void *state, const void *extra, void *out, int B, size_t S, int T, int V, int E,
                        int dtype, dlwpcs_stream_t stream);
int dlwpcs_cf_to_cl(const void *x, void *y, int B, int C, size_t S, int dtype, dlwpcs_stream_t stream);
int dlwpcs_cl_to_cf(const void *x, void *y, int B, int C, size_t S, int dtype, dlwpcs_stream_t stream);
int dlwpcs_add(const void *a, const void *b, void *y, size_t n, int dtype, dlwpcs_stream_t stream);

#define DLWPCS_MSE_TARGET_F32 0x100
#define DLWPCS_MSE_OVERWRITE  0x200
size_t dlwpcs_mse_scratch_bytes(void);
int dlwpcs_mse_fwd_bwd(const void *y, const void *t, void *dy, float *loss_out, size_t n, float weight, int dtype,
                       void *scratch, dlwpcs_stream_t stream);
size_t dlwpcs_head_mse_scratch_bytes(void);
#define DLWPCS_HEAD_DEFER_STAGE2 2
typedef struct dlwpcs_loss_tail {
    const float *partial;
    float *loss_out;
    int nblocks;
    float inv_n, weight;
    int overwrite;
} dlwpcs_loss_tail;
int dlwpcs_head_mse_tail(const dlwpcs_conv_desc *d, float weight, int overwrite, void *scratch, float *loss_out,
                         dlwpcs_loss_tail *tail);
int dlwpcs_loss_tail_run(const dlwpcs_loss_tail *tail, dlwpcs_stream_t stream);
int dlwpcs_head_mse_step(const dlwpcs_conv_desc *d, const void *x, const void *wpk_fwd, const void *bias_pk,
                         const void *wpk_bwd, const float *target, float weight, void *dy, void *dx, float *loss_out,
                         int overwrite, void *scratch, dlwpcs_stream_t stream);

int dlwpcs_head_mse_step_masked(const dlwpcs_conv_desc *d, const void *x, const void *wpk_fwd, const void *bias_pk,
                                const void *wpk_bwd, const float *target, float weight, void *dy, void *dx, float *loss_out,
                                int overwrite, void *scratch, float m_alpha, float m_vmax, dlwpcs_stream_t stream);

#define DLWPCS_LOSS_MSE 0
#define DLWPCS_LOSS_MAE 1
#define DLWPCS_LOSS_ACC 2
#define DLWPCS_REG_NONE   0
#define DLWPCS_REG_MSE    1
#define DLWPCS_REG_MAE    2
#define DLWPCS_REG_GLOBAL 3
typedef struct dlwpcs_loss_desc {
    int kind;
    float loss_weight;
    const float *weight;
    int weight_div, weight_period;
    const float *clim;
    int clim_div, clim_period;
    int regularize;
    int reverse;
    int overwrite;
} dlwpcs_loss_desc;
size_t dlwpcs_loss_scratch_bytes(void);
int dlwpcs_loss_fwd_bwd(const dlwpcs_loss_desc *L, const void *y, const void *t, void *dy, float *loss_out, size_t n,
                        int dtype, void *scratch, dlwpcs_stream_t stream);
#define DLWPCS_NORM_ALL   0
#define DLWPCS_NORM_VALID 1
int dlwpcs_loss_masked_fwd_bwd(const dlwpcs_loss_desc *L, const void *y, const void *t, int normalize,
                               void *dy, float *loss_out, uint32_t *valid_out, size_t n, int dtype,
                               void *scratch, dlwpcs_stream_t stream);
int dlwpcs_head_loss_step(const dlwpcs_conv_desc *d, const dlwpcs_loss_desc *L, const void *x, const void *wpk_fwd,
                          const void *bias_pk, const void *wpk_bwd, const float *target, void *dy, void *dx, float *loss_out,
                          void *scratch, int mask_dx, float m_alpha, float m_vmax, dlwpcs_stream_t stream);

#define DLWPCS_SCORE_MSE  0
#define DLWPCS_SCORE_RMSE 1
#define DLWPCS_SCORE_MAE  2
// ... 184 lines not shown
```

Measured before the change: 48690 samples/s.

## Add band-tiled LDS-staged forward conv kernel for mid-size cubed-sphere faces

Adds a new forward 3x3 halo convolution kernel that stages a band of face rows plus halo into LDS once through the halo table, then runs bf16 MFMA across 9 taps with double-buffered weight registers. It is enabled by default but only for layers whose (N, Cin, Cout) is (24, 64, 32). Other layers fall back to the generic path. The aim is better input reuse and less redundant gathering on that layer, at the cost of a large LDS footprint, which limits occupancy, and an extra code path.

```diff
diff --git a/dlwp-cs_amd/DLWP/_native.py b/dlwp-cs_amd/DLWP/_native.py
--- a/dlwp-cs_amd/DLWP/_native.py
+++ b/dlwp-cs_amd/DLWP/_native.py
@@ -170,6 +170,9 @@
                                                                                        c_void_p]),
     'dlwpcs_conv_small_bwd_data': (c_int, [ctypes.POINTER(ConvDesc)] + [c_void_p] * 4 + [c_void_p] * 4 + [c_float, c_float] +
                                    [c_void_p, c_void_p, c_size_t, c_void_p]),
+    'dlwpcs_conv_band_fwd': (c_int, [ctypes.POINTER(ConvDesc)] + [c_void_p] * 8 + [c_void_p, c_void_p, c_void_p, c_size_t,
+                                                                                      c_void_p]),
+    'dlwpcs_conv_band_tune': (c_int, [c_int]),
     'dlwpcs_conv_bwd_weights': (c_int, [ctypes.POINTER(ConvDesc)] + [c_void_p] * 4 + [c_void_p] * 6 +
                                 [c_void_p, c_void_p, c_size_t, c_void_p]),
     'dlwpcs_conv_wgrad_reduce_item': (c_int, [ctypes.POINTER(ConvDesc)] + [c_void_p] * 6 +
diff --git a/dlwp-cs_amd/DLWP/custom.py b/dlwp-cs_amd/DLWP/custom.py
--- a/dlwp-cs_amd/DLWP/custom.py
+++ b/dlwp-cs_amd/DLWP/custom.py
@@ -203,13 +203,14 @@
         return (self._is_mfma_config() and self.kernel_size[0] == 3 and pad_width == 1 and self.activation is None)
 
     def fused_call(self, src0, src1=None, up0=False, halo=True, act=ACT_NONE, alpha=0.0, vmax=0.0, premask0=None,
-                   premask1=None, dy_premasked=False, defer_ring0=False, want_pool=False, out_padded=False, small=False):
+                   premask1=None, dy_premasked=False, defer_ring0=False, want_pool=False, out_padded=False, small=False,
+                   band=False):
         return ops.cs_conv(src0, self.equatorial_kernel, self.polar_kernel, self.north_pole_kernel,
                            self.equatorial_bias, self.polar_bias, self.north_pole_bias, src1=src1,
                            ksize=self.kernel_size[0], halo=halo, up0=up0, flip_north_pole=self.flip_north_pole,
                            act=act, alpha=alpha, vmax=vmax, premask0=premask0, premask1=premask1,
                            dy_premasked=dy_premasked, defer_ring0=defer_ring0, want_pool=want_pool, out_padded=out_padded,
-                           small=small)
+                           small=small, band=band)
 
     def call(self, inputs, channels_last_io=False, **kwargs):
         channels_first = self.data_format == 'channels_first' and not channels_last_io
diff --git a/dlwp-cs_amd/DLWP/keras/models.py b/dlwp-cs_amd/DLWP/keras/models.py
--- a/dlwp-cs_amd/DLWP/keras/models.py
+++ b/dlwp-cs_amd/DLWP/keras/models.py
@@ -65,6 +65,7 @@
         self.fuse_head_loss = option('fuse_head')
         self.fold_head = option('fold_head')
         self.small_conv = option('small_conv')
+        self.band_conv = option('band_conv')
         self.static_batch_buffers = False
         self._ones = {}
         self._compiled = False
@@ -390,7 +391,7 @@
                                                  dy_premasked=out_uid in pm,
                                                  defer_ring0=bool(pm) and self.fold_ring and i in self._defer_ring,
                                                  want_pool=self.fuse_pool and i in self._pool_producers,
-                                                 small=self.small_conv)
+                                                 small=self.small_conv, band=self.band_conv)
             elif st[0] == 'pool_skip':
                 _, out_uid, lay, in_uid = st
                 values[out_uid], values[in_uid] = ops.avgpool2_skip(values[in_uid],
diff --git a/dlwp-cs_amd/DLWP/ops.py b/dlwp-cs_amd/DLWP/ops.py
--- a/dlwp-cs_amd/DLWP/ops.py
+++ b/dlwp-cs_amd/DLWP/ops.py
@@ -433,7 +433,7 @@
     @staticmethod
     def forward(ctx, src0, src1, w_eq, w_pol, w_np, b_eq, b_pol, b_np, ksize, halo, up0, flip, act, alpha, vmax,
                 c0_valid=0, premask0=None, premask1=None, dy_premasked=False, defer_ring0=False, want_pool=False,
-                out_padded=False, small=False):
+                out_padded=False, small=False, band=False):
         require_device(src0, 'cs_conv')
         src0 = _c(src0)
         B = src0.shape[0]
@@ -481,6 +481,7 @@
         if packed is not None:
             d.flags |= nat.CONV_PREPACKED
         small = bool(small) and _small_conv_ok(d)
+        band = bool(band) and _band_conv_ok(d)
         if yp is not None:
             check(lib().dlwpcs_conv_fwd_pool(ctypes.byref(d), ptr(src0), ptr(src1), *wargs, ptr(y), ptr(yp), ptr(table), ptr(ws),
                                              ws.numel(), stream_ptr()), 'dlwpcs_conv_fwd_pool')
@@ -490,6 +491,9 @@
             if small:
                 rc = lib().dlwpcs_conv_small_fwd(ctypes.byref(d), ptr(src0), ptr(src1), *wargs, ptr(y), ptr(table), ptr(ws),
                                                  ws.numel(), stream_ptr())
+            elif band:
+                rc = lib().dlwpcs_conv_band_fwd(ctypes.byref(d), ptr(src0), ptr(src1), *wargs, ptr(y), ptr(table), ptr(ws),
+                                                ws.numel(), stream_ptr())
             if rc == nat.E_UNSUPPORTED:
                 rc = lib().dlwpcs_conv_fwd(ctypes.byref(d), ptr(src0), ptr(src1), *wargs, ptr(y), ptr(table), ptr(ws),
                                            ws.numel(), stream_ptr())
@@ -566,7 +570,7 @@
                     dn.flags &= ~nat.CONV_DEFER_RING0
             dw_eq, dw_pol, dw_np, db_eq, db_pol, db_np = _weight_gradients(
                 dn, src0, src1, dz, None, ctx.params, table, ws, nbytes, direct, defer, need[2:8], has_np, has_bias, has_bnp)
-            return (dsrc0, dsrc1, dw_eq, dw_pol, dw_np, db_eq, db_pol, db_np) + (None,) * 15
+            return (dsrc0, dsrc1, dw_eq, dw_pol, dw_np, db_eq, db_pol, db_np) + (None,) * 16
         no_dgrad = dsrc0 is None and dsrc1 is None
         mask_on_load = d.ksize == 3 and (no_dgrad or d.dtype == nat.F32)
         batching = (direct and WGRAD_BATCH and d.B > 0 and not WGRAD_SIDE_STREAM and wgrad_batch_supported(d)
@@ -593,7 +597,16 @@
             batch_mask_ok=mask_on_load)
         if reuse_dz:
             run_bwd_data()
-        return (dsrc0, dsrc1, dw_eq, dw_pol, dw_np, db_eq, db_pol, db_np) + (None,) * 15
+        return (dsrc0, dsrc1, dw_eq, dw_pol, dw_np, db_eq, db_pol, db_np) + (None,) * 16
+
+
+_BAND_WINS = {(24, 64, 32)}
+
+
+def _band_conv_ok(d):
+    return (d.dtype == nat.BF16 and d.ksize == 3 and d.halo and d.C1 == 0 and not d.up0 and d.c0_valid == 0
+            and d.N * d.N > 320 and d.C0 % 32 == 0 and d.Cout % 32 == 0 and d.B > 0
+            and (_BAND_WINS is None or (d.N, d.C0, d.Cout) in _BAND_WINS))
 
 
 def _small_conv_ok(d):
@@ -652,7 +665,7 @@
 
 def cs_conv(src0, w_eq, w_pol, w_np=None, b_eq=None, b_pol=None, b_np=None, src1=None, ksize=3, halo=True, up0=False,
             flip_north_pole=True, act=nat.ACT_NONE, alpha=0.0, vmax=0.0, premask0=None, premask1=None, dy_premasked=False,
-            defer_ring0=False, want_pool=False, out_padded=False, small=False):
+            defer_ring0=False, want_pool=False, out_padded=False, small=False, band=False):
     if (w_np is None) != (b_np is None) and b_eq is not None:
         raise ValueError('cs_conv: north-pole kernel and bias must be given together')
     c0_valid = 0
@@ -668,7 +681,7 @@
             c0_valid = cin_w
     return _CSConv.apply(src0, src1, w_eq, w_pol, w_np, b_eq, b_pol, b_np, int(ksize), bool(halo), bool(up0),
                          bool(flip_north_pole), int(act), float(alpha), float(vmax), int(c0_valid), premask0, premask1,
-                         bool(dy_premasked), bool(defer_ring0), bool(want_pool), bool(out_padded), bool(small))
+                         bool(dy_premasked), bool(defer_ring0), bool(want_pool), bool(out_padded), bool(small), bool(band))
 
 
 def cs_conv_head_applicable(src0, src1, w_eq, head_w_eq, out_padded):
diff --git a/dlwp-cs_amd/DLWP/options.py b/dlwp-cs_amd/DLWP/options.py
--- a/dlwp-cs_amd/DLWP/options.py
+++ b/dlwp-cs_amd/DLWP/options.py
@@ -3,7 +3,7 @@
 DEFAULTS = {
     'graphs': True, 'premask': True, 'wgrad_batch': True, 'fuse_adam': True, 'fuse_pack': True, 'fuse_head': True,
     'fold_loss_tail': True, 'fuse_pool': True, 'fold_ring': True, 'cf_model': True, 'padded_io': True, 'host_staging': True, 'resident_data': True,
-    'dgrad_gather': True, 'fold_head': True, 'small_conv': True, 'check_finite': False,
+    'dgrad_gather': True, 'fold_head': True, 'small_conv': True, 'band_conv': True, 'check_finite': False,
 }
 
 
diff --git a/dlwp-cs_amd/build.py b/dlwp-cs_amd/build.py
--- a/dlwp-cs_amd/build.py
+++ b/dlwp-cs_amd/build.py
@@ -10,7 +10,7 @@
 OBJ = os.path.join(HERE, 'build' + ('_' + TAG if TAG else ''))
 LIBDIR = os.path.join(HERE, 'lib')
 LIB = os.path.join(LIBDIR, 'libdlwpcs%s.so' % ('_' + TAG if TAG else ''))
-SOURCES = ['halo_table.cpp', 'prof.cpp', 'comm.cpp', 'elementwise.hip', 'conv_mfma.hip', 'conv_inst_f32.hip', 'conv_inst_bf16.hip', 'conv_inst_edge.hip', 'conv_small.hip',
+SOURCES = ['halo_table.cpp', 'prof.cpp', 'comm.cpp', 'elementwise.hip', 'conv_mfma.hip', 'conv_inst_f32.hip', 'conv_inst_bf16.hip', 'conv_inst_edge.hip', 'conv_small.hip', 'conv_band.hip',
            'conv_generic.hip', 'wgrad_batch.hip', 'verify.hip', 'remap.hip', 'climatology.hip', 'solar.hip', 'scaling.hip', 'overlap.hip', 'packed.hip',
            'bilinear.hip', 'missing.hip', 'spectrum.hip', 'masked_loss.hip', 'ensemble.hip']
 HIPCC = os.environ.get('HIPCC', '/opt/rocm/bin/hipcc')
diff --git a/dlwp-cs_amd/csrc/conv_band.hip b/dlwp-cs_amd/csrc/conv_band.hip
--- /dev/null
+++ b/dlwp-cs_amd/csrc/conv_band.hip
@@ -0,0 +1,275 @@
+#include "conv_ws.h"
+
+namespace dlwpcs {
+
+struct BandParams {
+    const void *src;
+    const void *wpk;
+    const float *bias;
+    const int32_t *table;
+    void *out;
+    int B, N, W2;
+    int R, NB;
+    int Cin, Cout, CG, NT;
+    int Q;
+    uint32_t magicQ, magicN, magicNT, magicNB, magicB;
+    int act;
+    float alpha, vmax;
+    int patch_base;
+};
+
+constexpr int BD_THREADS = 256, BD_WAVES = 4;
+constexpr int BD_PROW = 32 * 2 + 16;
+constexpr int BD_U = 16;
+constexpr int BD_MAXPIX = 384;
+
+template <int MTW>
+__global__ void __launch_bounds__(BD_THREADS, 2) conv_band_kernel(const BandParams P) {
+    extern __shared__ __attribute__((aligned(16))) char smem[];
+    const int tid = threadIdx.x;
+    const int lane = tid & 63, wave = __builtin_amdgcn_readfirstlane(tid >> 6);
+    const int half = lane >> 5, l31 = lane & 31;
+    const uint32_t t = xcd_remap(blockIdx.x, gridDim.x);
+    const int q1 = P.magicNT ? __umulhi(t, P.magicNT) : (int)t;
+    const int nt = (int)t - q1 * P.NT;
+    const int bf = P.magicNB ? __umulhi((uint32_t)q1, P.magicNB) : q1;
+    const int band = q1 - bf * P.NB;
+    const int f = P.magicB ? __umulhi((uint32_t)bf, P.magicB) : bf;
+    const int b = bf - f * P.B;
+    const int v = f < 4 ? 0 : (f == 4 ? 1 : 2);
+    const int RB = P.Cin * 2 + 16;
+    const int r0 = band * P.R;
+    const int rows = min(P.R, P.N - r0);
+    const int band_pix = rows * P.N;
+    const int nitems = (rows + 2) * P.W2 * P.Q;
+    const int tbase = (f * P.W2 + r0) * P.W2;
+
+    const uint4 *wsrc = reinterpret_cast<const uint4 *>(P.wpk) + ((size_t)v * P.NT + nt) * P.CG * 576 + lane;
+    auto load_w = [&](int cg, uint4 (&w)[9]) __attribute__((always_inline)) {
+        const uint4 *p = wsrc + (size_t)min(cg, P.CG - 1) * 576;
+#pragma unroll
+        for (int tap = 0; tap < 9; ++tap) w[tap] = p[tap * 64];
+    };
+    uint4 wa[9], wb[9];
+    load_w(0, wa);
+
+    {
+        const int spix = 6 * P.N * P.N;
+        const rsrc_t rs = make_rsrc(reinterpret_cast<const bf16_t *>(P.src) + (size_t)b * spix * P.Cin, (uint32_t)(spix * P.Cin * 2));
+#pragma unroll 1
+        for (int e0 = 0; e0 < nitems; e0 += BD_THREADS * BD_U) {
+            int sp[BD_U];
+#pragma unroll
+            for (int u = 0; u < BD_U; ++u) {
+                const int e = e0 + tid + u * BD_THREADS;
+                const bool live = e < nitems;
+                const int cell = __umulhi((uint32_t)e, P.magicQ);
+                sp[u] = P.table[live ? tbase + cell : 0];
+                if (!live) sp[u] = -1;
+            }
+            u32x4 val[BD_U];
+#pragma unroll
+            for (int u = 0; u < BD_U; ++u) {
+                const int e = e0 + tid + u * BD_THREADS;
+                const int cell = __umulhi((uint32_t)e, P.magicQ), qv = e - cell * P.Q;
+                const uint32_t off = sp[u] >= 0 ? (uint32_t)(sp[u] * P.Cin + qv * 8) * 2u : ST_SKIP;
+                val[u] = __builtin_amdgcn_raw_buffer_load_b128(rs, off, 0, 0);
+            }
+#pragma unroll
+            for (int u = 0; u < BD_U; ++u) {
+                const int e = e0 + tid + u * BD_THREADS;
+                const int cell = __umulhi((uint32_t)e, P.magicQ), qv = e - cell * P.Q;
+                if (e < nitems) *reinterpret_cast<uint4 *>(smem + cell * RB + qv * 16) = make_uint4(val[u].x, val[u].y, val[u].z, val[u].w);
+            }
+        }
+    }
+
+    const int nmt = (band_pix + 31) >> 5;
+    const int wv = (wave + (int)(blockIdx.x >> 3) + (int)(blockIdx.x >> 8)) & (BD_WAVES - 1);
+    const int my_mt = max(0, min(MTW, (nmt - wv + BD_WAVES - 1) / BD_WAVES));
+    int abase[MTW];
+#pragma unroll
+    for (int i = 0; i < MTW; ++i) {
+        const int m = (wv + BD_WAVES * i) * 32 + l31;
+        int base = 0;
+        if (m < band_pix) {
+            const int oy = __umulhi((uint32_t)m, P.magicN), ox = m - oy * P.N;
+            base = (oy * P.W2 + ox) * RB;
+        }
+        abase[i] = base + half * 16;
+    }
+    float4 bq[4];
+#pragma unroll
+    for (int jq = 0; jq < 4; ++jq)
+        bq[jq] = P.bias ? *reinterpret_cast<const float4 *>(P.bias + (size_t)v * P.NT * 32 + nt * 32 + 8 * jq + 4 * half)
+                        : make_float4(0.f, 0.f, 0.f, 0.f);
+    f32x16 acc[MTW];
+
+    load_w(1, wb);
+    __syncthreads();
+    if (my_mt == 0) return;
+
+    auto matrix = [&](auto mta_tag) __attribute__((always_inline)) {
+        constexpr int MTA = decltype(mta_tag)::value;
+        constexpr int BD_R = MTA == 1 ? 6 : 3, BD_D = BD_R - 1;
+        uint4 fa[BD_R][MTA];
+#pragma unroll
+        for (int i = 0; i < MTA; ++i)
+#pragma unroll
+            for (int jq = 0; jq < 4; ++jq) {
+                acc[i][4 * jq] = bq[jq].x; acc[i][4 * jq + 1] = bq[jq].y; acc[i][4 * jq + 2] = bq[jq].z; acc[i][4 * jq + 3] = bq[jq].w;
+            }
+        auto rd = [&](int cg, int tap, uint4 (&a)[MTA]) __attribute__((always_inline)) {
+            const char *lds = smem + cg * 32 + ((tap / 3) * P.W2 + tap % 3) * RB;
+#pragma unroll
+            for (int i = 0; i < MTA; ++i) a[i] = *reinterpret_cast<const uint4 *>(lds + abase[i]);
+        };
+#pragma unroll
+        for (int st = 0; st < BD_D; ++st) rd(0, st, fa[st % BD_R]);
+        __builtin_amdgcn_sched_group_barrier(0x100, BD_D * MTA, 0);
+#pragma unroll 1
+        for (int cg = 0; cg < P.CG; cg += 2) {
+#pragma unroll
+            for (int st = 0; st < 18; ++st) {
+                rd(cg + (st + BD_D) / 9, (st + BD_D) % 9, fa[(st + BD_D) % BD_R]);
+#pragma unroll
+                for (int i = 0; i < MTA; ++i) frag_mma<bf16_t>(acc[i], st < 9 ? wa[st] : wb[st - 9], fa[st % BD_R][i]);
+                __builtin_amdgcn_sched_group_barrier(0x100, MTA, 0);
+                __builtin_amdgcn_sched_group_barrier(0x008, MTA, 0);
+                if (st == 8) { asm volatile("" ::: "memory"); load_w(cg + 2, wa); }
+                if (st == 17) { asm volatile("" ::: "memory"); load_w(cg + 3, wb); }
+            }
+        }
+    };
+    if (MTW >= 3 && my_mt >= 3) matrix(std::integral_constant<int, (MTW >= 3 ? 3 : 1)>{});
+    else if (MTW >= 2 && my_mt == 2) matrix(std::integral_constant<int, (MTW >= 2 ? 2 : 1)>{});
+    else matrix(std::integral_constant<int, 1>{});
+
+    constexpr int NPS = 2;
+    uint32_t soff[MTW][NPS];
+    const int c = nt * 32 + (lane & 3) * 8;
+    const int face_pix = P.N * P.N;
+#pragma unroll
+    for (int i = 0; i < MTW; ++i)
+#pragma unroll
+        for (int ps = 0; ps < NPS; ++ps) {
+            const int m = (wv + BD_WAVES * i) * 32 + ps * 16 + (lane >> 2);
+            const int off = ((f * face_pix + r0 * P.N + m) * P.Cout + c) * 2;
+            soff[i][ps] = m < band_pix ? (uint32_t)off : ST_SKIP;
+        }
+    const float e_alpha = P.act == DLWPCS_ACT_LEAKY_CLIP ? P.alpha : 1.f;
+    const float e_vmax = P.act == DLWPCS_ACT_LEAKY_CLIP ? P.vmax : __builtin_inff();
+    const bool fast_act = e_alpha >= 0.f && e_alpha <= 1.f && e_vmax >= 0.f;
+    const int amode = P.act != DLWPCS_ACT_LEAKY_CLIP ? 2 : (fast_act ? 1 : 0);
+    auto quad = [&](const f32x16 &a, int jq) __attribute__((always_inline)) {
+        float4 v4 = make_float4(a[4 * jq], a[4 * jq + 1], a[4 * jq + 2], a[4 * jq + 3]);
+        if (amode == 2) return v4;
+        if (amode == 1) {
+            typedef float f32x2 __attribute__((ext_vector_type(2)));
+            auto lc = [&](float x, float ax) {
+                float tt, y;
+                asm("v_max_f32 %0, %1, %2" : "=v"(tt) : "v"(x), "v"(ax));
+                asm("v_minimum3_f32 %0, %1, %2, %2" : "=v"(y) : "v"(tt), "v"(e_vmax));
+                return y;
+            };
+            const f32x2 a01 = f32x2{v4.x, v4.y} * e_alpha, a23 = f32x2{v4.z, v4.w} * e_alpha;
+            v4.x = lc(v4.x, a01.x); v4.y = lc(v4.y, a01.y); v4.z = lc(v4.z, a23.x); v4.w = lc(v4.w, a23.y);
+        } else {
+            v4.x = act_leaky_clip(v4.x, e_alpha, e_vmax); v4.y = act_leaky_clip(v4.y, e_alpha, e_vmax);
+            v4.z = act_leaky_clip(v4.z, e_alpha, e_vmax); v4.w = act_leaky_clip(v4.w, e_alpha, e_vmax);
+        }
+        return v4;
+    };
+    const rsrc_t d_out = make_rsrc(reinterpret_cast<bf16_t *>(P.out) + (size_t)b * 6 * face_pix * P.Cout, (uint32_t)(6 * face_pix * P.Cout * 2));
+    char *const patch = smem + P.patch_base + wave * (32 * BD_PROW);
+#pragma unroll
+    for (int i = 0; i < MTW; ++i) {
+        if (i < my_mt) {
+#pragma unroll
+            for (int k = 0; k < 4; ++k) {
+                const float4 v4 = quad(acc[i], k);
+                *reinterpret_cast<uint2 *>(patch + l31 * BD_PROW + (8 * k + 4 * half) * 2) = make_uint2(f2bf2(v4.x, v4.y), f2bf2(v4.z, v4.w));
+            }
+            __builtin_amdgcn_wave_barrier();
+#pragma unroll
+            for (int ps = 0; ps < NPS; ++ps) {
+                const uint4 o = *reinterpret_cast<const uint4 *>(patch + (ps * 16 + (lane >> 2)) * BD_PROW + (lane & 3) * 16);
+                bst128(o, d_out, soff[i][ps]);
+            }
+            __builtin_amdgcn_wave_barrier();
+        }
+    }
+}
+
+static int g_tune_rows = 0;
+
+static size_t band_lds(int R, int N, int Cin) { return (size_t)(R + 2) * (N + 2) * (Cin * 2 + 16) + (size_t)BD_WAVES * 32 * BD_PROW; }
+
+static int band_rows(int N, int Cin) {
+    int R = BD_MAXPIX / N;
+    if (R > N) R = N;
+    while (R > 1 && 2 * band_lds(R, N, Cin) > 160 * 1024) --R;
+    return R;
+}
+
+bool conv_band_serves(int B, int N, int Cin, int Cout) {
+    if (!(N * N > 320 && N <= BD_MAXPIX && Cin >= 32 && Cout >= 32 && Cin % 32 == 0 && Cout % 32 == 0 && B >= 0)) return false;
+    const int R = band_rows(N, Cin);
+    const long nwg = (long)B * 6 * ceil_div(N, R) * (Cout / 32);
+    const int cmax = Cin > Cout ? Cin : Cout;
+    return band_lds(R, N, Cin) <= 160 * 1024 && nwg < (1l << 16) && (long)(R + 2) * (N + 2) * (Cin / 8) < (1l << 16) &&
+           (long)6 * N * N * cmax * 2 < (1l << 31);
+}
+
+static int launch_band_t(const BandParams &P, int mtw, size_t lds, unsigned grid, hipStream_t s) {
+    auto go = [&](auto kern) -> int {
+        if (lds > 64 * 1024) {
+            hipError_t e = hipFuncSetAttribute((const void *)kern, hipFuncAttributeMaxDynamicSharedMemorySize, (int)lds);
+            if (e != hipSuccess) return fail(DLWPCS_E_LAUNCH, "conv_band: hipFuncSetAttribute: %s", hipGetErrorString(e));
+        }
+        hipLaunchKernelGGL(kern, dim3(grid), dim3(BD_THREADS), lds, s, P);
+        return check_launch("conv_band");
+    };
+    if (mtw == 1) return go(conv_band_kernel<1>);
+    if (mtw == 2) return go(conv_band_kernel<2>);
+    return go(conv_band_kernel<3>);
+}
+
+int launch_conv_band(const ConvKParams &K, hipStream_t s) {
+    if (K.mode != MODE_HALO) return fail(DLWPCS_E_UNSUPPORTED, "conv_band: serves halo convolutions");
+    const int N = K.Nin;
+    if (K.C1 != 0 || K.up0 || K.ymask || K.pool_out || K.head_w || K.edge)
+        return fail(DLWPCS_E_UNSUPPORTED, "conv_band: one source, no upsampling, no mask on load, no pooled or folded second output");
+    if (K.No != N || !conv_band_serves(K.B, N, K.Cin, K.Cout))
+        return fail(DLWPCS_E_UNSUPPORTED, "conv_band: B=%d N=%d Cin=%d Cout=%d outside faces of more than 320 cells with channel counts that are multiples of 32",
+                    K.B, N, K.Cin, K.Cout);
+    BandParams P{};
+    P.src = K.src0; P.wpk = K.wpk; P.bias = K.bias; P.table = K.table; P.out = K.out;
+    P.B = K.B; P.N = N; P.W2 = N + 2;
+    P.R = band_rows(N, K.Cin);
+    if (g_tune_rows > 0 && g_tune_rows <= N && g_tune_rows * N <= BD_MAXPIX && band_lds(g_tune_rows, N, K.Cin) <= 160 * 1024)
+        P.R = g_tune_rows;
+    P.NB = ceil_div(N, P.R);
+    P.Cin = K.Cin; P.Cout = K.Cout; P.CG = K.Cin / 16; P.NT = K.Cout / 32; P.Q = K.Cin / 8;
+    P.magicQ = div_magic(P.Q); P.magicN = div_magic(N);
+    P.magicNT = P.NT > 1 ? div_magic(P.NT) : 0; P.magicNB = P.NB > 1 ? div_magic(P.NB) : 0; P.magicB = P.B > 1 ? div_magic(P.B) : 0;
+    P.act = K.act; P.alpha = K.alpha; P.vmax = K.vmax;
+    const size_t lds = band_lds(P.R, N, P.Cin);
+    P.patch_base = (int)(lds - (size_t)BD_WAVES * 32 * BD_PROW);
+    const int mtw = ceil_div(ceil_div(P.R * N, 32), BD_WAVES);
+    const long nwg = (long)P.B * 6 * P.NB * P.NT;
+    if (mtw > 3 || nwg >= (1l << 16))
+        return fail(DLWPCS_E_UNSUPPORTED, "conv_band: B=%d N=%d Cin=%d beyond the kernel's index range", P.B, N, P.Cin);
+    if (K.pool_done) *K.pool_done = 0;
+    if (K.head_done) *K.head_done = 0;
+    if (K.dry_run || K.B == 0) return DLWPCS_OK;
+    return launch_band_t(P, mtw, lds, (unsigned)nwg, s);
+}
+
+}
+
+extern "C" int dlwpcs_conv_band_tune(int rows) {
+    if (rows < 0) return dlwpcs::fail(DLWPCS_E_INVALID, "conv_band_tune: rows >= 0");
+    dlwpcs::g_tune_rows = rows;
+    return DLWPCS_OK;
+}
diff --git a/dlwp-cs_amd/csrc/conv_mfma.hip b/dlwp-cs_amd/csrc/conv_mfma.hip
--- a/dlwp-cs_amd/csrc/conv_mfma.hip
+++ b/dlwp-cs_amd/csrc/conv_mfma.hip
@@ -1215,6 +1215,12 @@
     return d->dtype == DLWPCS_BF16 && d->ksize == 3 && d->halo && d->C1 == 0 && !d->up0 && d->c0_valid == 0 &&
            !(d->flags & DLWPCS_CONV_OUT_PADDED) && conv_small_serves(d->B, d->N, d->C0, d->Cout);
 }
+bool conv_band_serves(int B, int N, int Cin, int Cout);
+int launch_conv_band(const ConvKParams &K, hipStream_t s);
+static bool conv_band_layer_ok(const dlwpcs_conv_desc *d) {
+    return d->dtype == DLWPCS_BF16 && d->ksize == 3 && d->halo && d->C1 == 0 && !d->up0 && d->c0_valid == 0 &&
+           !(d->flags & DLWPCS_CONV_OUT_PADDED) && conv_band_serves(d->B, d->N, d->C0, d->Cout);
+}
 
 struct WsLayout {
     size_t wpk_f, bias, wpk_b, dxv, dz, partial, bpartial, total;
@@ -1477,7 +1483,7 @@
                          const void *b_eq, const void *b_pol, const void *b_np,
                          void *y, const int32_t *table_dev,
                          void *workspace, size_t workspace_bytes, dlwpcs_stream_t stream, void *y_pooled, int *pool_done,
-                         const ConvHeadArgs *head = nullptr, bool small = false);
+                         const ConvHeadArgs *head = nullptr, int alt = 0);
 
 extern "C" int dlwpcs_conv_fwd(const dlwpcs_conv_desc *d, const void *src0, const void *src1,
                                const void *w_eq, const void *w_pol, const void *w_np,
@@ -1540,11 +1546,14 @@
                          const void *b_eq, const void *b_pol, const void *b_np,
                          void *y, const int32_t *table_dev,
                          void *workspace, size_t workspace_bytes, dlwpcs_stream_t stream, void *y_pooled, int *pool_done,
-                         const ConvHeadArgs *head, bool small) {
+                         const ConvHeadArgs *head, int alt) {
     int rc = validate(d, "conv_fwd");
     if (rc) return rc;
+    const bool small = alt == 1, band = alt == 2;
     if (small && !conv_small_layer_ok(d))
         return fail(DLWPCS_E_UNSUPPORTED, "conv_small_fwd: serves bf16 3x3 halo layers with one source on faces of <= 320 cells, channel counts multiples of 32");
+    if (band && !conv_band_layer_ok(d))
+        return fail(DLWPCS_E_UNSUPPORTED, "conv_band_fwd: serves bf16 3x3 halo layers with one source on faces of more than 320 cells, channel counts multiples of 32");
     if (!src0 || !w_eq || (!w_pol && !(d->flags & DLWPCS_CONV_PREPACKED)) || !y || !workspace)
         return fail(DLWPCS_E_INVALID, "conv_fwd: null pointer");
     if (d->C1 > 0 && !src1) return fail(DLWPCS_E_INVALID, "conv_fwd: C1 > 0 but src1 is null");
@@ -1579,6 +1588,7 @@
     if ((d->flags & DLWPCS_CONV_OUT_PADDED) && !pw_applies(d))
         return fail(DLWPCS_E_UNSUPPORTED, "conv_fwd: DLWPCS_CONV_OUT_PADDED serves the bf16 pointwise output layer only");
     if (small) return launch_conv_small(P, s);
+    if (band) return launch_conv_band(P, s);
     if (pw_applies(d)) {
         PwParams Q{};
         Q.in = (const bf16_t *)src0; Q.wpk = (const bf16_t *)wpk; Q.bias = b_eq ? bpk : nullptr; Q.out = (bf16_t *)y;
@@ -1794,7 +1804,16 @@
                                      void *y, const int32_t *table_dev,
                                      void *workspace, size_t workspace_bytes, dlwpcs_stream_t stream) {
     return conv_fwd_impl(d, src0, src1, w_eq, w_pol, w_np, b_eq, b_pol, b_np, y, table_dev, workspace, workspace_bytes, stream,
-                         nullptr, nullptr, nullptr, true);
+                         nullptr, nullptr, nullptr, 1);
+}
+
+extern "C" int dlwpcs_conv_band_fwd(const dlwpcs_conv_desc *d, const void *src0, const void *src1,
+                                    const void *w_eq, const void *w_pol, const void *w_np,
+                                    const void *b_eq, const void *b_pol, const void *b_np,
+                                    void *y, const int32_t *table_dev,
+                                    void *workspace, size_t workspace_bytes, dlwpcs_stream_t stream) {
+    return conv_fwd_impl(d, src0, src1, w_eq, w_pol, w_np, b_eq, b_pol, b_np, y, table_dev, workspace, workspace_bytes, stream,
+                         nullptr, nullptr, nullptr, 2);
 }
 
 extern "C" int dlwpcs_conv_small_bwd_data(const dlwpcs_conv_desc *d, const void *dz,
diff --git a/include/dlwpcs.h b/include/dlwpcs.h
--- a/include/dlwpcs.h
+++ b/include/dlwpcs.h
@@ -117,6 +117,14 @@
                                void *dsrc0, void *dsrc1, const void *m0, const void *m1, float m_alpha, float m_vmax,
                                const int32_t *inv_table_dev,
                                void *workspace, size_t workspace_bytes, dlwpcs_stream_t stream);
+
+int dlwpcs_conv_band_fwd(const dlwpcs_conv_desc *d,
+                         const void *src0, const void *src1,
+                         const void *w_eq, const void *w_pol, const void *w_np,
+                         const void *b_eq, const void *b_pol, const void *b_np,
+                         void *y, const int32_t *table_dev,
+                         void *workspace, size_t workspace_bytes, dlwpcs_stream_t stream);
+int dlwpcs_conv_band_tune(int rows);
 
 int dlwpcs_conv_ring_info(const dlwpcs_conv_desc *d, size_t *dxv_offset, int *channels);
 
```

Result: no change. 48860 samples/s (median of 2 runs) (+0.3%).
